# mudit1729/dinov2-od

Measured on AMD Instinct MI355X. Metric: images/sec forward, DINOv2 ViT-B/14 518x518 + 100-query head, higher is better.
Workload: dtype bf16; 1 GPU; ViT-B/14 518x518 bf16, 100 queries, batch 64 per GPU (BASELINE configs[2]'s batch of 64; it fits one GPU, so every GPU runs the whole configuration: weak scaling); global_batch=64, per_gpu_batch=64, image=518, queries=100, parallelism=dp1, hipgraph=True, n_ranks_seen=1, micro_batches=2

## Files before the change

dinov2_od_amd/csrc/dod_api.hip:

```cpp
#include "dod_internal.h"
#include "gemm_plan.h"

#include <cstdarg>
#include <cstdio>
#include <atomic>
#include <cstdlib>

using namespace dod;

static std::string g_err;

static int vfail(const dod_handle* h, int code, const char* fmt, va_list ap, int launch_rc = 0) {
  char buf[512];
  const int n = vsnprintf(buf, sizeof buf, fmt, ap);
  if (launch_rc && n >= 0 && (size_t)n < sizeof buf) snprintf(buf + n, sizeof buf - n, " rejected (rc %d)", launch_rc);
  if (h) h->err = buf; else g_err = buf;
  return code;
}
int dod::fail(const dod_handle* h, int code, const char* fmt, ...) {
  va_list ap; va_start(ap, fmt); code = vfail(h, code, fmt, ap); va_end(ap);
  return code;
}
int dod::rejected(const dod_handle* h, int r, const char* fmt, ...) {
  if (!r) return DOD_OK;
  va_list ap; va_start(ap, fmt); const int code = vfail(h, r == 3 ? DOD_ERR_HIP : DOD_ERR_INVALID, fmt, ap, r); va_end(ap);
  return code;
}

static bool check_common(dod_handle* h, int B, int H, int W, int* rc) {
  if (!h) { *rc = fail(nullptr, DOD_ERR_INVALID, "null handle"); return false; }
  if (!h->finalized) { *rc = fail(h, DOD_ERR_STATE, "dod_finalize_weights has not been called"); return false; }
  if (B <= 0) { *rc = fail(h, DOD_ERR_INVALID, "batch must be positive (got %d)", B); return false; }
  if (H < h->cfg.patch || W < h->cfg.patch) { *rc = fail(h, DOD_ERR_INVALID, "image %dx%d smaller than one %dx%d patch", H, W, h->cfg.patch, h->cfg.patch); return false; }
  return true;
}

static std::atomic<int> g_options[DOD_OPT_COUNT] = {{-1}, {-1}, {-1}, {-1}, {-1}, {-1}, {-1}, {-1}, {-1}, {-1}, {-1}};
int dod_option(int which) { return which >= 0 && which < DOD_OPT_COUNT ? g_options[which].load() : -1; }
static const char* const k_option_names[DOD_OPT_COUNT] = {"tailsplit", "dec_fused_split", "mha_chunk_images", "no_fused_patch", "ln_fold", "deterministic", "f32_ksplit",
                                                       "attn_bwd_flash", "epi_regmath", "f32x3_tile", "attn_diet"};

static std::atomic<long> g_form_launches[FORM_COUNT];
static const char* const k_form_names[FORM_COUNT] = {"bf16_128_r2", "bf16_128_r3", "bf16_m16", "k64", "ppm", "x3_16w", "x3_pp", "h2", "fp8_rows", "fp8mx_256x128",
                                                     "fp8mx2_256x128", "fp8mx2_256x256", "f32", "patch_fused"};
void gemm_form_launched(int form) { if (form >= 0 && form < FORM_COUNT) ++g_form_launches[form]; }

extern "C" {

int dod_test_set_option(const char* name, int value) {
  if (!name) return fail(nullptr, DOD_ERR_INVALID, "null option name");
  for (int i = 0; i < DOD_OPT_COUNT; ++i)
    if (!strcmp(name, k_option_names[i])) { g_options[i].store(value); return DOD_OK; }
  return fail(nullptr, DOD_ERR_INVALID, "unknown test option '%s'", name);
}
long dod_test_counter(const char* name) {
  if (name && !strcmp(name, "tail_splits")) return gemm_tail_split_count();
  if (name && !strcmp(name, "rem_cuts")) return gemm_rem_cut_count();
  if (name && !strcmp(name, "f32_ksplits")) return gemm_f32_ksplit_count();
  if (name && !strcmp(name, "epi_regmath")) return gemm_epi_regmath_count();
  if (name && !strcmp(name, "attn_diet")) return attn_half_tile_count();
  if (name && !strcmp(name, "f32x3_launches")) return gemm_f32x3_count(0);
  if (name && !strcmp(name, "f32x3_wide_launches")) return gemm_f32x3_count(1);
  if (name && !strcmp(name, "optim_launches")) return optim_launch_count();
  if (name && !strcmp(name, "optim_chunk_elems")) return optim_constant(0);
  if (name && !strcmp(name, "optim_table_tensors")) return optim_constant(1);
  if (name && !strcmp(name, "optim_norm_table_tensors")) return optim_constant(2);
  if (name && !strncmp(name, "form_", 5))
    for (int i = 0; i < FORM_COUNT; ++i)
      if (!strcmp(name + 5, k_form_names[i])) return g_form_launches[i].load();
  return -1;
}

int dod_test_gemm_plan(int family, int M, int N, int K, unsigned epi_flags, int cus, size_t scratch_bytes, dod_gemm_step* steps, int max_steps) {
  if (family < GEMM_BF16 || family > GEMM_F32 || M <= 0 || N <= 0 || K <= 0 || cus <= 0 || !steps) return -1;
  const GemmPlan pl = gemm_plan(family, M, N, K, epi_flags, gemm_policy(cus, scratch_bytes, scratch_bytes > 0));
  if (pl.n > 4 || pl.n > max_steps) return -1;
  for (int i = 0; i < pl.n; ++i) {
    const GemmStep& st = pl.step[i];
    steps[i].form = st.form; steps[i].row0 = st.row0; steps[i].rows = st.rows; steps[i].kslices = st.kslices; steps[i].regmath = st.regmath; steps[i].gm = st.gm;
  }
  return pl.n;
}

const char* dod_version(void) { return "dinodet 0.3 (gfx950)"; }
int dod_abi_version(void) { return DOD_ABI_VERSION; }

int dod_device_count(void) {
  int n = 0;
  return hipGetDeviceCount(&n) == hipSuccess ? n : -1;
}

const char* dod_last_error(const dod_handle* h) { return h ? h->err.c_str() : g_err.c_str(); }

int dod_create(const dod_config* cfg, dod_handle** out) {
  if (!cfg || !out) return fail(nullptr, DOD_ERR_INVALID, "null argument");
  const dod_config& c = *cfg;
  if (c.hidden <= 0 || c.layers <= 0 || c.heads <= 0 || c.hidden % c.heads) return fail(nullptr, DOD_ERR_INVALID, "bad backbone dims hidden=%d heads=%d layers=%d", c.hidden, c.heads, c.layers);
  if (c.hidden % 64) return fail(nullptr, DOD_ERR_INVALID, "hidden (%d) must be a multiple of 64", c.hidden);
  {
    const int fm = c.precision == DOD_PREC_FP32 ? 4 : 64;
    if (c.ffn_hidden <= 0 || c.ffn_hidden % fm) return fail(nullptr, DOD_ERR_INVALID, "ffn_hidden (%d) must be a multiple of %d in this precision", c.ffn_hidden, fm);
  }
  if (c.patch <= 0 || c.pos_grid <= 0) return fail(nullptr, DOD_ERR_INVALID, "bad patch/pos_grid");
  if (c.num_queries <= 0 || c.dec_hidden <= 0 || c.dec_heads <= 0 || c.dec_layers <= 0 || c.num_classes <= 0 || c.dim_feedforward <= 0) return fail(nullptr, DOD_ERR_INVALID, "bad decoder dims");
  if (c.dec_hidden % 64 || c.dim_feedforward % 4) return fail(nullptr, DOD_ERR_INVALID, "decoder hidden (%d) must be a multiple of 64, dim_feedforward (%d) of 4", c.dec_hidden, c.dim_feedforward);
  if (c.target_dim && c.target_dim != c.dec_hidden) return fail(nullptr, DOD_ERR_INVALID, "projection dim %d != decoder hidden %d", c.target_dim, c.dec_hidden);
  if (!c.target_dim && c.hidden != c.dec_hidden) return fail(nullptr, DOD_ERR_INVALID, "backbone width %d != decoder hidden %d and no projection", c.hidden, c.dec_hidden);
  if (c.use_deformable && (c.n_points <= 0 || c.n_points > 8)) return fail(nullptr, DOD_ERR_INVALID, "n_points must be 1..8");
  if (c.dec_layers > 64) return fail(nullptr, DOD_ERR_INVALID, "at most 64 decoder layers");
  if (c.precision != DOD_PREC_FP32 && c.precision != DOD_PREC_BF16 && c.precision != DOD_PREC_FP8 && c.precision != DOD_PREC_BF16X3 && c.precision != DOD_PREC_FP16X2) return fail(nullptr, DOD_ERR_INVALID, "unknown precision %d", c.precision);
  dod_handle* h = new (std::nothrow) dod_handle();
  if (!h) return fail(nullptr, DOD_ERR_STATE, "out of host memory");
  h->cfg = c;
  *out = h;
  return DOD_OK;
}

void dod_destroy(dod_handle* h) {
  if (!h) return;
  for (auto& r : h->prof) { (void)hipEventDestroy(r.a); (void)hipEventDestroy(r.b); }
  for (auto e : h->evpool) (void)hipEventDestroy(e);
  for (void* p : h->owned) (void)hipFree(p);
  delete h;
}

int dod_set_weight(dod_handle* h, const char* key, const void* dev_ptr, const int64_t* shape, int ndim, int dtype) {
  if (!h || !key || !dev_ptr || ndim < 0 || ndim > 8 || (ndim && !shape)) return fail(h, DOD_ERR_INVALID, "dod_set_weight: bad argument");
  if (dtype != DOD_F32 && dtype != DOD_BF16) return fail(h, DOD_ERR_INVALID, "dod_set_weight('%s'): dtype %d is neither DOD_F32 nor DOD_BF16", key, dtype);
  std::string k(key);
  if (k.rfind("module.", 0) == 0) k = k.substr(7);
  WRef r; r.raw = dev_ptr; r.dtype = dtype; r.ptr = dtype == DOD_F32 ? (const float*)dev_ptr : nullptr; r.shape.assign(shape, shape + ndim);
  h->w[k] = r;
  h->finalized = false;
  return DOD_OK;
}

int dod_reserve_gemm_scratch(size_t bytes) { return (gemm_tail_reserve(bytes) || gemm_f32_ksplit_reserve()) ? fail(nullptr, DOD_ERR_HIP, "scratch allocation of %zu bytes failed", bytes) : DOD_OK; }

int dod_finalize_weights(dod_handle* h, void* stream) {
  if (!h) return fail(nullptr, DOD_ERR_INVALID, "null handle");
  { static const size_t mb = [] { const char* v = getenv("DINODET_GEMM_SCRATCH_MB"); return v && atoi(v) > 0 ? (size_t)atoi(v) : (size_t)64; }();
    (void)gemm_tail_reserve(mb << 20);
    (void)gemm_f32_ksplit_reserve(); }
  int rc = finalize_impl(h, (hipStream_t)stream);
  if (rc || !h->has_dec) return rc;
  hipStream_t s = (hipStream_t)stream;
  const dod_config& g = h->cfg;
  const size_t Q = g.num_queries, Dd = g.dec_hidden;
  h->l0_tgt = h->l0_proj = nullptr;
  Carver sz(nullptr);
  const size_t bytes = carve_decoder(h, sz, 1, 1, nullptr, false) + 256;
  void* tmp = nullptr;
  float *t0 = nullptr, *p0 = nullptr;
  HIPCHK(h, hipMalloc(&tmp, bytes));
  if (hipMalloc((void**)&t0, Q * Dd * 4) != hipSuccess || (g.use_deformable && hipMalloc((void**)&p0, Q * (size_t)h->ncat * 4) != hipSuccess)) {
    (void)hipFree(tmp); if (t0) (void)hipFree(t0);
    return fail(h, DOD_ERR_HIP, "allocation of the decoder's layer-0 constants failed");
  }
  h->owned.push_back(t0); if (p0) h->owned.push_back(p0);
  Carver cv((void*)(((uintptr_t)tmp + 255) & ~(uintptr_t)255));
  DecWS dw;
  carve_decoder(h, cv, 1, 1, &dw, false);
  rc = decoder_impl(h, nullptr, 1, 1, dw, nullptr, s, true);
  if (!rc) {
    hipError_t e1 = hipMemcpyAsync(t0, dw.tgt, Q * Dd * 4, hipMemcpyDeviceToDevice, s);
    hipError_t e2 = p0 ? hipMemcpyAsync(p0, dw.proj, Q * (size_t)h->ncat * 4, hipMemcpyDeviceToDevice, s) : hipSuccess;
    hipError_t e3 = hipStreamSynchronize(s);
    if (e1 != hipSuccess || e2 != hipSuccess || e3 != hipSuccess) rc = fail(h, DOD_ERR_HIP, "decoder layer-0 constants: %s", hipGetErrorString(e3 != hipSuccess ? e3 : (e1 != hipSuccess ? e1 : e2)));
  } else (void)hipStreamSynchronize(s);
  (void)hipFree(tmp);
  if (rc) return rc;
  h->l0_tgt = t0; h->l0_proj = p0;
  return DOD_OK;
}

int dod_prepare(dod_handle* h, int H, int W, void* stream) {
  if (!h) return fail(nullptr, DOD_ERR_INVALID, "null handle");
  return prepare_impl(h, H, W, (hipStream_t)stream);
}

int dod_num_tokens(const dod_handle* h, int H, int W) { return h ? (H / h->cfg.patch) * (W / h->cfg.patch) + 1 : 0; }

size_t dod_workspace_bytes(const dod_handle* h, int B, int H, int W) {
  if (!h || B <= 0 || H < h->cfg.patch || W < h->cfg.patch) return 0;
  const int N = dod_num_tokens(h, H, W);
  Carver c(nullptr);
  carve_backbone(h, c, B, N, nullptr);
  carve_decoder(h, c, B, N, nullptr, false);
  return c.off + 256;
}

size_t dod_decoder_workspace_bytes(const dod_handle* h, int B, int N) {
  if (!h || B <= 0 || N <= 0) return 0;
  Carver c(nullptr);
  carve_decoder(h, c, B, N, nullptr, true);
  return c.off + 256;
}

int dod_set_tap(dod_handle* h, int stage, float* dst) {
  if (!h) return fail(nullptr, DOD_ERR_INVALID, "null handle");
  if (dst) h->taps[stage] = dst; else h->taps.erase(stage);
  return DOD_OK;
}

int dod_forward(dod_handle* h, const float* pixels, int B, int H, int W, float* det, void* workspace, size_t wsb, void* stream) {
  int rc;
  if (!check_common(h, B, H, W, &rc)) return rc;
  if (!pixels || !det || !workspace) return fail(h, DOD_ERR_INVALID, "null buffer");
  if (wsb < dod_workspace_bytes(h, B, H, W)) return fail(h, DOD_ERR_STATE, "workspace too small: %zu < %zu", wsb, dod_workspace_bytes(h, B, H, W));
  const int N = dod_num_tokens(h, H, W);
  Carver c(align_ws(workspace));
  BbWS bw; DecWS dw;
  carve_backbone(h, c, B, N, &bw);
  carve_decoder(h, c, B, N, &dw, false);
  CARVE_FITS(h, c, workspace, wsb)
  rc = backbone_impl(h, pixels, B, H, W, bw, nullptr, true, (hipStream_t)stream); if (rc) return rc;
  return decoder_impl(h, bw.mem, B, N, dw, det, (hipStream_t)stream);
}

int dod_forward_u8(dod_handle* h, const uint8_t* pixels_hwc, int B, int H, int W, float* det, void* workspace, size_t wsb, void* stream) {
  int rc;
  if (!check_common(h, B, H, W, &rc)) return rc;
  if (!pixels_hwc || !det || !workspace) return fail(h, DOD_ERR_INVALID, "null buffer");
  if (wsb < dod_workspace_bytes(h, B, H, W)) return fail(h, DOD_ERR_STATE, "workspace too small: %zu < %zu", wsb, dod_workspace_bytes(h, B, H, W));
  const int N = dod_num_tokens(h, H, W);
  Carver c(align_ws(workspace));
  BbWS bw; DecWS dw;
  carve_backbone(h, c, B, N, &bw);
  carve_decoder(h, c, B, N, &dw, false);
  CARVE_FITS(h, c, workspace, wsb)
  rc = backbone_impl(h, nullptr, B, H, W, bw, nullptr, true, (hipStream_t)stream, -1, nullptr, pixels_hwc); if (rc) return rc;
  return decoder_impl(h, bw.mem, B, N, dw, det, (hipStream_t)stream);
}

int dod_backbone_forward(dod_handle* h, const float* pixels, int B, int H, int W, float* features, void* workspace, size_t wsb, void* stream) {
  int rc;
  if (!check_common(h, B, H, W, &rc)) return rc;
  if (!pixels || !features || !workspace) return fail(h, DOD_ERR_INVALID, "null buffer");
  if (wsb < dod_workspace_bytes(h, B, H, W)) return fail(h, DOD_ERR_STATE, "workspace too small: %zu < %zu", wsb, dod_workspace_bytes(h, B, H, W));
  const int N = dod_num_tokens(h, H, W);
  Carver c(align_ws(workspace));
  BbWS bw;
  carve_backbone(h, c, B, N, &bw);
  CARVE_FITS(h, c, workspace, wsb)
  return backbone_impl(h, pixels, B, H, W, bw, features, false, (hipStream_t)stream);
}

int dod_backbone_prefix(dod_handle* h, const float* pixels, int B, int H, int W, int nblocks, float* x_out, void* workspace, size_t wsb, void* stream) {
  int rc;
  if (!check_common(h, B, H, W, &rc)) return rc;
  if (!pixels || !x_out || !workspace) return fail(h, DOD_ERR_INVALID, "null buffer");
  if (nblocks < 0 || nblocks > h->cfg.layers) return fail(h, DOD_ERR_INVALID, "nblocks %d outside 0..%d", nblocks, h->cfg.layers);
  if (wsb < dod_workspace_bytes(h, B, H, W)) return fail(h, DOD_ERR_STATE, "workspace too small: %zu < %zu", wsb, dod_workspace_bytes(h, B, H, W));
  const int N = dod_num_tokens(h, H, W);
  Carver c(align_ws(workspace));
  BbWS bw;
  carve_backbone(h, c, B, N, &bw);
  CARVE_FITS(h, c, workspace, wsb)
  return backbone_impl(h, pixels, B, H, W, bw, nullptr, false, (hipStream_t)stream, nblocks, x_out);
}

int dod_decoder_forward(dod_handle* h, const float* memory, int B, int N, float* det, void* workspace, size_t wsb, void* stream) {
  if (!h) return fail(nullptr, DOD_ERR_INVALID, "null handle");
  if (!h->finalized) return fail(h, DOD_ERR_STATE, "dod_finalize_weights has not been called");
  if (B <= 0 || N <= 0) return fail(h, DOD_ERR_INVALID, "bad B=%d N=%d", B, N);
  if (!memory || !det || !workspace) return fail(h, DOD_ERR_INVALID, "null buffer");
  if (wsb < dod_decoder_workspace_bytes(h, B, N)) return fail(h, DOD_ERR_STATE, "workspace too small");
  Carver c(align_ws(workspace));
  DecWS dw;
  carve_decoder(h, c, B, N, &dw, true);
  CARVE_FITS(h, c, workspace, wsb)
  hipStream_t s = (hipStream_t)stream;
  const void* mem_op = memory;
  if (is_bf16(h)) {
    KCHK(h, launch_cast_bf16(memory, (bf16_t*)dw.mem_op, (size_t)B * N * h->cfg.dec_hidden, s));
    mem_op = dw.mem_op;
  }
  return decoder_impl(h, mem_op, B, N, dw, det, s);
}

int dod_profile(dod_handle* h, int enable) {
  if (!h) return fail(nullptr, DOD_ERR_INVALID, "null handle");
  for (auto& r : h->prof) { h->evpool.push_back(r.a); h->evpool.push_back(r.b); }
  h->prof.clear();
  h->prof_on = enable != 0;
  return DOD_OK;
}

int dod_profile_read(dod_handle* h, int cls, double* ms, double* flops, int* launches) {
  if (!h || cls < 0 || cls >= PC_COUNT) return fail(h, DOD_ERR_INVALID, "bad profile class");
  double t = 0, f = 0; int n = 0;
  for (auto& r : h->prof) {
    if (r.cls != cls) continue;
    HIPCHK(h, hipEventSynchronize(r.b));
    float e = 0.f;
    HIPCHK(h, hipEventElapsedTime(&e, r.a, r.b));
    t += e; f += r.flops; ++n;
  }
  if (ms) *ms = t; if (flops) *flops = f; if (launches) *launches = n;
  return DOD_OK;
}

int dod_op_linear(int in_dtype, const void* A, int lda, const void* W, int ldw, int M, int N, int K, const float* bias,
                  const float* scale, const float* resid, int ldr, void* out, int out_dtype, int ldc, int act, void* stream) {
  if (!A || !W || !out) return fail(nullptr, DOD_ERR_INVALID, "null buffer");
  GemmEpi e = epi(bias, out_dtype == DOD_F32 ? (float*)out : nullptr, out_dtype == DOD_BF16 ? out : nullptr, ldc, act, scale, resid, ldr);
  if (act == DOD_ACT_SWIGLU_PAIRS) {
    if (in_dtype != DOD_BF16 || out_dtype != DOD_BF16 || scale || resid || (N & 7)) return fail(nullptr, DOD_ERR_INVALID, "DOD_ACT_SWIGLU_PAIRS: bf16 in / out, N %% 8 == 0, no scale / residual");
    e.act = ACT_NONE; e.glu = 1;
  }
  int r = in_dtype == DOD_BF16 ? launch_gemm_bf16((const bf16_t*)A, lda, (const bf16_t*)W, ldw, M, N, K, e, (hipStream_t)stream)
                               : launch_gemm_f32((const float*)A, lda, (const float*)W, ldw, M, N, K, e, (hipStream_t)stream);
  return rejected(nullptr, r, "dod_op_linear M=%d N=%d K=%d", M, N, K);
}
int dod_op_gemm_f32x(const float* A, int lda, int a_kmajor, long long a_sb, long long a_sh, const float* W, int ldw, int w_kmajor, long long w_sb,
                     long long w_sh, float* C, int ldc, long long c_sb, long long c_sh, int M, int N, int K, int batch, int hb, float alpha,
                     int accumulate, int ksplit, void* stream) {
  if (!A || !W || !C) return fail(nullptr, DOD_ERR_INVALID, "null buffer");
  GemmF32X g; memset(&g, 0, sizeof g);
  g.A = A; g.lda = lda; g.a_kmajor = a_kmajor; g.a_sb = a_sb; g.a_sh = a_sh;
  g.W = W; g.ldw = ldw; g.w_kmajor = w_kmajor; g.w_sb = w_sb; g.w_sh = w_sh;
  g.C = C; g.ldc = ldc; g.c_sb = c_sb; g.c_sh = c_sh;
  g.M = M; g.N = N; g.K = K; g.batch = batch; g.hb = hb; g.alpha = alpha; g.accumulate = accumulate; g.ksplit = ksplit;
  return rejected(nullptr, launch_gemm_f32x(g, (hipStream_t)stream), "dod_op_gemm_f32x M=%d N=%d K=%d batch=%d", M, N, K, batch);
}
int dod_op_gemm_f32x3(const float* A, int lda, int a_kmajor, long long a_sb, long long a_sh, const float* W, int ldw, int w_kmajor, long long w_sb,
                      long long w_sh, float* C, int ldc, long long c_sb, long long c_sh, int M, int N, int K, int batch, int hb, float alpha,
                      int accumulate, int ksplit, void* stream) {
  if (!A || !W || !C) return fail(nullptr, DOD_ERR_INVALID, "null buffer");
  GemmF32X g; memset(&g, 0, sizeof g);
  g.A = A; g.lda = lda; g.a_kmajor = a_kmajor; g.a_sb = a_sb; g.a_sh = a_sh;
  g.W = W; g.ldw = ldw; g.w_kmajor = w_kmajor; g.w_sb = w_sb; g.w_sh = w_sh;
  g.C = C; g.ldc = ldc; g.c_sb = c_sb; g.c_sh = c_sh;
  g.M = M; g.N = N; g.K = K; g.batch = batch; g.hb = hb; g.alpha = alpha; g.accumulate = accumulate; g.ksplit = ksplit;
  return rejected(nullptr, launch_gemm_f32x3(g, (hipStream_t)stream), "dod_op_gemm_f32x3 M=%d N=%d K=%d batch=%d", M, N, K, batch);
}
int dod_op_linear_f32x3(const float* X, int ldx, const float* W, const float* bias, const float* scale, const float* resid, int ldr, int M, int N, int K,
                        float* Y, int ldy, int act, void* stream) {
  if (!X || !W || !Y) return fail(nullptr, DOD_ERR_INVALID, "null buffer");
  if (act < DOD_ACT_NONE || act > DOD_ACT_SIGMOID) return fail(nullptr, DOD_ERR_INVALID, "dod_op_linear_f32x3: activation %d", act);
  GemmF32X g; memset(&g, 0, sizeof g);
  g.A = X; g.lda = ldx; g.W = W; g.ldw = K; g.C = Y; g.ldc = ldy; g.M = M; g.N = N; g.K = K; g.batch = 1; g.hb = 1; g.alpha = 1.0f; g.ksplit = 1;
  g.bias = bias; g.scale = scale; g.resid = resid; g.ldr = ldr; g.act = act;
  return rejected(nullptr, launch_gemm_f32x3(g, (hipStream_t)stream), "dod_op_linear_f32x3 M=%d N=%d K=%d", M, N, K);
}
int dod_op_linear_fp8(const void* A, int lda, const float* a_scale, const void* W, int ldw, const float* w_scale, int M, int N, int K,
                      const float* bias, const float* scale, const float* resid, int ldr, void* out, int out_dtype, int ldc, int act,
                      void* stream) {
  if (!A || !W || !out || !a_scale || !w_scale) return fail(nullptr, DOD_ERR_INVALID, "null buffer");
  GemmEpi e = epi(bias, out_dtype == DOD_F32 ? (float*)out : nullptr, out_dtype == DOD_BF16 ? out : nullptr, ldc, act, scale, resid, ldr);
  e.a_scale = a_scale; e.w_scale = w_scale;
  return rejected(nullptr, launch_gemm_fp8((const unsigned char*)A, lda, (const unsigned char*)W, ldw, M, N, K, e, (hipStream_t)stream), "dod_op_linear_fp8 M=%d N=%d K=%d", M, N, K);
}
int dod_op_linear_fp8_mx(const void* A, int lda, const void* a_block_scales, const void* W, int ldw, const float* w_scale, int M, int N, int K,
                         const float* bias, const float* scale, const float* resid, int ldr, void* out, int out_dtype, int ldc, int act,
                         void* stream) {
  if (!A || !W || !out || !a_block_scales || !w_scale) return fail(nullptr, DOD_ERR_INVALID, "null buffer");
  GemmEpi e = epi(bias, out_dtype == DOD_F32 ? (float*)out : nullptr, out_dtype == DOD_BF16 ? out : nullptr, ldc, act, scale, resid, ldr);
  e.a_bs = (const unsigned char*)a_block_scales; e.w_scale = w_scale;
  return rejected(nullptr, launch_gemm_fp8((const unsigned char*)A, lda, (const unsigned char*)W, ldw, M, N, K, e, (hipStream_t)stream), "dod_op_linear_fp8_mx M=%d N=%d K=%d", M, N, K);
}
int dod_op_linear_fp8_glu_mx(const void* A, int lda, const float* a_scale, const void* W, int ldw, const float* w_scale, int M, int N, int K,
                             const float* bias, void* out_q, int ldq, void* out_block_scales, void* stream) {
  if (!A || !W || !a_scale || !w_scale || !out_q || !out_block_scales) return fail(nullptr, DOD_ERR_INVALID, "null buffer");
  GemmEpi e = epi(bias, nullptr, out_q, ldq);
  e.a_scale = a_scale; e.w_scale = w_scale; e.glu = 1; e.out_bs = (unsigned char*)out_block_scales;
  return rejected(nullptr, launch_gemm_fp8((const unsigned char*)A, lda, (const unsigned char*)W, ldw, M, N, K, e, (hipStream_t)stream), "dod_op_linear_fp8_glu_mx M=%d N=%d K=%d", M, N, K);
}
int dod_op_linear_fp8_mx2(const void* A, int lda, const void* a_block_scales, const void* W, int ldw, const void* w_block_scales, int M, int N, int K,
                          const float* bias, const float* scale, const float* resid, int ldr, void* out, int out_dtype, int ldc, int act,
                          void* glu_out_block_scales, void* stream) {
  if (!A || !W || !out || !a_block_scales || !w_block_scales) return fail(nullptr, DOD_ERR_INVALID, "null buffer");
  GemmEpi e = epi(bias, out_dtype == DOD_F32 ? (float*)out : nullptr, out_dtype == DOD_BF16 ? out : nullptr, ldc, act, scale, resid, ldr);
  e.a_bs = (const unsigned char*)a_block_scales; e.w_bs = (const unsigned char*)w_block_scales;
  if (glu_out_block_scales) { e.out_f32 = nullptr; e.out_bf16 = (bf16_t*)out; e.glu = 1; e.out_bs = (unsigned char*)glu_out_block_scales; }
  return rejected(nullptr, launch_gemm_fp8((const unsigned char*)A, lda, (const unsigned char*)W, ldw, M, N, K, e, (hipStream_t)stream), "dod_op_linear_fp8_mx2 M=%d N=%d K=%d", M, N, K);
}
int dod_op_quant_mx_fp8(const void* x, int in_dtype, int ld, int rows, int cols, void* q, int ldq, void* block_scales, void* stream) {
  if (!x || !q || !block_scales) return fail(nullptr, DOD_ERR_INVALID, "null buffer");
  return rejected(nullptr, launch_quant_mx_fp8(x, in_dtype == DOD_BF16, ld, rows, cols, (unsigned char*)q, ldq, (unsigned char*)block_scales, (hipStream_t)stream), "dod_op_quant_mx_fp8 rows=%d cols=%d", rows, cols);
}
int dod_op_split_pair(const float* x, int ld, int rows, int cols, void* out, void* stream) {
  if (!x || !out) return fail(nullptr, DOD_ERR_INVALID, "null buffer");
  return launch_split2(x, ld, (bf16_t*)out, rows, cols, (hipStream_t)stream) ? fail(nullptr, DOD_ERR_HIP, "launch failed") : DOD_OK;
}
int dod_op_linear_x3(const void* A2, const void* W2, int M, int N, int K, const float* bias, const float* scale, const float* resid, int ldr,
                     void* out, int out_layout, int ldc, int act, void* stream) {
  if (!A2 || !W2 || !out) return fail(nullptr, DOD_ERR_INVALID, "null buffer");
  GemmEpi e = epi(bias, out_layout == 0 ? (float*)out : nullptr, out_layout != 0 ? out : nullptr, ldc, act, scale, resid, ldr);
  if (out_layout == 2) e.out_split = -N;
  return rejected(nullptr, launch_gemm_x3((const bf16_t*)A2, 2 * K, (const bf16_t*)W2, 2 * K, M, N, K, e, (hipStream_t)stream), "dod_op_linear_x3 M=%d N=%d K=%d", M, N, K);
}
int dod_op_split_h2(const float* x, int ld, int rows, int cols, void* out, void* wexp, void* stream) {
  if (!x || !out) return fail(nullptr, DOD_ERR_INVALID, "null buffer");
  return rejected(nullptr, launch_split_h2(x, ld, out, rows, cols, (unsigned char*)wexp, (hipStream_t)stream), "dod_op_split_h2 rows=%d cols=%d", rows, cols);
}
int dod_op_linear_h2(const void* A, const void* W, const void* wexp, int M, int N, int K, const float* bias, const float* scale, const float* resid,
                     int ldr, void* out, int out_layout, int ldc, int act, void* stream) {
  if (!A || !W || !wexp || !out) return fail(nullptr, DOD_ERR_INVALID, "null buffer");
  GemmEpi e = epi(bias, out_layout == 0 ? (float*)out : nullptr, out_layout != 0 ? out : nullptr, ldc, act, scale, resid, ldr);
  if (out_layout == 2) e.out_split = -N;
  if (out_layout == 3) e.out_h2 = 1;
  e.h2_wexp = (const unsigned char*)wexp;
  return rejected(nullptr, launch_gemm_h2(A, 4 * K, W, 3 * K, M, N, K, e, (hipStream_t)stream), "dod_op_linear_h2 M=%d N=%d K=%d", M, N, K);
}
int dod_op_linear_ln(int family, const void* A, const void* W, const void* wexp, int M, int N, int K, const float* bias, const float* scale,
                     const float* resid, int ldr, void* out, int out_layout, int ldc, int act, const dod_ln_fold* ln, void* stream) {
  if (!A || !W || !out || !ln) return fail(nullptr, DOD_ERR_INVALID, "null buffer");
  if (family != DOD_PREC_BF16 && family != DOD_PREC_BF16X3 && family != DOD_PREC_FP16X2) return fail(nullptr, DOD_ERR_INVALID, "family must be a bf16 / bf16x3 / fp16x2 precision");
  if ((ln->stats == nullptr) != (ln->csum == nullptr)) return fail(nullptr, DOD_ERR_INVALID, "stats and csum go together");
  if (ln->stats && scale) return fail(nullptr, DOD_ERR_INVALID, "the folded consumer has no LayerScale");
  if (ln->part && !(resid && out_layout == 0)) return fail(nullptr, DOD_ERR_INVALID, "the folded producer is the fp32 residual epilogue");
  GemmEpi e = epi(bias, out_layout == 0 ? (float*)out : nullptr, out_layout != 0 ? out : nullptr, ldc, act, scale, resid, ldr);
  if (out_layout == 2) e.out_split = -N;
  if (out_layout == 3) e.out_h2 = 1;
  e.ln_stats = (const float2*)ln->stats; e.ln_c = ln->csum;
  if (ln->part_in) {
    if (!ln->stats || ln->stats_out == ln->stats) return fail(nullptr, DOD_ERR_INVALID, "part_in needs stats (the shift) and a DIFFERENT stats_out buffer");
    e.ln_part_in = (const float2*)ln->part_in; e.ln_npart = (K + 127) / 128; e.ln_stats_out = (float2*)ln->stats_out; e.ln_eps = ln->eps;
  }
  if (ln->part) {
    e.ln_part = (float2*)ln->part; e.ln_npart = (N + 127) / 128; e.ln_op = ln->op_out; e.ln_shift = (const float2*)ln->shift;
    e.ln_op_kind = family == DOD_PREC_FP16X2 ? LNOP_H2 : (family == DOD_PREC_BF16X3 ? LNOP_PAIR : LNOP_BF16);
    e.ln_op_ld = family == DOD_PREC_BF16 ? N : 2 * N;
  }
  int r;
  if (family == DOD_PREC_FP16X2) {
    if (!wexp) return fail(nullptr, DOD_ERR_INVALID, "null buffer");
    e.h2_wexp = (const unsigned char*)wexp;
    r = launch_gemm_h2(A, 4 * K, W, 3 * K, M, N, K, e, (hipStream_t)stream);
  } else if (family == DOD_PREC_BF16X3) r = launch_gemm_x3((const bf16_t*)A, 2 * K, (const bf16_t*)W, 2 * K, M, N, K, e, (hipStream_t)stream);
  else r = launch_gemm_bf16((const bf16_t*)A, K, (const bf16_t*)W, K, M, N, K, e, (hipStream_t)stream);
  return rejected(nullptr, r, "dod_op_linear_ln M=%d N=%d K=%d", M, N, K);
}
int dod_op_rowstats(const float* x, int rows, int D, float eps, void* op_out, int family, void* stats, void* stream) {
  if (!x || !op_out || !stats) return fail(nullptr, DOD_ERR_INVALID, "null buffer");
  const int kind = family == DOD_PREC_FP16X2 ? LNOP_H2 : (family == DOD_PREC_BF16X3 ? LNOP_PAIR : (family == DOD_PREC_BF16 ? LNOP_BF16 : 0));
  return rejected(nullptr, launch_rowstats(x, rows, D, eps, op_out, kind, (float2*)stats, (hipStream_t)stream), "dod_op_rowstats rows=%d D=%d", rows, D);
}
int dod_op_ln_finalize(const void* part, int rows, int D, float eps, void* stats, void* stream) {
  if (!part || !stats) return fail(nullptr, DOD_ERR_INVALID, "null buffer");
  return rejected(nullptr, launch_ln_finalize((const float2*)part, (D + 127) / 128, rows, D, eps, (float2*)stats, (hipStream_t)stream), "dod_op_ln_finalize rows=%d D=%d", rows, D);
}
int dod_op_attention_x3(const void* qkv2, void* ctx2, int B, int N, int heads, float scale, void* stream) {
  if (!qkv2 || !ctx2) return fail(nullptr, DOD_ERR_INVALID, "null buffer");
  return rejected(nullptr, launch_attn_x3((const bf16_t*)qkv2, (bf16_t*)ctx2, B, N, heads, scale, (hipStream_t)stream), "dod_op_attention_x3");
}
static bool attn_grid_fits(int B, int N, int heads) {
  return (((long long)B * heads + 7) / 8 * 8) * (((long long)N + 127) / 128 + 1) <= 0x7fffffffLL;
}
int dod_op_attention_x3_h2(const void* qkv2, void* ctx_h2, int B, int N, int heads, float scale, void* stream) {
  if (!qkv2 || !ctx_h2) return fail(nullptr, DOD_ERR_INVALID, "null buffer");
  if (B <= 0 || N <= 0 || heads <= 0) return fail(nullptr, DOD_ERR_INVALID, "dod_op_attention_x3_h2: B=%d N=%d heads=%d must be positive", B, N, heads);
  if (!attn_grid_fits(B, N, heads)) return fail(nullptr, DOD_ERR_INVALID, "dod_op_attention_x3_h2: B=%d N=%d heads=%d is more workgroups than one launch holds", B, N, heads);
  return rejected(nullptr, launch_attn_x3((const bf16_t*)qkv2, (bf16_t*)ctx_h2, B, N, heads, scale, (hipStream_t)stream, 1), "dod_op_attention_x3_h2");
}
int dod_op_quant_rows_fp8(const void* x, int in_dtype, int ld, int rows, int cols, void* q, int ldq, float* scale, void* stream) {
  if (!x || !q || !scale) return fail(nullptr, DOD_ERR_INVALID, "null buffer");
  return rejected(nullptr, launch_quant_rows_fp8(x, in_dtype == DOD_BF16, ld, rows, cols, (unsigned char*)q, ldq, scale, (hipStream_t)stream), "dod_op_quant_rows_fp8 rows=%d cols=%d", rows, cols);
}
int dod_op_layernorm(const float* x, const float* add, const float* gamma, const float* beta, float eps, int rows, int D, void* out, int out_dtype, void* stream) {
  if (!x || !gamma || !beta || !out) return fail(nullptr, DOD_ERR_INVALID, "null buffer");
  return rejected(nullptr, launch_layernorm(x, add, gamma, beta, eps, rows, D, ln_out(out_dtype == DOD_F32 ? (float*)out : nullptr, out_dtype == DOD_BF16 ? (bf16_t*)out : nullptr), (hipStream_t)stream), "dod_op_layernorm rows=%d D=%d", rows, D);
}
int dod_op_attention_bf16(const void* qkv, void* ctx, int B, int N, int heads, float scale, void* stream) {
  if (!qkv || !ctx) return fail(nullptr, DOD_ERR_INVALID, "null buffer");
  return rejected(nullptr, launch_attn_bf16((const bf16_t*)qkv, (bf16_t*)ctx, B, N, heads, scale, (hipStream_t)stream), "dod_op_attention_bf16");
}
int dod_op_attention_bf16_mx(const void* qkv, void* ctx_q8, void* ctx_bs, int B, int N, int heads, float scale, void* stream) {
  if (!qkv || !ctx_q8 || !ctx_bs) return fail(nullptr, DOD_ERR_INVALID, "null buffer");
  if (B <= 0 || N <= 0 || heads <= 0) return fail(nullptr, DOD_ERR_INVALID, "dod_op_attention_bf16_mx: B=%d N=%d heads=%d must be positive", B, N, heads);
  if (!attn_grid_fits(B, N, heads)) return fail(nullptr, DOD_ERR_INVALID, "dod_op_attention_bf16_mx: B=%d N=%d heads=%d is more workgroups than one launch holds", B, N, heads);
  return rejected(nullptr, launch_attn_bf16((const bf16_t*)qkv, (bf16_t*)ctx_q8, B, N, heads, scale, (hipStream_t)stream, (unsigned char*)ctx_bs), "dod_op_attention_bf16_mx");
}
int dod_op_attention_f32(const float* q, const float* k, const float* v, float* o, int ldq, int ldk, int ldv, int ldo, int Lq, int Lk,
                         int B, int heads, int dh, float scale, void* stream) {
  if (!q || !k || !v || !o) return fail(nullptr, DOD_ERR_INVALID, "null buffer");
  AttnF32 a; a.q = q; a.k = k; a.v = v; a.o = o; a.ldq = ldq; a.ldk = ldk; a.ldv = ldv; a.ldo = ldo; a.Lq = Lq; a.Lk = Lk; a.B = B; a.heads = heads; a.dh = dh; a.scale = scale;
  return rejected(nullptr, launch_attn_f32(a, (hipStream_t)stream), "dod_op_attention_f32 (dh=%d)", dh);
}
int dod_op_deform_sample(const float* proj, int ldp, const float* values, int B, int Q, int N, int Hd, int P, int dh, int hh, int ww, float* out, void* stream) {
  if (!proj || !values || !out) return fail(nullptr, DOD_ERR_INVALID, "null buffer");
  if (hh * ww != N) return fail(nullptr, DOD_ERR_INVALID, "Cannot reshape input of size %d into a %dx%d feature map", N, hh, ww);
  return rejected(nullptr, launch_deform_sample(proj, ldp, values, B, Q, N, Hd, P, dh, hh, ww, out, (hipStream_t)stream), "dod_op_deform_sample");
}
int dod_op_pos_resize(const float* pos_in, int G, int gh, int gw, int D, float* pos_out, void* stream) {
  if (!pos_in || !pos_out) return fail(nullptr, DOD_ERR_INVALID, "null buffer");
  return launch_pos_resize(pos_in, G, gh, gw, D, pos_out, (hipStream_t)stream) ? fail(nullptr, DOD_ERR_HIP, "launch failed") : DOD_OK;
}
int dod_op_im2col(const float* img, int B, int H, int W, int patch, int Kp, void* out, int out_dtype, void* stream) {
  if (!img || !out) return fail(nullptr, DOD_ERR_INVALID, "null buffer");
  int r = launch_im2col(img, B, H, W, patch, Kp, out_dtype == DOD_F32 ? (float*)out : nullptr, out_dtype == DOD_BF16 ? (bf16_t*)out : nullptr, (hipStream_t)stream);
  return r ? fail(nullptr, DOD_ERR_INVALID, "dod_op_im2col rejected") : DOD_OK;
}

}
```

dinov2_od_amd/csrc/dod_common.h:

```cpp
#pragma once
#include <hip/hip_runtime.h>
#include <stdint.h>
#include <stdlib.h>

typedef __attribute__((ext_vector_type(8))) __bf16 bf16x8;
typedef __attribute__((ext_vector_type(4))) __bf16 bf16x4;
typedef __attribute__((ext_vector_type(2))) __bf16 bf16x2;
typedef __attribute__((ext_vector_type(16))) float f32x16;
typedef __attribute__((ext_vector_type(4))) float f32x4;
typedef __attribute__((ext_vector_type(2))) float f32x2;
typedef unsigned short bf16_t;

#define DOD_WAVE 64

enum { DOD_OPT_TAILSPLIT = 0,
       DOD_OPT_DEC_FUSED_SPLIT,
       DOD_OPT_MHA_CHUNK_IMAGES,
       DOD_OPT_NO_FUSED_PATCH,
       DOD_OPT_LN_FOLD,
       DOD_OPT_DETERMINISTIC,
       DOD_OPT_F32_KSPLIT,
       DOD_OPT_ATTN_BWD_FLASH,
       DOD_OPT_EPI_REGMATH,
       DOD_OPT_F32X3_TILE,
       DOD_OPT_ATTN_DIET,
       DOD_OPT_COUNT };
int dod_option(int which);
long gemm_tail_split_count();
long optim_launch_count();
long optim_constant(int which);
long gemm_rem_cut_count();
long attn_half_tile_count();
long gemm_epi_regmath_count();
enum { FORM_BF16_128_R2 = 0, FORM_BF16_128_R3, FORM_BF16_M16, FORM_K64, FORM_PPM, FORM_X3_16W, FORM_X3_PP, FORM_H2, FORM_FP8_ROWS, FORM_FP8MX_256X128,
       FORM_FP8MX2_256X128, FORM_FP8MX2_256X256, FORM_F32, FORM_PATCH_FUSED, FORM_COUNT };
void gemm_form_launched(int form);
enum { GEMM_BF16 = 0, GEMM_X3, GEMM_H2, GEMM_FP8, GEMM_F32 };

#ifdef DINODET_TUNING
#define DOD_TUNE_ENV(name) getenv(name)
#else
#define DOD_TUNE_ENV(name) (static_cast<const char*>(nullptr))
#endif

__device__ __forceinline__ bf16_t f2bf(float f) {
  __bf16 b = (__bf16)f;
  return __builtin_bit_cast(bf16_t, b);
}
__device__ __forceinline__ float bf2f(bf16_t h) {
  return __builtin_bit_cast(float, ((uint32_t)h) << 16);
}
__device__ __forceinline__ uint32_t pack2bf(float lo, float hi) {
  f32x2 v = {lo, hi};
  bf16x2 h = __builtin_convertvector(v, bf16x2);
  return __builtin_bit_cast(uint32_t, h);
}
__device__ __forceinline__ float wave_sum(float v) {
#pragma unroll
  for (int o = 32; o > 0; o >>= 1) v += __shfl_xor(v, o, 64);
  return v;
}
__device__ __forceinline__ float wave_max(float v) {
#pragma unroll
  for (int o = 32; o > 0; o >>= 1) v = fmaxf(v, __shfl_xor(v, o, 64));
  return v;
}
__device__ __forceinline__ unsigned pack4_fp8(float a, float b, float c, float d) {
  int w = __builtin_amdgcn_cvt_pk_fp8_f32(a, b, 0, false);
  w = __builtin_amdgcn_cvt_pk_fp8_f32(c, d, w, true);
  return (unsigned)w;
}
__device__ __forceinline__ unsigned mx_ebyte(float amax) {
  const unsigned b = __float_as_uint(amax * (1.0f / 448.0f));
  unsigned eb = ((b >> 23) & 0xffu) + ((b & 0x7fffffu) ? 1u : 0u);
  eb = eb < 1u ? 1u : (eb > 253u ? 253u : eb);
  return eb;
}
__device__ __forceinline__ float mx_inv_scale(unsigned eb) { return __uint_as_float((254u - eb) << 23); }
__device__ __forceinline__ size_t mx_scale_off(int K, int bi) { return (size_t)(bi & 1) * (K >> 6) + (bi >> 1); }
typedef __attribute__((ext_vector_type(2))) _Float16 f16x2;
typedef __attribute__((ext_vector_type(8))) _Float16 f16x8;
__device__ __forceinline__ float clampf_(float v, float lim) { return __builtin_fminf(__builtin_fmaxf(v, -lim), lim); }
__device__ __forceinline__ void h2_quad(float4 v, float shi, uint2& f16, unsigned& hi8, unsigned& lo8) {
  v.x = clampf_(v.x, 65504.f); v.y = clampf_(v.y, 65504.f); v.z = clampf_(v.z, 65504.f); v.w = clampf_(v.w, 65504.f);
  const f16x2 p0 = {(_Float16)v.x, (_Float16)v.y}, p1 = {(_Float16)v.z, (_Float16)v.w};
  f16.x = __builtin_bit_cast(unsigned, p0); f16.y = __builtin_bit_cast(unsigned, p1);
  const float hx = (float)p0.x, hy = (float)p0.y, hz = (float)p1.x, hw = (float)p1.y;
  const float slo = shi * 2048.0f;
  hi8 = pack4_fp8(clampf_(hx * shi, 448.f), clampf_(hy * shi, 448.f), clampf_(hz * shi, 448.f), clampf_(hw * shi, 448.f));
  lo8 = pack4_fp8(clampf_((v.x - hx) * slo, 448.f), clampf_((v.y - hy) * slo, 448.f), clampf_((v.z - hz) * slo, 448.f), clampf_((v.w - hw) * slo, 448.f));
}
__device__ __forceinline__ size_t h2_off8(int K, int c) { return (size_t)2 * K + (size_t)(c >> 4) * 32 + (c & 15); }

__device__ __forceinline__ float gelu_erf(float x) { return 0.5f * x * (1.0f + erff(x * 0.70710678118654752440f)); }
typedef float f32x2_t __attribute__((ext_vector_type(2)));
__device__ __forceinline__ f32x2_t gelu_fast2(f32x2_t x) {
  f32x2_t ax; ax.x = __builtin_fabsf(x.x); ax.y = __builtin_fabsf(x.y);
  const f32x2_t z = ax * 0.8493218002880191f;
  const f32x2_t d = __builtin_elementwise_fma(z, (f32x2_t)(0.2727374808792225f), (f32x2_t)(1.0f));
  f32x2_t t; t.x = __builtin_amdgcn_rcpf(d.x); t.y = __builtin_amdgcn_rcpf(d.y);
  f32x2_t p = __builtin_elementwise_fma(t, (f32x2_t)(0.5f * 1.061405429f), (f32x2_t)(0.5f * -1.453152027f));
  p = __builtin_elementwise_fma(p, t, (f32x2_t)(0.5f * 1.421413741f));
  p = __builtin_elementwise_fma(p, t, (f32x2_t)(0.5f * -0.284496736f));
  p = __builtin_elementwise_fma(p, t, (f32x2_t)(0.5f * 0.254829592f));
  const f32x2_t nz2 = -z * z;
  f32x2_t e; e.x = __builtin_amdgcn_exp2f(nz2.x); e.y = __builtin_amdgcn_exp2f(nz2.y);
  const f32x2_t q = ax * (t * p);
  const f32x2_t r = __builtin_elementwise_fma(ax, (f32x2_t)(0.5f), x * 0.5f);
  return __builtin_elementwise_fma(-q, e, r);
}
__device__ __forceinline__ void gelu_fast4(float4& v) {
  f32x2_t a = {v.x, v.y}, b = {v.z, v.w};
  a = gelu_fast2(a); b = gelu_fast2(b);
  v.x = a.x; v.y = a.y; v.z = b.x; v.w = b.y;
}
__device__ __forceinline__ float sigmoidf_(float x) { return 1.0f / (1.0f + expf(-x)); }

enum { ACT_NONE = 0, ACT_RELU = 1, ACT_GELU = 2, ACT_SIGMOID = 3 };

struct GemmEpi {
  const float* bias;
  const float* scale;
  const float* resid;
  int ldr;
  float* out_f32;
  bf16_t* out_bf16;
  int ldc;
  int act;
  const float* pos;
  int rows_per_img;
  int out_rows_per_img;
  int out_split;
  const float* a_scale;
  const float* w_scale;
  unsigned char* out_bs;
  const unsigned char* a_bs;
  const unsigned char* w_bs;
  int out_h2;
  const unsigned char* h2_wexp;
  int ksplit;
  int kslice_len;
  long long kslice_stride;
  int glu;
  void* ln_op;
  int ln_op_kind;
  int ln_op_ld;
  float2* ln_part;
  int ln_npart;
  const float2* ln_shift;
  const float2* ln_stats;
  const float* ln_c;
  const float2* ln_part_in;
  float2* ln_stats_out;
  float ln_eps;
};
enum { LNOP_BF16 = 1, LNOP_PAIR = 2, LNOP_H2 = 3 };
inline bool gemm_epi_rows_ok(const GemmEpi& e) {
  return e.rows_per_img == 0 && !e.pos && e.ksplit <= 1 && !e.a_scale && !e.a_bs && !e.out_bs;
}
inline GemmEpi gemm_epi_rows(const GemmEpi& e, int m0) {
  GemmEpi r = e;
  const size_t m = (size_t)m0;
  if (r.resid) r.resid += m * r.ldr;
  if (r.out_f32) r.out_f32 += m * r.ldc;
  if (r.out_bf16) r.out_bf16 += m * r.ldc;
  if (r.ln_op) r.ln_op = reinterpret_cast<char*>(r.ln_op) + m * (size_t)r.ln_op_ld * 2;
  if (r.ln_part) r.ln_part += m * r.ln_npart;
  if (r.ln_shift) r.ln_shift += m;
  if (r.ln_stats) r.ln_stats += m;
  if (r.ln_part_in) r.ln_part_in += m * r.ln_npart;
  if (r.ln_stats_out) r.ln_stats_out += m;
  return r;
}

int launch_gemm_bf16(const bf16_t* A, int lda, const bf16_t* W, int ldw, int M, int N, int K,
                     const GemmEpi& e, hipStream_t s);
int launch_gemm_f32(const float* A, int lda, const float* W, int ldw, int M, int N, int K,
                    const GemmEpi& e, hipStream_t s, bool allow_ksplit = false);
int gemm_f32_ksplit_reserve();
long gemm_f32_ksplit_count();
struct GemmF32X {
  const float* A; const float* W; float* C; const float* bias;
  const float* scale;
  const float* resid;
  int ldr;
  int lda, ldw, ldc, M, N, K;
  long long a_sb, a_sh, w_sb, w_sh, c_sb, c_sh;
  int batch, hb;
  int a_kmajor, w_kmajor;
  float alpha;
  int accumulate;
  int act;
  int ksplit;
};
int launch_gemm_f32x(const GemmF32X& g, hipStream_t s);
int launch_gemm_f32x3(const GemmF32X& g, hipStream_t s);
long gemm_f32x3_count(int wide);
int launch_quant_mx_fp8(const void* x, int in_bf16, int ld, int rows, int cols, unsigned char* q, int ldq, unsigned char* bs, hipStream_t s);
int launch_gemm_fp8(const unsigned char* A, int lda, const unsigned char* W, int ldw, int M, int N, int K,
                    const GemmEpi& e, hipStream_t s);
int launch_attn_x3(const bf16_t* qkv2, bf16_t* ctx3, int B, int N, int heads, float scale, hipStream_t s, int ctx_h2 = 0);
int launch_swiglu_fp8(const bf16_t* in, int rows, int Fh, unsigned char* q, float* scale, hipStream_t s);
int launch_quant_rows_fp8(const void* x, int in_bf16, int ld, int rows, int cols, unsigned char* q, int ldq, float* scale,
                          hipStream_t s);

struct LnOut {
  float* f32 = nullptr;
  bf16_t* bf16 = nullptr;
  unsigned char* fp8 = nullptr;
  float* scale = nullptr;
  bf16_t* split = nullptr;
  bf16_t* a3 = nullptr;
  unsigned char* bs = nullptr;
};
inline LnOut ln_out(float* f32, bf16_t* bf16 = nullptr, bf16_t* a3 = nullptr) { LnOut o; o.f32 = f32; o.bf16 = bf16; o.a3 = a3; return o; }
int launch_layernorm(const float* x, const float* add, const float* gamma, const float* beta, float eps, int rows, int D, const LnOut& out,
                     hipStream_t s, int split_h2 = 0);
int launch_rowstats(const float* x, int rows, int D, float eps, void* op, int op_kind, float2* stats, hipStream_t s);
int launch_ln_finalize(const float2* part, int npart, int rows, int D, float eps, float2* stats, hipStream_t s);
int launch_ln_fold(const float* W, int rows, int cols, const float* gamma, const float* beta, const float* bias_in, float* Wout, float* bias_out, hipStream_t s);
int launch_rowsum(const float* W, int rows, int cols, int round_bf16, float* c, hipStream_t s);

int launch_attn_bf16(const bf16_t* qkv, bf16_t* ctx, int B, int N, int heads, float scale, hipStream_t s, unsigned char* ctx_bs = nullptr);

struct AttnF32 {
  const float *q, *k, *v; float* o;
  int ldq, ldk, ldv, ldo;
  int Lq, Lk;
  int B, heads, dh;
  float scale;
  bf16_t* o3 = nullptr;
  float* lse = nullptr;
};
int launch_attn_f32(const AttnF32& a, hipStream_t s);
struct AttnF32Bwd {
  const float *q, *k, *v, *o, *d_o, *lse;
  float *dq, *dk, *dv, *delta;
  int ldq, ldk, ldv, ldo, lddq, lddk, lddv;
  int Lq, Lk, B, heads, dh;
  float scale;
};
int launch_attn_f32_bwd(const AttnF32Bwd& a, hipStream_t s);

int launch_im2col(const float* img, int B, int H, int W, int patch, int Kp, float* out_f32, bf16_t* out_bf16, hipStream_t s);
int launch_patch_pack(const float* W, int D, int p, bf16_t* out, int x3, hipStream_t s);
int launch_patch_embed(const void* img, int u8, int B, int H, int W, int p, const bf16_t* Wp, int x3, const float* bias, const float* pos,
                       float* out, int D, hipStream_t s);
int launch_cls_row(const float* cls, const float* pos, float* x, int B, int N, int D, hipStream_t s);
int launch_pos_resize(const float* pos_in, int G, int gh, int gw, int D, float* pos_out, hipStream_t s);
int launch_interleave_halves(const float* src, float* dst, int F, int cols, hipStream_t s);
int launch_swiglu(const float* in_f32, const bf16_t* in_bf16, int rows, int Fh, float* out_f32, bf16_t* out_bf16, hipStream_t s);
int launch_cast_bf16(const float* in, bf16_t* out, size_t n, hipStream_t s);
int launch_copy2d(const float* src, int ld_src, float* dst, int ld_dst, int rows, int cols, int cols_pad, hipStream_t s);
int launch_lora_merge(const float* W, const float* A, const float* Bm, float alpha, int out_f, int in_f, int r, float* dst, hipStream_t s);
int launch_split3(const float* in, int ld_in, bf16_t* out, int rows, int K, int mode, hipStream_t s);
int launch_split2(const float* in, int ld_in, bf16_t* out, int rows, int K, hipStream_t s);
int launch_split_h2(const float* in, int ld_in, void* out, int rows, int K, unsigned char* wexp, hipStream_t s);
int launch_gemm_h2(const void* A, int lda, const void* W, int ldw, int M, int N, int K, const GemmEpi& e, hipStream_t s);
int launch_gemm_x3(const bf16_t* A2, int lda, const bf16_t* W2, int ldw, int M, int N, int K, const GemmEpi& e, hipStream_t s);
int gemm_dispatch(int family, const void* A, int lda, const void* W, int ldw, int M, int N, int K, const GemmEpi& e, hipStream_t s, bool allow_ksplit = false);
int device_cus();
struct KernelLds { const void* fn; int bytes; };
void gemm_lds_attr_once(bool* done, const KernelLds* k, int n);
int gemm_tile_mode();
int run_gemm_bf16_128(const bf16_t* A, int lda, const bf16_t* W, int ldw, int M, int N, int K, const GemmEpi& e, int slots, hipStream_t s);
int run_gemm_bf16_m16(const bf16_t* A, int lda, const bf16_t* W, int ldw, int M, int N, int K, const GemmEpi& e, int gm, hipStream_t s);
int run_gemm_x3_16w(const bf16_t* A2, int lda, const bf16_t* W2, int ldw, int M, int N, int K, const GemmEpi& e, hipStream_t s);
int run_gemm_k64(const bf16_t* A, int lda, const bf16_t* W, int ldw, int M, int N, int K, const GemmEpi& e, bool regmath, hipStream_t s);
int run_gemm_pp(bool x3, const bf16_t* A, int lda, const bf16_t* W, int ldw, int M, int N, int K, const GemmEpi& e, hipStream_t s);
int run_gemm_h2(const void* A, int lda, const void* W, int ldw, int M, int N, int K, const GemmEpi& e, hipStream_t s);
int run_gemm_ksplit_reduce(const float* part, int S, int R, int N, const GemmEpi& e, int m_base, int M, int K, hipStream_t s);
int run_gemm_fp8(int form, const unsigned char* A, int lda, const unsigned char* W, int ldw, int M, int N, int K, const GemmEpi& e, int gm, hipStream_t s);
int run_gemm_f32(const float* A, int lda, const float* W, int ldw, int M, int N, int K, const GemmEpi& e, int S, hipStream_t s);
int gemm_tail_reserve(size_t bytes);
size_t gemm_tail_reserved();
float* gemm_tail_slab(hipStream_t s);
bool gemm_f32_ksplit_reserved();
int launch_bcast_rows(const float* src, float* dst, int B, int rows, int D, hipStream_t s);

int launch_deform_sample(const float* proj, int ldp, const float* values, int B, int Q, int N, int Hd, int P, int dh,
                         int h, int w, float* out, hipStream_t s, int proj_shared = 0, bf16_t* out3 = nullptr);
```

dinov2_od_amd/csrc/dod_forward.hip:

```cpp
#include "dod_internal.h"

#include <cmath>
#include <cstdlib>

using namespace dod;

size_t dod::carve_decoder(const dod_handle* h, Carver& c, int B, int N, DecWS* w, bool need_mem_op) {
  const dod_config& g = h->cfg;
  const size_t BQ = (size_t)B * g.num_queries, Dd = g.dec_hidden, M = (size_t)B * N;
  DecWS t;
  t.tgt = (float*)c.take(BQ * Dd * 4); t.t2 = (float*)c.take(BQ * Dd * 4); t.att = (float*)c.take(BQ * Dd * 4);
  t.samp = (float*)c.take(BQ * Dd * 4); t.qkv = (float*)c.take(BQ * 3 * Dd * 4);
  t.proj = (float*)c.take(BQ * (size_t)(h->ncat > 0 ? h->ncat : 4) * 4);
  t.ffn = (float*)c.take(BQ * (size_t)g.dim_feedforward * 4); t.hb = (float*)c.take(BQ * (Dd / 2) * 4);
  t.qd = (float*)c.take(BQ * Dd * 4);
  { const size_t kmax = Dd > (size_t)g.dim_feedforward ? Dd : (size_t)g.dim_feedforward;
    const bool want3 = is_bf16(h) || is_x3(h);
    t.a3 = want3 ? (bf16_t*)c.take(BQ * 3 * kmax * 2) : nullptr;
    t.a3b = want3 ? (bf16_t*)c.take(BQ * 3 * kmax * 2) : nullptr; }
  t.mem2 = is_x3(h) ? (bf16_t*)c.take(M * 2 * Dd * 2) : nullptr;
  t.mem_op = need_mem_op ? c.take(M * Dd * esz(h)) : nullptr;
  if (g.use_deformable) {
    int uniq = 0; for (auto& L : h->DL) if (L.vp_alias < 0) ++uniq;
    if (!h->finalized) uniq = g.dec_layers;
    t.values = (float*)c.take(M * Dd * 4 * (size_t)(uniq > 0 ? uniq : 1)); t.kv = nullptr;
  } else {
    t.values = nullptr; t.kv = (float*)c.take(M * 2 * Dd * 4);
  }
  if (w) *w = t;
  return c.off;
}

size_t dod::carve_backbone(const dod_handle* h, Carver& c, int B, int N, BbWS* w) {
  const dod_config& g = h->cfg;
  const size_t M = (size_t)B * N, D = g.hidden, es = esz(h), Np = N - 1;
  const size_t F1 = g.swiglu ? 2 * (size_t)g.ffn_hidden : (size_t)g.ffn_hidden;
  size_t hb = M * F1; const size_t col = (size_t)B * Np * (size_t)(h->Kp ? h->Kp : (3 * g.patch * g.patch + 63) / 64 * 64);
  if (col > hb) hb = col;
  BbWS t;
  t.x = (float*)c.take(M * D * 4); t.y = c.take(M * D * es); t.qkv = c.take(M * 3 * D * es); t.ctx = c.take(M * D * es);
  t.hbuf = c.take(hb * es); t.gated = g.swiglu ? c.take(M * (size_t)g.ffn_hidden * es) : nullptr;
  t.mem = c.take(M * (size_t)(g.target_dim ? g.target_dim : g.hidden) * es);
  t.rs = is_fp8(h) ? (float*)c.take(M * 4) : nullptr;
  t.bs = (is_fp8(h) && g.swiglu && g.ffn_hidden % 256 == 0) ? (unsigned char*)c.take(M * (size_t)(g.ffn_hidden / 32)) : nullptr;
  t.bsx = (is_fp8(h) && D % 256 == 0) ? (unsigned char*)c.take(M * (D / 32)) : nullptr;
  const bool foldable = ln_foldable(h);
  t.lnp = foldable ? (float2*)c.take(M * ((D + 127) / 128) * 8) : nullptr;
  t.lns = foldable ? (float2*)c.take(M * 8) : nullptr;
  t.lns2 = foldable ? (float2*)c.take(M * 8) : nullptr;
  if (w) *w = t;
  return c.off;
}

int dod::prepare_impl(dod_handle* h, int H, int W, hipStream_t s) {
  const dod_config& g = h->cfg;
  if (!h->finalized || !h->has_bb) return fail(h, DOD_ERR_STATE, "backbone weights not finalized");
  if (H < g.patch || W < g.patch) return fail(h, DOD_ERR_INVALID, "image %dx%d smaller than one patch", H, W);
  if (h->pos_H == H && h->pos_W == W) return DOD_OK;
  const int gh = H / g.patch, gw = W / g.patch;
  if (gh * gw == g.pos_grid * g.pos_grid && H == W) { h->pos_hw = h->pos; h->pos_H = H; h->pos_W = W; return DOD_OK; }
  const std::pair<int, int> key(gh, gw);
  auto it = h->pos_cache.find(key);
  if (it == h->pos_cache.end()) {
    hipStreamCaptureStatus cs = hipStreamCaptureStatusNone;
    if (s && hipStreamIsCapturing(s, &cs) == hipSuccess && cs != hipStreamCaptureStatusNone)
      return fail(h, DOD_ERR_STATE, "first forward at %dx%d inside a stream capture: call dod_prepare(h, %d, %d) before capturing", H, W, H, W);
    const size_t need = (size_t)(gh * gw + 1) * g.hidden;
    float* buf = nullptr;
    HIPCHK(h, hipMalloc((void**)&buf, need * 4));
    h->owned.push_back(buf);
    KCHK(h, launch_pos_resize(h->pos, g.pos_grid, gh, gw, g.hidden, buf, s));
    it = h->pos_cache.emplace(key, buf).first;
  }
  h->pos_hw = it->second; h->pos_H = H; h->pos_W = W;
  return DOD_OK;
}

namespace {

void spatial_factor(int hw, int* h, int* w) {
  int s = (int)std::sqrt((double)hw);
  while ((s + 1) * (s + 1) <= hw) ++s;
  while (s * s > hw) --s;
  if (s * s != hw) {
    for (int i = s; i > 0; --i) if (hw % i == 0) { *h = i; *w = hw / i; return; }
  }
  *h = s; *w = s;
}

int tap(dod_handle* h, int stage, const void* src, bool src_bf16, size_t n, hipStream_t s) {
  auto it = h->taps.find(stage);
  if (it == h->taps.end() || !it->second) return 0;
  if (!src_bf16) { (void)hipMemcpyAsync(it->second, src, n * 4, hipMemcpyDeviceToDevice, s); return 0; }
  return launch_widen_bf16((const bf16_t*)src, it->second, n, s);
}

int linear(dod_handle* h, bool bf, const void* A, int lda, const void* W, int ldw, int M, int N, int K, const GemmEpi& e, hipStream_t s, int flops_K = 0) {
  ProfScope ps(h, s, bf ? PC_GEMM_BF16 : PC_GEMM_F32, 2.0 * M * N * (e.rows_per_img > 0 ? 3.0 * h->cfg.patch * h->cfg.patch : (double)(flops_K ? flops_K : K)));
  int r = bf ? launch_gemm_bf16((const bf16_t*)A, lda, (const bf16_t*)W, ldw, M, N, K, e, s)
             : launch_gemm_f32((const float*)A, lda, (const float*)W, ldw, M, N, K, e, s, h->cfg.precision != DOD_PREC_FP32);
  return rejected(h, r, "linear launch (M=%d N=%d K=%d bf16=%d)", M, N, K, (int)bf);
}
int linear3(dod_handle* h, const void* A3, const void* W3, int M, int N, int K, const GemmEpi& e, hipStream_t s) {
  ProfScope ps(h, s, PC_GEMM_BF16, 2.0 * M * N * (double)K);
  int r = launch_gemm_x3((const bf16_t*)A3, 2 * K, (const bf16_t*)W3, 2 * K, M, N, K, e, s);
  return rejected(h, r, "bf16x3 linear launch (M=%d N=%d K=%d)", M, N, K);
}

struct Operand {
  const void* rows;
  const float* row_scale = nullptr;
  const unsigned char* bs = nullptr;
};

int block_linear(dod_handle* h, const Operand& a, const PackedLinear& W, int M, int N, int K, GemmEpi e, hipStream_t s) {
  if (is_h2(h)) {
    ProfScope ps(h, s, PC_GEMM_BF16, 2.0 * M * N * (double)K);
    e.h2_wexp = W.wexp;
    return rejected(h, launch_gemm_h2(a.rows, 4 * K, W.W, 3 * K, M, N, K, e, s), "fp16x2 linear launch (M=%d N=%d K=%d)", M, N, K);
  }
  if (is_x3(h)) return linear3(h, a.rows, W.W, M, N, K, e, s);
  if (W.wscale || W.wbs) {
    ProfScope ps(h, s, PC_GEMM_FP8, 2.0 * M * N * (double)K);
    e.a_scale = a.row_scale; e.w_scale = W.wscale; e.a_bs = a.bs; e.w_bs = W.wbs;
    return rejected(h, launch_gemm_fp8((const unsigned char*)a.rows, K, (const unsigned char*)W.W, K, M, N, K, e, s), "fp8 linear launch (M=%d N=%d K=%d)", M, N, K);
  }
  return linear(h, is_bf16(h), a.rows, K, W.W, K, M, N, K, e, s);
}

struct BlockRun {
  dod_handle* h; const BbWS& ws; hipStream_t s;
  int B, N, M, D, F;
  bool bf, f8, x3, h2, fold;
  float scale;
  float2* stat[2];
  int cur = 0;
  bool fresh = false;
  int op_kind, npart;

  BlockRun(dod_handle* h_, const BbWS& ws_, hipStream_t s_, int B_, int N_, bool fold_)
      : h(h_), ws(ws_), s(s_), B(B_), N(N_), M(B_ * N_), D(h_->cfg.hidden), F(h_->cfg.ffn_hidden), bf(is_bf16(h_)), f8(is_fp8(h_)), x3(is_x3(h_)),
        h2(is_h2(h_)), fold(fold_), scale(1.0f / std::sqrt((float)(h_->cfg.hidden / h_->cfg.heads))), stat{ws_.lns, ws_.lns2},
        op_kind(is_h2(h_) ? LNOP_H2 : (is_x3(h_) ? LNOP_PAIR : LNOP_BF16)), npart((h_->cfg.hidden + 127) / 128) {}

  bool mx(const BLayer& L) const { return f8 && L.qkv.wbs && ws.bsx; }

  GemmEpi residual_epi(const PackedLinear& W, const float* layer_scale, bool next_norm_reads) {
    GemmEpi e = epi(W.bias, ws.x, nullptr, D, ACT_NONE, layer_scale, ws.x, D);
    if (fold && next_norm_reads) {
      e.ln_op = ws.y; e.ln_op_kind = op_kind; e.ln_op_ld = (op_kind == LNOP_BF16 ? D : 2 * D); e.ln_part = ws.lnp; e.ln_npart = npart; e.ln_shift = stat[cur];
      fresh = true;
    }
    return e;
  }
  GemmEpi normed_epi(GemmEpi e, const PackedLinear& W) {
    if (fold) {
      e.ln_stats = stat[cur]; e.ln_c = W.csum;
      if (fresh) { e.ln_part_in = ws.lnp; e.ln_npart = npart; e.ln_stats_out = stat[cur ^ 1]; e.ln_eps = h->cfg.ln_eps; cur ^= 1; fresh = false; }
    }
    return e;
  }
  int norm(const BLayer& L, const float* gamma, const float* beta, Operand* y) {
    *y = Operand{ws.y, f8 && !mx(L) ? ws.rs : nullptr, mx(L) ? ws.bsx : nullptr};
    if (fold) return 0;
    LnOut o;
    if (x3) o.split = (bf16_t*)ws.y;
    else if (f8) { o.fp8 = (unsigned char*)ws.y; o.scale = (float*)y->row_scale; o.bs = (unsigned char*)y->bs; }
    else if (bf) o.bf16 = (bf16_t*)ws.y;
    else o.f32 = (float*)ws.y;
    ProfScope ps(h, s, PC_LAYERNORM, 0);
    KCHK(h, launch_layernorm(ws.x, nullptr, gamma, beta, h->cfg.ln_eps, M, D, o, s, h2 ? 1 : 0));
    return 0;
  }
  int attention(const BLayer& L, const Operand& y, Operand* ctx) {
    const int heads = h->cfg.heads;
    const bool flash = D / heads == 64;
    GemmEpi eq = epi(L.qkv.bias, bf ? nullptr : (float*)ws.qkv, bf ? ws.qkv : nullptr, 3 * D);
    if (x3 && flash) { eq = epi(L.qkv.bias, nullptr, ws.qkv, 6 * D); eq.out_split = -3 * D; }
    int rc = block_linear(h, y, L.qkv, M, 3 * D, D, normed_epi(eq, L.qkv), s); if (rc) return rc;
    const double flops = 4.0 * B * (double)N * N * D;
    *ctx = Operand{ws.ctx};
    if (x3 && flash) {
      ProfScope ps(h, s, PC_ATTN_BF16, flops);
      KCHK(h, launch_attn_x3((const bf16_t*)ws.qkv, (bf16_t*)ws.ctx, B, N, heads, scale, s, h2 ? 1 : 0));
    } else if (bf && mx(L)) {
      ProfScope ps(h, s, PC_ATTN_BF16, flops);
      KCHK(h, launch_attn_bf16((const bf16_t*)ws.qkv, (bf16_t*)ws.y, B, N, heads, scale, s, ws.bsx));
      *ctx = Operand{ws.y, nullptr, ws.bsx};
    } else if (bf) {
      { ProfScope ps(h, s, PC_ATTN_BF16, flops); KCHK(h, launch_attn_bf16((const bf16_t*)ws.qkv, (bf16_t*)ws.ctx, B, N, heads, scale, s)); }
      if (f8) {
        KCHK(h, launch_quant_rows_fp8(ws.ctx, 1, D, M, D, (unsigned char*)ws.y, D, ws.rs, s));
        *ctx = Operand{ws.y, ws.rs};
      }
    } else {
      float* o = x3 ? (float*)ws.hbuf : (float*)ws.ctx;
      {
        ProfScope ps(h, s, PC_ATTN_F32, flops);
        AttnF32 a; const float* q = (const float*)ws.qkv;
        a.q = q; a.k = q + D; a.v = q + 2 * D; a.o = o; a.ldq = a.ldk = a.ldv = 3 * D; a.ldo = D;
        a.Lq = a.Lk = N; a.B = B; a.heads = heads; a.dh = D / heads; a.scale = scale;
        KCHK(h, launch_attn_f32(a, s));
      }
      if (x3) KCHK(h, split(o, D, ws.ctx));
    }
    return 0;
  }
  int split(const float* src, int cols, void* dst) {
    return h2 ? launch_split_h2(src, cols, dst, M, cols, nullptr, s) : launch_split2(src, cols, (bf16_t*)dst, M, cols, s);
  }
  int mlp_in(const BLayer& L, const Operand& y, Operand* hidden) {
    const dod_config& g = h->cfg;
    static const bool mx_gate_env = [] { const char* v = DOD_TUNE_ENV("DINODET_FP8_MX_GATE"); return !(v && v[0] == '0'); }();
    const PackedLinear& W = L.fc1;
    int rc;
    if (!g.swiglu) {
      GemmEpi e1 = epi(W.bias, bf ? nullptr : (float*)ws.hbuf, bf ? ws.hbuf : nullptr, F, ACT_GELU);
      if (x3) { e1 = epi(W.bias, nullptr, ws.hbuf, 2 * F, ACT_GELU); if (h2) e1.out_h2 = 1; else e1.out_split = -F; }
      *hidden = Operand{ws.hbuf};
      return block_linear(h, y, W, M, F, D, normed_epi(e1, W), s);
    }
    if (L.glu) {
      GemmEpi eg = epi(W.bias, nullptr, ws.gated, F);
      *hidden = Operand{ws.gated};
      const bool gate_mx = f8 && ws.bs && (mx(L) || (mx_gate_env && F % 256 == 0));
      if (x3) { eg = epi(W.bias, nullptr, ws.hbuf, 2 * F); if (h2) eg.out_h2 = 1; else eg.out_split = -F; *hidden = Operand{ws.hbuf}; }
      else if (gate_mx) { eg.out_bs = ws.bs; *hidden = Operand{ws.gated, nullptr, ws.bs}; }
      else if (f8) eg = epi(W.bias, nullptr, ws.hbuf, F);
      eg.glu = 1;
      rc = block_linear(h, y, W, M, 2 * F, D, normed_epi(eg, W), s); if (rc) return rc;
      if (f8 && !gate_mx) {
        KCHK(h, launch_quant_rows_fp8(ws.hbuf, 1, F, M, F, (unsigned char*)ws.gated, F, ws.rs, s));
        *hidden = Operand{ws.gated, ws.rs};
      }
      return 0;
    }
    rc = block_linear(h, y, W, M, 2 * F, D, normed_epi(epi(W.bias, bf ? nullptr : (float*)ws.hbuf, bf ? ws.hbuf : nullptr, 2 * F), W), s); if (rc) return rc;
    *hidden = Operand{ws.gated};
    if (f8) { KCHK(h, launch_swiglu_fp8((const bf16_t*)ws.hbuf, M, F, (unsigned char*)ws.gated, ws.rs, s)); *hidden = Operand{ws.gated, ws.rs}; }
    else KCHK(h, launch_swiglu(bf ? nullptr : (const float*)ws.hbuf, bf ? (const bf16_t*)ws.hbuf : nullptr, M, F, bf ? nullptr : (float*)ws.gated, bf ? (bf16_t*)ws.gated : nullptr, s));
    if (x3) { KCHK(h, split((const float*)ws.gated, F, ws.hbuf)); *hidden = Operand{ws.hbuf}; }
    return 0;
  }
  int block(const BLayer& L, bool more) {
    if (mx(L) && h->cfg.swiglu && !(L.glu && ws.bs)) return fail(h, DOD_ERR_STATE, "fp8 SwiGLU MLP needs the fused gate (block-scaled rows)");
    Operand y, ctx, hidden;
    int rc = norm(L, L.ln1w, L.ln1b, &y); if (rc) return rc;
    rc = attention(L, y, &ctx); if (rc) return rc;
    rc = block_linear(h, ctx, L.o, M, D, D, residual_epi(L.o, L.ls1, true), s); if (rc) return rc;
    rc = norm(L, L.ln2w, L.ln2b, &y); if (rc) return rc;
    rc = mlp_in(L, y, &hidden); if (rc) return rc;
    return block_linear(h, hidden, L.fc2, M, D, F, residual_epi(L.fc2, L.ls2, more), s);
  }
};

}

int dod::backbone_impl(dod_handle* h, const float* pixels, int B, int H, int W, const BbWS& ws, float* feat_f32, bool want_mem, hipStream_t s,
                       int stop_blocks, float* x_out, const unsigned char* pixels_u8) {
  const dod_config& g = h->cfg;
  const bool bf = is_bf16(h);
  const int D = g.hidden, p = g.patch;
  const int gh = H / p, gw = W / p, Np = gh * gw, N = Np + 1, M = B * N;
  if (!h->has_bb) return fail(h, DOD_ERR_STATE, "no backbone weights were registered");
  if (bf && D / g.heads != 64) return fail(h, DOD_ERR_INVALID, "bf16 attention kernel needs head_dim 64 (got %d)", D / g.heads);
  int rc = prepare_impl(h, H, W, s); if (rc) return rc;
  if (pixels_u8 && !h->Wpe) return fail(h, DOD_ERR_INVALID, "uint8 input needs the fused patch embed (bf16 / bf16x3 / fp8 precision, patch size 14 or 16)");
  if (h->Wpe && (pixels_u8 || W % 2 == 0)) {
    ProfScope ps(h, s, PC_GEMM_BF16, 2.0 * B * Np * (double)D * 3.0 * p * p);
    KCHK(h, launch_patch_embed(pixels_u8 ? (const void*)pixels_u8 : (const void*)pixels, pixels_u8 ? 1 : 0, B, H, W, p, h->Wpe, is_x3(h) ? 1 : 0,
                               h->bpatch, h->pos_hw, ws.x, D, s));
  } else if (is_x3(h) && h->Wpatch2 && (size_t)3 * D * 6 >= (size_t)h->Kp2 * 4) {
    const int K2 = h->Kp2;
    KCHK(h, launch_im2col(pixels, B, H, W, p, K2, (float*)ws.hbuf, nullptr, s));
    KCHK(h, launch_split2((const float*)ws.hbuf, K2, (bf16_t*)ws.qkv, B * Np, K2, s));
    GemmEpi e = epi(h->bpatch, ws.x, nullptr, D);
    e.pos = h->pos_hw; e.rows_per_img = Np; e.out_rows_per_img = N;
    ProfScope ps(h, s, PC_GEMM_BF16, 2.0 * B * Np * (double)D * 3.0 * p * p);
    KCHK(h, launch_gemm_x3((const bf16_t*)ws.qkv, 2 * K2, h->Wpatch2, 2 * K2, B * Np, D, K2, e, s));
  } else {
    KCHK(h, launch_im2col(pixels, B, H, W, p, h->Kp, bf ? nullptr : (float*)ws.hbuf, bf ? (bf16_t*)ws.hbuf : nullptr, s));
    GemmEpi e = epi(h->bpatch, ws.x, nullptr, D);
    e.pos = h->pos_hw; e.rows_per_img = Np; e.out_rows_per_img = N;
    rc = linear(h, bf, ws.hbuf, h->Kp, h->Wpatch, h->Kp, B * Np, D, h->Kp, e, s); if (rc) return rc;
  }
  KCHK(h, launch_cls_row(h->cls, h->pos_hw, ws.x, B, N, D, s));
  tap(h, 0, ws.x, false, (size_t)M * D, s);
  float* yf = bf ? nullptr : (float*)ws.y; bf16_t* yb = bf ? (bf16_t*)ws.y : nullptr;
  const bool x3 = is_x3(h);
  const int nblocks = stop_blocks >= 0 ? (stop_blocks < g.layers ? stop_blocks : g.layers) : g.layers;
  const bool fold = ln_foldable(h) && !h->L.empty() && h->L[0].fold;
  if (fold && !(ws.lnp && ws.lns && ws.lns2)) return fail(h, DOD_ERR_STATE, "internal: the weights were packed with the LayerNorm folded but the workspace has no statistics buffers");
  BlockRun run(h, ws, s, B, N, fold);
  if (fold && nblocks > 0) { ProfScope ps(h, s, PC_LAYERNORM, 0); KCHK(h, launch_rowstats(ws.x, M, D, g.ln_eps, ws.y, run.op_kind, run.stat[0], s)); }
  for (int i = 0; i < nblocks; ++i) {
    rc = run.block(h->L[i], i + 1 < g.layers); if (rc) return rc;
    tap(h, 1 + i, ws.x, false, (size_t)M * D, s);
  }
  if (stop_blocks >= 0) {
    HIPCHK(h, hipMemcpyAsync(x_out, ws.x, (size_t)M * D * 4, hipMemcpyDeviceToDevice, s));
    return DOD_OK;
  }
  if (!g.target_dim) {
    float* of = feat_f32 ? feat_f32 : (bf ? nullptr : (want_mem ? (float*)ws.mem : nullptr));
    bf16_t* ob = (bf && want_mem) ? (bf16_t*)ws.mem : nullptr;
    KCHK(h, launch_layernorm(ws.x, nullptr, h->lnfw, h->lnfb, g.ln_eps, M, D, ln_out(of, ob), s));
    if (!bf && want_mem && feat_f32) HIPCHK(h, hipMemcpyAsync(ws.mem, feat_f32, (size_t)M * D * 4, hipMemcpyDeviceToDevice, s));
  } else {
    const int Dd = g.target_dim;
    if (x3) {
      { LnOut o; o.split = (bf16_t*)ws.y; KCHK(h, launch_layernorm(ws.x, nullptr, h->lnfw, h->lnfb, g.ln_eps, M, D, o, s)); }
      float* dst = feat_f32 ? feat_f32 : (float*)ws.mem;
      rc = linear3(h, ws.y, h->Wproj, M, Dd, D, epi(h->bproj, dst, nullptr, Dd), s); if (rc) return rc;
      if (feat_f32 && want_mem) HIPCHK(h, hipMemcpyAsync(ws.mem, feat_f32, (size_t)M * Dd * 4, hipMemcpyDeviceToDevice, s));
      return DOD_OK;
    }
    KCHK(h, launch_layernorm(ws.x, nullptr, h->lnfw, h->lnfb, g.ln_eps, M, D, ln_out(yf, yb), s));
    if (feat_f32) { rc = linear(h, bf, ws.y, D, h->Wproj, D, M, Dd, D, epi(h->bproj, feat_f32, nullptr, Dd), s); if (rc) return rc; }
    if (want_mem) { rc = linear(h, bf, ws.y, D, h->Wproj, D, M, Dd, D, epi(h->bproj, bf ? nullptr : (float*)ws.mem, bf ? ws.mem : nullptr, Dd), s); if (rc) return rc; }
  }
  return DOD_OK;
}

int dod::decoder_impl(dod_handle* h, const void* mem_op, int B, int N, const DecWS& ws, float* det, hipStream_t s, bool l0_only) {
  const dod_config& g = h->cfg;
  const bool bf = is_bf16(h);
  const int Dd = g.dec_hidden, Q = g.num_queries, Hd = g.dec_heads, Pn = g.n_points, Fd = g.dim_feedforward, C = g.num_classes;
  const int BQ = B * Q, M = B * N, dh = Dd / Hd;
  if (!h->has_dec) return fail(h, DOD_ERR_STATE, "no decoder weights were registered");
  if (Dd % Hd) return fail(h, DOD_ERR_INVALID, "decoder hidden %d not divisible by heads %d", Dd, Hd);
  if (dh > 128 || dh % 4) return fail(h, DOD_ERR_INVALID, "decoder head_dim %d unsupported (<=128, multiple of 4)", dh);
  int rc;
  if (!l0_only) tap(h, 1000, mem_op, bf, (size_t)M * Dd, s);
  const bool x3 = is_x3(h) && ws.mem2;
  if (x3 && !l0_only) KCHK(h, launch_split2((const float*)mem_op, Dd, ws.mem2, M, Dd, s));
  const bool l0_const = !l0_only && h->l0_tgt && (!g.use_deformable || h->l0_proj);
  if (!l0_const) KCHK(h, launch_bcast_rows(h->query, ws.tgt, 1, Q, Dd, s));
  int fh = 0, fw = 0;
  if (g.use_deformable && !l0_only) {
    spatial_factor(N, &fh, &fw);
    int u = 0;
    for (int j = 0; j < g.dec_layers; ++j) {
      DLayer& L = h->DL[j];
      if (L.vp_alias >= 0) continue;
      float* dst = ws.values + (size_t)u * M * Dd; ++u;
      if (x3 && L.vp_w2) rc = linear3(h, ws.mem2, L.vp_w2, M, Dd, Dd, epi(L.vp_b, dst, nullptr, Dd), s);
      else rc = linear(h, bf, mem_op, Dd, L.vp_w, Dd, M, Dd, Dd, epi(L.vp_b, dst, nullptr, Dd), s);
      if (rc) return rc;
    }
    tap(h, 2000, ws.values, false, (size_t)M * Dd, s);
  }
  const float sscale = 1.0f / std::sqrt((float)dh);
  static const int qrows = DOD_TUNE_ENV("DINODET_QSPLIT_ROWS") ? atoi(DOD_TUNE_ENV("DINODET_QSPLIT_ROWS")) : 1024;
  const bool fuse3 = dod_option(DOD_OPT_DEC_FUSED_SPLIT) != 0;
  auto splits = [&](const bf16_t* W3, int rows, int Nout, int ldc, int act) {
    return (bf || x3) && W3 && ws.a3 && rows >= qrows && Nout >= 128 && Nout % 4 == 0 && ldc % 4 == 0 && act != ACT_SIGMOID;
  };
  auto qlinear = [&](const float* A, int K, const float* Wf, const bf16_t* W3, int rows, int Nout, const GemmEpi& e, const bf16_t* A3 = nullptr) -> int {
    if (splits(W3, rows, Nout, e.ldc, e.act)) {
      if (!A3) { KCHK(h, launch_split3(A, K, ws.a3, rows, K, 0, s)); A3 = ws.a3; }
      return linear(h, true, A3, 3 * K, W3, 3 * K, rows, Nout, 3 * K, e, s, K);
    }
    return linear(h, false, A, K, Wf, K, rows, Nout, K, e, s);
  };
  const bf16_t* tgt3 = nullptr;
  auto post_norm = [&](const float* gamma, const float* beta, int rows, bool next_splits) -> int {
    KCHK(h, launch_layernorm(ws.t2, nullptr, gamma, beta, g.dec_ln_eps, rows, Dd, ln_out(ws.tgt, nullptr, next_splits ? ws.a3 : nullptr), s));
    tgt3 = next_splits ? ws.a3 : nullptr;
    return 0;
  };
  auto self_attn = [&](const DLayer& L, int nb) -> int {
    const int rows = nb * Q;
    int r = qlinear(ws.tgt, Dd, L.in_w, L.in_w3, rows, 3 * Dd, epi(L.in_b, ws.qkv, nullptr, 3 * Dd), tgt3); if (r) return r;
    tgt3 = nullptr;
    AttnF32 a; a.q = ws.qkv; a.k = ws.qkv + Dd; a.v = ws.qkv + 2 * Dd; a.o = ws.att; a.ldq = a.ldk = a.ldv = 3 * Dd; a.ldo = Dd;
    a.Lq = a.Lk = Q; a.B = nb; a.heads = Hd; a.dh = dh; a.scale = sscale;
    const bool o3 = fuse3 && splits(L.out_w3, rows, Dd, Dd, ACT_NONE);
    if (o3) a.o3 = ws.a3;
    KCHK(h, launch_attn_f32(a, s));
    r = qlinear(ws.att, Dd, L.out_w, L.out_w3, rows, Dd, epi(L.out_b, ws.t2, nullptr, Dd, ACT_NONE, nullptr, ws.tgt, Dd), o3 ? ws.a3 : nullptr); if (r) return r;
    const bool n3 = fuse3 && !g.use_deformable && nb == B && splits(L.ca_q_w3, rows, Dd, Dd, ACT_NONE);
    return post_norm(L.n1w, L.n1b, rows, n3);
  };
  auto ffn = [&](const DLayer& L, bool last_layer, const bf16_t* L_next_in_w3) -> int {
    const bool f3 = fuse3 && splits(L.l1w3, BQ, Fd, Fd, ACT_RELU) && splits(L.l2w3, BQ, Dd, Dd, ACT_NONE) && Fd % 4 == 0;
    int r;
    if (f3) {
      GemmEpi e1 = epi(L.l1b, nullptr, nullptr, 3 * Fd, ACT_RELU);
      e1.out_bf16 = ws.a3b; e1.out_split = Fd;
      r = qlinear(ws.tgt, Dd, L.l1w, L.l1w3, BQ, Fd, e1, tgt3);
    } else r = qlinear(ws.tgt, Dd, L.l1w, L.l1w3, BQ, Fd, epi(L.l1b, ws.ffn, nullptr, Fd, ACT_RELU), tgt3);
    if (r) return r;
    tgt3 = nullptr;
    r = qlinear(ws.ffn, Fd, L.l2w, L.l2w3, BQ, Dd, epi(L.l2b, ws.t2, nullptr, Dd, ACT_NONE, nullptr, ws.tgt, Dd), f3 ? ws.a3b : nullptr); if (r) return r;
    const bool n3 = fuse3 && (last_layer ? splits(h->bb0_w3, BQ, Dd / 2, Dd / 2, ACT_RELU) : splits(L_next_in_w3, BQ, 3 * Dd, 3 * Dd, ACT_NONE));
    return post_norm(L.n3w, L.n3b, BQ, n3);
  };
  int uniq_idx[64]; { int u = 0; for (int j = 0; j < g.dec_layers && j < 64; ++j) uniq_idx[j] = h->DL[j].vp_alias < 0 ? u++ : -1; }
  for (int j = 0; j < g.dec_layers; ++j) {
    const DLayer& L = h->DL[j];
    const bool const0 = j == 0 && l0_const;
    const bool shared0 = (j == 0 && (B > 1 || const0));
    if (const0) { KCHK(h, launch_bcast_rows(h->l0_tgt, ws.tgt, B, Q, Dd, s)); tgt3 = nullptr; }
    else { rc = self_attn(L, shared0 ? 1 : B); if (rc) return rc; }
    if (g.use_deformable) {
      if (!const0) { rc = linear(h, false, ws.tgt, Dd, L.cat_w, Dd, shared0 ? Q : BQ, h->ncat, Dd, epi(L.cat_b, ws.proj, nullptr, h->ncat), s); if (rc) return rc; }
      if (l0_only) return DOD_OK;
      if (shared0 && !const0) KCHK(h, launch_bcast_rows(ws.tgt, ws.tgt + (size_t)Q * Dd, B - 1, Q, Dd, s));
      const int src = L.vp_alias >= 0 ? L.vp_alias : j;
      const float* vals = ws.values + (size_t)uniq_idx[src] * M * Dd;
      const bool s3 = fuse3 && splits(L.op_w3, BQ, Dd, Dd, ACT_NONE);
      KCHK(h, launch_deform_sample(const0 ? h->l0_proj : ws.proj, h->ncat, vals, B, Q, N, Hd, Pn, dh, fh, fw, ws.samp, s, shared0 ? 1 : 0, s3 ? ws.a3 : nullptr));
      rc = qlinear(ws.samp, Dd, L.op_w, L.op_w3, BQ, Dd, epi(L.op_b, ws.t2, nullptr, Dd, ACT_NONE, nullptr, ws.tgt, Dd), s3 ? ws.a3 : nullptr); if (rc) return rc;
      const bool n3 = fuse3 && splits(L.l1w3, BQ, Fd, Fd, ACT_RELU);
      rc = post_norm(L.n2w, L.n2b, BQ, n3); if (rc) return rc;
    } else {
      if (l0_only) return DOD_OK;
      if (shared0 && !const0) KCHK(h, launch_bcast_rows(ws.tgt, ws.tgt + (size_t)Q * Dd, B - 1, Q, Dd, s));
      rc = qlinear(ws.tgt, Dd, L.ca_q_w, L.ca_q_w3, BQ, Dd, epi(L.ca_q_b, ws.qd, nullptr, Dd), tgt3); if (rc) return rc;
      tgt3 = nullptr;
      if (x3 && L.ca_kv_w2) rc = linear3(h, ws.mem2, L.ca_kv_w2, M, 2 * Dd, Dd, epi(L.ca_kv_b, ws.kv, nullptr, 2 * Dd), s);
      else rc = linear(h, bf, mem_op, Dd, L.ca_kv_w, Dd, M, 2 * Dd, Dd, epi(L.ca_kv_b, ws.kv, nullptr, 2 * Dd), s);
      if (rc) return rc;
      AttnF32 a; a.q = ws.qd; a.k = ws.kv; a.v = ws.kv + Dd; a.o = ws.att; a.ldq = Dd; a.ldk = a.ldv = 2 * Dd; a.ldo = Dd;
      a.Lq = Q; a.Lk = N; a.B = B; a.heads = Hd; a.dh = dh; a.scale = sscale;
      const bool o3 = fuse3 && splits(L.ca_out_w3, BQ, Dd, Dd, ACT_NONE);
      if (o3) a.o3 = ws.a3;
      KCHK(h, launch_attn_f32(a, s));
      rc = qlinear(ws.att, Dd, L.ca_out_w, L.ca_out_w3, BQ, Dd, epi(L.ca_out_b, ws.t2, nullptr, Dd, ACT_NONE, nullptr, ws.tgt, Dd), o3 ? ws.a3 : nullptr); if (rc) return rc;
      const bool n3 = fuse3 && splits(L.l1w3, BQ, Fd, Fd, ACT_RELU);
      rc = post_norm(L.n2w, L.n2b, BQ, n3); if (rc) return rc;
    }
    rc = ffn(L, j + 1 == g.dec_layers, j + 1 < g.dec_layers ? h->DL[j + 1].in_w3 : nullptr); if (rc) return rc;
    tap(h, 3000 + j, ws.tgt, false, (size_t)BQ * Dd, s);
  }
  rc = linear(h, false, ws.tgt, Dd, h->cls_w, Dd, BQ, C, Dd, epi(h->cls_b, det, nullptr, C + 4), s); if (rc) return rc;
  rc = qlinear(ws.tgt, Dd, h->bb0_w, h->bb0_w3, BQ, Dd / 2, epi(h->bb0_b, ws.hb, nullptr, Dd / 2, ACT_RELU), tgt3); if (rc) return rc;
  rc = linear(h, false, ws.hb, Dd / 2, h->bb2_w, Dd / 2, BQ, 4, Dd / 2, epi(h->bb2_b, det + C, nullptr, C + 4, ACT_SIGMOID), s); if (rc) return rc;
  return DOD_OK;
}
```

dinov2_od_amd/csrc/dod_internal.h:

```cpp
#pragma once
#include "dod_common.h"
#include "../../include/dinodet.h"

#include <cstring>
#include <map>
#include <string>
#include <vector>

struct WRef { const float* ptr; std::vector<int64_t> shape; const void* raw = nullptr; int dtype = DOD_F32; size_t numel() const { size_t n = 1; for (auto s : shape) n *= (size_t)s; return n; } };

struct PackedLinear {
  void* W = nullptr;
  float* bias = nullptr;
  const unsigned char* wexp = nullptr;
  const float* wscale = nullptr;
  const unsigned char* wbs = nullptr;
  const float* csum = nullptr;
};
struct BLayer {
  PackedLinear qkv, o, fc1, fc2;
  float *ln1w = nullptr, *ln1b = nullptr, *ln2w = nullptr, *ln2b = nullptr, *ls1 = nullptr, *ls2 = nullptr;
  bool glu = false;
  bool fold = false;
};
struct DLayer {
  float *in_w = nullptr, *in_b = nullptr, *out_w = nullptr, *out_b = nullptr;
  float *n1w = nullptr, *n1b = nullptr, *n2w = nullptr, *n2b = nullptr, *n3w = nullptr, *n3b = nullptr;
  float *l1w = nullptr, *l1b = nullptr, *l2w = nullptr, *l2b = nullptr;
  bf16_t *in_w3 = nullptr, *out_w3 = nullptr, *l1w3 = nullptr, *l2w3 = nullptr, *op_w3 = nullptr, *ca_q_w3 = nullptr, *ca_out_w3 = nullptr;
  float *cat_w = nullptr, *cat_b = nullptr, *op_w = nullptr, *op_b = nullptr, *vp_b = nullptr;
  void* vp_w = nullptr;
  bf16_t* vp_w2 = nullptr;
  bf16_t* ca_kv_w2 = nullptr;
  int vp_alias = -1;
  float *ca_q_w = nullptr, *ca_q_b = nullptr, *ca_kv_b = nullptr, *ca_out_w = nullptr, *ca_out_b = nullptr;
  void* ca_kv_w = nullptr;
};

struct dod_handle {
  dod_config cfg;
  std::map<std::string, WRef> w;
  mutable std::string err;
  bool finalized = false;
  bool has_bb = false, has_dec = false;
  std::vector<void*> owned;
  std::vector<BLayer> L;
  void* Wpatch = nullptr; int Kp = 0;
  bf16_t* Wpatch2 = nullptr; int Kp2 = 0;
  bf16_t* Wpe = nullptr;
  float *bpatch = nullptr, *cls = nullptr, *pos = nullptr, *lnfw = nullptr, *lnfb = nullptr, *bproj = nullptr;
  void* Wproj = nullptr;
  std::vector<DLayer> DL;
  bf16_t* bb0_w3 = nullptr;
  float *query = nullptr, *cls_w = nullptr, *cls_b = nullptr, *bb0_w = nullptr, *bb0_b = nullptr, *bb2_w = nullptr, *bb2_b = nullptr;
  int ncat = 0;
  float *l0_tgt = nullptr, *l0_proj = nullptr;
  std::map<std::pair<int, int>, float*> pos_cache;
  int pos_H = -1, pos_W = -1; float* pos_hw = nullptr;
  std::map<int, float*> taps;
  bool prof_on = false;
  struct ProfRec { hipEvent_t a, b; int cls; double flops; };
  std::vector<ProfRec> prof;
  std::vector<hipEvent_t> evpool;
};

namespace dod {

int fail(const dod_handle* h, int code, const char* fmt, ...) __attribute__((format(printf, 3, 4)));
int rejected(const dod_handle* h, int r, const char* fmt, ...) __attribute__((format(printf, 3, 4)));
#define HIPCHK(h, x) do { hipError_t e_ = (x); if (e_ != hipSuccess) return dod::fail(h, DOD_ERR_HIP, "%s: %s", #x, hipGetErrorString(e_)); } while (0)
#define KCHK(h, x) do { int r_ = (x); if (r_) return dod::rejected(h, r_, "%s", #x); } while (0)

enum { PC_GEMM_BF16 = 0, PC_ATTN_BF16 = 1, PC_GEMM_F32 = 2, PC_ATTN_F32 = 3, PC_LAYERNORM = 4, PC_OTHER = 5, PC_GEMM_FP8 = 6, PC_COUNT = 7 };
struct ProfScope {
  dod_handle* h; hipStream_t s; int cls; double flops; hipEvent_t a = nullptr;
  ProfScope(dod_handle* h_, hipStream_t s_, int cls_, double flops_) : h(h_), s(s_), cls(cls_), flops(flops_) {
    if (!h->prof_on) return;
    a = take();
    if (a) (void)hipEventRecord(a, s);
  }
  hipEvent_t take() {
    hipEvent_t e = nullptr;
    if (!h->evpool.empty()) { e = h->evpool.back(); h->evpool.pop_back(); return e; }
    if (hipEventCreate(&e) != hipSuccess) return nullptr;
    return e;
  }
  ~ProfScope() {
    if (!h->prof_on || !a) return;
    hipEvent_t b = take();
    if (!b) { h->evpool.push_back(a); return; }
    (void)hipEventRecord(b, s);
    h->prof.push_back({a, b, cls, flops});
  }
};

inline bool is_fp8(const dod_handle* h) { return h->cfg.precision == DOD_PREC_FP8; }
inline bool is_x3(const dod_handle* h) { return h->cfg.precision == DOD_PREC_BF16X3 || h->cfg.precision == DOD_PREC_FP16X2; }
inline bool is_h2(const dod_handle* h) { return h->cfg.precision == DOD_PREC_FP16X2; }
inline bool is_bf16(const dod_handle* h) { return h->cfg.precision == DOD_PREC_BF16 || is_fp8(h); }
inline size_t esz(const dod_handle* h) { return is_x3(h) ? 6 : (is_bf16(h) ? 2 : 4); }
inline size_t align_up(size_t x, size_t a = 256) { return (x + a - 1) / a * a; }
inline bool ln_foldable(const dod_handle* h) { return !is_fp8(h) && (is_bf16(h) || is_x3(h)) && h->cfg.hidden % 32 == 0; }

inline GemmEpi epi(const float* bias, float* of32, void* obf, int ldc, int act = ACT_NONE, const float* scale = nullptr, const float* resid = nullptr, int ldr = 0) {
  GemmEpi e; memset(&e, 0, sizeof e);
  e.bias = bias; e.out_f32 = of32; e.out_bf16 = (bf16_t*)obf; e.ldc = ldc; e.act = act; e.scale = scale; e.resid = resid; e.ldr = ldr;
  return e;
}

struct Carver {
  char* base; size_t off = 0;
  explicit Carver(void* b) : base((char*)b) {}
  void* take(size_t bytes) { void* p = base ? base + off : nullptr; off += align_up(bytes); return p; }
};
inline void* align_ws(void* p) { return (void*)(((uintptr_t)p + 255) & ~(uintptr_t)255); }
#define CARVE_FITS(h, c, workspace, wsb)                                                                                      \
  if ((size_t)((c).base - (char*)(workspace)) + (c).off > (wsb))                                                              \
    return dod::fail(h, DOD_ERR_STATE, "internal: workspace carve %zu exceeds the %zu bytes provided", (size_t)((c).base - (char*)(workspace)) + (c).off, (size_t)(wsb));
struct DecWS { float *tgt, *t2, *att, *samp, *qkv, *proj, *ffn, *hb, *qd; void* mem_op; float* values; float* kv; bf16_t* a3; bf16_t* a3b; bf16_t* mem2; };
struct BbWS { float* x; void *y, *qkv, *ctx, *hbuf, *gated, *mem; float* rs; unsigned char* bs; unsigned char* bsx; float2 *lnp, *lns, *lns2; };
size_t carve_decoder(const dod_handle* h, Carver& c, int B, int N, DecWS* w, bool need_mem_op);
size_t carve_backbone(const dod_handle* h, Carver& c, int B, int N, BbWS* w);

int finalize_impl(dod_handle* h, hipStream_t s);
int launch_widen_bf16(const bf16_t* in, float* out, size_t n, hipStream_t s);
int prepare_impl(dod_handle* h, int H, int W, hipStream_t s);
int backbone_impl(dod_handle* h, const float* pixels, int B, int H, int W, const BbWS& ws, float* feat_f32, bool want_mem, hipStream_t s,
                  int stop_blocks = -1, float* x_out = nullptr, const unsigned char* pixels_u8 = nullptr);
int decoder_impl(dod_handle* h, const void* mem_op, int B, int N, const DecWS& ws, float* det, hipStream_t s, bool l0_only = false);

}
```

dinov2_od_amd/csrc/dod_pack.hip:

```cpp
#include "dod_internal.h"

#include <cstdlib>

using namespace dod;

namespace {

struct Packer {
  dod_handle* h; hipStream_t s; std::vector<void*> tmp; int rc = 0;
  Packer(dod_handle* h_, hipStream_t s_) : h(h_), s(s_) {}
  Packer(const Packer&) = delete;
  ~Packer() {
    if (tmp.empty()) return;
    (void)hipStreamSynchronize(s);
    for (void* t : tmp) (void)hipFree(t);
  }
  template <typename T> T* alloc(size_t n, bool temp = false) {
    void* p = nullptr;
    if (rc) return nullptr;
    hipError_t me = hipMalloc(&p, n * sizeof(T) ? n * sizeof(T) : 4);
    if (me != hipSuccess) { rc = fail(h, DOD_ERR_HIP, "hipMalloc of %zu bytes failed: %s", n * sizeof(T), hipGetErrorString(me)); return nullptr; }
    (temp ? tmp : h->owned).push_back(p);
    return (T*)p;
  }
  const WRef* find(const std::string& k) { auto it = h->w.find(k); return it == h->w.end() ? nullptr : &it->second; }
  const WRef* need(const std::string& k, std::initializer_list<int64_t> shape) {
    const WRef* r = find(k);
    if (!r) { if (!rc) rc = fail(h, DOD_ERR_MISSING, "missing weight '%s'", k.c_str()); return nullptr; }
    if (r->shape != std::vector<int64_t>(shape)) {
      if (!rc) { std::string got; for (auto d : r->shape) got += std::to_string(d) + ","; rc = fail(h, DOD_ERR_INVALID, "weight '%s' has shape [%s] (unexpected)", k.c_str(), got.c_str()); }
      return nullptr;
    }
    return r;
  }
  float* copy(const std::string& k, std::initializer_list<int64_t> shape) {
    const WRef* r = need(k, shape); if (!r) return nullptr;
    float* d = alloc<float>(r->numel()); if (!d) return nullptr;
    hipError_t ce = hipMemcpyAsync(d, r->ptr, r->numel() * 4, hipMemcpyDeviceToDevice, s);
    if (ce != hipSuccess && !rc) rc = fail(h, DOD_ERR_HIP, "copy of '%s' failed: %s", k.c_str(), hipGetErrorString(ce));
    return d;
  }
  const float* eff_weight(const std::string& prefix, int out_f, int in_f) {
    if (find(prefix + ".linear.weight")) {
      const WRef* W = need(prefix + ".linear.weight", {out_f, in_f});
      const WRef* A = find(prefix + ".lora_A.weight");
      const WRef* Bm = find(prefix + ".lora_B.weight");
      if (!W) return nullptr;
      if (!A || !Bm) { rc = fail(h, DOD_ERR_MISSING, "missing lora_A/lora_B for '%s'", prefix.c_str()); return nullptr; }
      const int r = (int)A->shape[0];
      if (A->shape != std::vector<int64_t>{r, in_f} || Bm->shape != std::vector<int64_t>{out_f, r}) { rc = fail(h, DOD_ERR_INVALID, "bad LoRA shapes for '%s'", prefix.c_str()); return nullptr; }
      float* m = alloc<float>((size_t)out_f * in_f, true); if (!m) return nullptr;
      if (launch_lora_merge(W->ptr, A->ptr, Bm->ptr, h->cfg.lora_alpha, out_f, in_f, r, m, s) && !rc) rc = fail(h, DOD_ERR_HIP, "lora merge launch failed: %s", hipGetErrorString(hipGetLastError()));
      return m;
    }
    const WRef* W = need(prefix + ".weight", {out_f, in_f});
    return W ? W->ptr : nullptr;
  }
  float* eff_bias(const std::string& prefix, int out_f) {
    if (find(prefix + ".linear.bias")) return copy(prefix + ".linear.bias", {out_f});
    return copy(prefix + ".bias", {out_f});
  }
  bf16_t* split_w(const float* src, int rows, int cols) {
    if (!src || !(is_bf16(h) || is_x3(h)) || cols % 64) return nullptr;
    bf16_t* b = alloc<bf16_t>((size_t)rows * 3 * cols); if (!b) return nullptr;
    if (launch_split3(src, cols, b, rows, cols, 1, s)) { if (!rc) rc = fail(h, DOD_ERR_HIP, "split3 launch failed"); return nullptr; }
    return b;
  }
  bf16_t* pair_w(const float* src, int rows, int cols) {
    if (!src || cols % 32) return nullptr;
    bf16_t* b = alloc<bf16_t>((size_t)rows * 2 * cols); if (!b) return nullptr;
    if (launch_split2(src, cols, b, rows, cols, s)) { if (!rc) rc = fail(h, DOD_ERR_HIP, "split2 launch failed"); return nullptr; }
    return b;
  }
  void* pack_operand(const float* src, int rows, int cols, int cols_pad, bool force_f32 = false) {
    if (!src) return nullptr;
    const bool bf = is_bf16(h) && !force_f32;
    float* f = alloc<float>((size_t)rows * cols_pad, bf); if (!f) return nullptr;
    if (launch_copy2d(src, cols, f, cols_pad, rows, cols, cols_pad, s)) { if (!rc) rc = fail(h, DOD_ERR_HIP, "copy2d launch failed"); return nullptr; }
    if (!bf) return f;
    bf16_t* b = alloc<bf16_t>((size_t)rows * cols_pad); if (!b) return nullptr;
    if (launch_cast_bf16(f, b, (size_t)rows * cols_pad, s)) { if (!rc) rc = fail(h, DOD_ERR_HIP, "cast launch failed"); return nullptr; }
    return b;
  }
  PackedLinear pack_linear(const float* src, int rows, int cols, float* bias, const float* csum = nullptr, bool fp8_ok = true) {
    const dod_config& c = h->cfg;
    PackedLinear p; p.bias = bias; p.csum = csum;
    if (is_h2(h)) {
      if (!src || cols % 32) return p;
      unsigned char* b = alloc<unsigned char>((size_t)rows * 3 * cols); unsigned char* ex = alloc<unsigned char>((size_t)rows);
      if (!b || !ex) return p;
      if (launch_split_h2(src, cols, b, rows, cols, ex, s)) { if (!rc) rc = fail(h, DOD_ERR_HIP, "split_h2 launch failed"); return p; }
      p.W = b; p.wexp = ex;
    } else if (is_x3(h)) p.W = pair_w(src, rows, cols);
    else if (is_fp8(h) && fp8_ok) {
      if (!src) return p;
      unsigned char* q = alloc<unsigned char>((size_t)rows * cols);
      if (c.hidden % 256 == 0 && (!c.swiglu || c.ffn_hidden % 256 == 0)) {
        unsigned char* bs = alloc<unsigned char>((size_t)rows * (cols >> 5));
        if (!q || !bs) return p;
        if (launch_quant_mx_fp8(src, 0, cols, rows, cols, q, cols, bs, s)) { if (!rc) rc = fail(h, DOD_ERR_HIP, "fp8 block-scaled weight quantisation launch failed"); return p; }
        p.W = q; p.wbs = bs;
      } else {
        float* sc = alloc<float>(rows);
        if (!q || !sc) return p;
        if (launch_quant_rows_fp8(src, 0, cols, rows, cols, q, cols, sc, s)) { if (!rc) rc = fail(h, DOD_ERR_HIP, "fp8 weight quantisation launch failed"); return p; }
        p.W = q; p.wscale = sc;
      }
    } else p.W = pack_operand(src, rows, cols, cols);
    return p;
  }
  float* fold_ln(const float* w, int rows, const float* gamma, const float* beta, float* bias) {
    const int D = h->cfg.hidden;
    float* wf = alloc<float>((size_t)rows * D, true);
    if (!w || !wf || !gamma || !beta || !bias) return nullptr;
    if (launch_ln_fold(w, rows, D, gamma, beta, bias, wf, bias, s)) { if (!rc) rc = fail(h, DOD_ERR_HIP, "LayerNorm fold launch failed"); return nullptr; }
    return wf;
  }
  float* col_sums(const float* wf, int rows) {
    float* cs = alloc<float>((size_t)rows);
    if (!wf || !cs) return nullptr;
    if (launch_rowsum(wf, rows, h->cfg.hidden, (is_bf16(h) && !is_x3(h)) ? 1 : 0, cs, s)) { if (!rc) rc = fail(h, DOD_ERR_HIP, "row sum launch failed"); return nullptr; }
    return cs;
  }
};

int widen_bf16_weights(Packer& P) {
  dod_handle* h = P.h;
  std::map<const void*, float*> widened;
  for (auto& kv : h->w) {
    WRef& r = kv.second;
    if (r.dtype == DOD_F32) { r.ptr = (const float*)r.raw; continue; }
    auto it = widened.find(r.raw);
    if (it == widened.end()) {
      float* f = P.alloc<float>(r.numel(), true);
      if (!f || launch_widen_bf16((const bf16_t*)r.raw, f, r.numel(), P.s)) return P.rc ? P.rc : fail(h, DOD_ERR_HIP, "widening of a bf16 weight failed");
      it = widened.emplace(r.raw, f).first;
    }
    r.ptr = it->second;
  }
  return DOD_OK;
}

int pack_backbone(Packer& P) {
  dod_handle* h = P.h; hipStream_t s = P.s;
  const dod_config& c = h->cfg;
  const int D = c.hidden, F = c.ffn_hidden, G = c.pos_grid, p = c.patch;
  const std::string bb = "backbone.dino.", e = bb + "embeddings.";
  h->cls = P.copy(e + "cls_token", {1, 1, D});
  h->pos = P.copy(e + "position_embeddings", {1, (int64_t)G * G + 1, D});
  h->bpatch = P.copy(e + "patch_embeddings.projection.bias", {D});
  {
    const WRef* W = P.need(e + "patch_embeddings.projection.weight", {D, 3, p, p});
    const int K = 3 * p * p;
    h->Kp = is_bf16(h) ? (K + 63) / 64 * 64 : K;
    if (W) h->Wpatch = P.pack_operand(W->ptr, D, K, h->Kp);
    h->Wpe = nullptr;
    if (W && (is_bf16(h) || is_x3(h)) && (p == 14 || p == 16) && D % 4 == 0 && dod_option(DOD_OPT_NO_FUSED_PATCH) <= 0) {
      bf16_t* wp = P.alloc<bf16_t>((size_t)D * 3 * (p / 2) * 32 * (is_x3(h) ? 2 : 1));
      if (wp && !launch_patch_pack(W->ptr, D, p, wp, is_x3(h) ? 1 : 0, s)) h->Wpe = wp;
    }
    if (W && is_x3(h)) {
      h->Kp2 = (K + 31) / 32 * 32;
      float* padded = P.alloc<float>((size_t)D * h->Kp2, true);
      if (padded && !launch_copy2d(W->ptr, K, padded, h->Kp2, D, K, h->Kp2, s)) h->Wpatch2 = P.pair_w(padded, D, h->Kp2);
    }
  }
  static const bool fold_env = [] { const char* v = getenv("DINODET_LN_FOLD"); return !(v && v[0] == '0'); }();
  const int fold_opt = dod_option(DOD_OPT_LN_FOLD);
  const bool fold = (fold_opt >= 0 ? fold_opt != 0 : fold_env) && ln_foldable(h);
  h->L.resize(c.layers);
  for (int i = 0; i < c.layers && !P.rc; ++i) {
    BLayer& L = h->L[i];
    const std::string lp = bb + "encoder.layer." + std::to_string(i) + ".";
    L.ln1w = P.copy(lp + "norm1.weight", {D}); L.ln1b = P.copy(lp + "norm1.bias", {D});
    L.ln2w = P.copy(lp + "norm2.weight", {D}); L.ln2b = P.copy(lp + "norm2.bias", {D});
    L.ls1 = P.copy(lp + "layer_scale1.lambda1", {D}); L.ls2 = P.copy(lp + "layer_scale2.lambda1", {D});
    L.fold = fold;
    float* cat = P.alloc<float>((size_t)3 * D * D, true);
    float* bqkv = P.alloc<float>((size_t)3 * D);
    const char* names[3] = {"query", "key", "value"};
    for (int t = 0; t < 3 && !P.rc; ++t) {
      const std::string q = lp + "attention.attention." + names[t];
      const float* w = P.eff_weight(q, D, D);
      float* b = P.eff_bias(q, D);
      if (!w || !b || !cat || !bqkv) break;
      HIPCHK(h, hipMemcpyAsync(cat + (size_t)t * D * D, w, (size_t)D * D * 4, hipMemcpyDeviceToDevice, s));
      HIPCHK(h, hipMemcpyAsync(bqkv + (size_t)t * D, b, (size_t)D * 4, hipMemcpyDeviceToDevice, s));
    }
    if (P.rc) break;
    float* cqkv = nullptr;
    if (fold) {
      float* cf = P.fold_ln(cat, 3 * D, L.ln1w, L.ln1b, bqkv);
      if (cf) { cat = cf; cqkv = P.col_sums(cat, 3 * D); }
      if (!cf || !cqkv) { if (!P.rc) P.rc = fail(h, DOD_ERR_HIP, "LayerNorm fold failed"); break; }
    }
    L.qkv = P.pack_linear(cat, 3 * D, D, bqkv, cqkv);
    const float* wo = P.eff_weight(lp + "attention.output.dense", D, D);
    L.o = P.pack_linear(wo, D, D, nullptr);
    L.o.bias = P.eff_bias(lp + "attention.output.dense", D);
    float* c1 = nullptr;
    if (c.swiglu) {
      const float* w_in = P.eff_weight(lp + "mlp.weights_in", 2 * F, D);
      float* b1 = P.eff_bias(lp + "mlp.weights_in", 2 * F);
      static const bool glu_off = DOD_TUNE_ENV("DINODET_NO_FUSED_GLU") != nullptr;
      const bool glu_ok = is_x3(h) ? (F % 32 == 0) : is_bf16(h);
      if (fold) w_in = P.fold_ln(w_in, 2 * F, L.ln2w, L.ln2b, b1);
      if (w_in && b1 && glu_ok && !glu_off) {
        float* wi = P.alloc<float>((size_t)2 * F * D, true);
        float* bi = P.alloc<float>((size_t)2 * F);
        if (wi && bi && !launch_interleave_halves(w_in, wi, F, D, s) && !launch_interleave_halves(b1, bi, F, 1, s)) { w_in = wi; b1 = bi; L.glu = true; }
      }
      if (fold) c1 = P.col_sums(w_in, 2 * F);
      L.fc1 = P.pack_linear(w_in, 2 * F, D, b1, c1);
      L.fc2 = P.pack_linear(P.eff_weight(lp + "mlp.weights_out", D, F), D, F, nullptr);
      L.fc2.bias = P.eff_bias(lp + "mlp.weights_out", D);
    } else {
      const float* w1 = P.eff_weight(lp + "mlp.fc1", F, D);
      float* b1 = P.eff_bias(lp + "mlp.fc1", F);
      if (fold) { w1 = P.fold_ln(w1, F, L.ln2w, L.ln2b, b1); c1 = P.col_sums(w1, F); }
      L.fc1 = P.pack_linear(w1, F, D, b1, c1);
      L.fc2 = P.pack_linear(P.eff_weight(lp + "mlp.fc2", D, F), D, F, nullptr, nullptr, false);
      L.fc2.bias = P.eff_bias(lp + "mlp.fc2", D);
    }
  }
  if (!P.rc) for (auto& L : h->L) if (L.fold && (!L.qkv.csum || !L.fc1.csum || !L.fc1.W)) { P.rc = fail(h, DOD_ERR_HIP, "LayerNorm fold failed"); break; }
  if (P.rc) return P.rc;
  h->lnfw = P.copy(bb + "layernorm.weight", {D}); h->lnfb = P.copy(bb + "layernorm.bias", {D});
  if (c.target_dim) {
    const WRef* W = P.need("backbone.projection.weight", {c.target_dim, D});
    if (W) h->Wproj = is_x3(h) ? (void*)P.pair_w(W->ptr, c.target_dim, D) : P.pack_operand(W->ptr, c.target_dim, D, D);
    h->bproj = P.copy("backbone.projection.bias", {c.target_dim});
  }
  return DOD_OK;
}

int pack_decoder(Packer& P) {
  dod_handle* h = P.h; hipStream_t s = P.s;
  const dod_config& c = h->cfg;
  const int Dd = c.dec_hidden, Q = c.num_queries, Hd = c.dec_heads, Pn = c.n_points, Fd = c.dim_feedforward, C = c.num_classes;
  const std::string dp = "decoder.";
  h->query = P.copy(dp + "query_embed.weight", {Q, Dd});
  h->cls_w = P.copy(dp + "class_embed.weight", {C, Dd}); h->cls_b = P.copy(dp + "class_embed.bias", {C});
  h->bb0_w = P.copy(dp + "bbox_embed.mlp.0.weight", {Dd / 2, Dd}); h->bb0_b = P.copy(dp + "bbox_embed.mlp.0.bias", {Dd / 2});
  h->bb0_w3 = P.split_w(h->bb0_w, Dd / 2, Dd);
  h->bb2_w = P.copy(dp + "bbox_embed.mlp.2.weight", {4, Dd / 2}); h->bb2_b = P.copy(dp + "bbox_embed.mlp.2.bias", {4});
  h->ncat = 2 + 3 * Hd * Pn;
  h->DL.resize(c.dec_layers);
  for (int j = 0; j < c.dec_layers && !P.rc; ++j) {
    DLayer& L = h->DL[j];
    const std::string lp = dp + "decoder.layers." + std::to_string(j) + ".";
    L.in_w = P.copy(lp + "self_attn.in_proj_weight", {3 * Dd, Dd}); L.in_b = P.copy(lp + "self_attn.in_proj_bias", {3 * Dd});
    L.out_w = P.copy(lp + "self_attn.out_proj.weight", {Dd, Dd}); L.out_b = P.copy(lp + "self_attn.out_proj.bias", {Dd});
    L.n1w = P.copy(lp + "norm1.weight", {Dd}); L.n1b = P.copy(lp + "norm1.bias", {Dd});
    L.n2w = P.copy(lp + "norm2.weight", {Dd}); L.n2b = P.copy(lp + "norm2.bias", {Dd});
    L.n3w = P.copy(lp + "norm3.weight", {Dd}); L.n3b = P.copy(lp + "norm3.bias", {Dd});
    L.l1w = P.copy(lp + "linear1.weight", {Fd, Dd}); L.l1b = P.copy(lp + "linear1.bias", {Fd});
    L.l2w = P.copy(lp + "linear2.weight", {Dd, Fd}); L.l2b = P.copy(lp + "linear2.bias", {Dd});
    L.in_w3 = P.split_w(L.in_w, 3 * Dd, Dd); L.out_w3 = P.split_w(L.out_w, Dd, Dd);
    L.l1w3 = P.split_w(L.l1w, Fd, Dd); L.l2w3 = P.split_w(L.l2w, Dd, Fd);
    if (c.use_deformable) {
      const WRef* rw = P.need(lp + "reference_points_proj.weight", {2, Dd});
      const WRef* rb = P.need(lp + "reference_points_proj.bias", {2});
      const WRef* ow = P.need(lp + "cross_attn.sampling_offsets.weight", {(int64_t)Hd * Pn * 2, Dd});
      const WRef* ob = P.need(lp + "cross_attn.sampling_offsets.bias", {(int64_t)Hd * Pn * 2});
      const WRef* aw = P.need(lp + "cross_attn.attention_weights.weight", {(int64_t)Hd * Pn, Dd});
      const WRef* ab = P.need(lp + "cross_attn.attention_weights.bias", {(int64_t)Hd * Pn});
      L.cat_w = P.alloc<float>((size_t)h->ncat * Dd); L.cat_b = P.alloc<float>(h->ncat);
      if (P.rc || !rw || !rb || !ow || !ob || !aw || !ab || !L.cat_w || !L.cat_b) break;
      HIPCHK(h, hipMemcpyAsync(L.cat_w, rw->ptr, (size_t)2 * Dd * 4, hipMemcpyDeviceToDevice, s));
      HIPCHK(h, hipMemcpyAsync(L.cat_w + (size_t)2 * Dd, ow->ptr, (size_t)Hd * Pn * 2 * Dd * 4, hipMemcpyDeviceToDevice, s));
      HIPCHK(h, hipMemcpyAsync(L.cat_w + (size_t)(2 + Hd * Pn * 2) * Dd, aw->ptr, (size_t)Hd * Pn * Dd * 4, hipMemcpyDeviceToDevice, s));
      HIPCHK(h, hipMemcpyAsync(L.cat_b, rb->ptr, 2 * 4, hipMemcpyDeviceToDevice, s));
      HIPCHK(h, hipMemcpyAsync(L.cat_b + 2, ob->ptr, (size_t)Hd * Pn * 2 * 4, hipMemcpyDeviceToDevice, s));
      HIPCHK(h, hipMemcpyAsync(L.cat_b + 2 + Hd * Pn * 2, ab->ptr, (size_t)Hd * Pn * 4, hipMemcpyDeviceToDevice, s));
      L.op_w = P.copy(lp + "cross_attn.output_proj.weight", {Dd, Dd}); L.op_b = P.copy(lp + "cross_attn.output_proj.bias", {Dd});
      L.op_w3 = P.split_w(L.op_w, Dd, Dd);
      const WRef* vw = P.need(lp + "cross_attn.value_proj.weight", {Dd, Dd});
      const WRef* vb = P.need(lp + "cross_attn.value_proj.bias", {Dd});
      if (!vw || !vb) break;
      for (int k = 0; k < j; ++k) {
        const std::string kp = dp + "decoder.layers." + std::to_string(k) + ".";
        if (h->w[kp + "cross_attn.value_proj.weight"].ptr == vw->ptr && h->w[kp + "cross_attn.value_proj.bias"].ptr == vb->ptr) { L.vp_alias = h->DL[k].vp_alias >= 0 ? h->DL[k].vp_alias : k; break; }
      }
      if (L.vp_alias < 0) {
        L.vp_w = P.pack_operand(vw->ptr, Dd, Dd, Dd); L.vp_b = P.copy(lp + "cross_attn.value_proj.bias", {Dd});
        if (is_x3(h)) L.vp_w2 = P.pair_w(vw->ptr, Dd, Dd);
      }
    } else {
      const WRef* iw = P.need(lp + "multihead_attn.in_proj_weight", {3 * Dd, Dd});
      const WRef* ib = P.need(lp + "multihead_attn.in_proj_bias", {3 * Dd});
      if (!iw || !ib) break;
      L.ca_q_w = (float*)P.pack_operand(iw->ptr, Dd, Dd, Dd, true);
      L.ca_kv_w = P.pack_operand(iw->ptr + (size_t)Dd * Dd, 2 * Dd, Dd, Dd);
      if (is_x3(h)) L.ca_kv_w2 = P.pair_w(iw->ptr + (size_t)Dd * Dd, 2 * Dd, Dd);
      L.ca_q_b = P.alloc<float>(Dd); L.ca_kv_b = P.alloc<float>(2 * Dd);
      if (P.rc) break;
      HIPCHK(h, hipMemcpyAsync(L.ca_q_b, ib->ptr, (size_t)Dd * 4, hipMemcpyDeviceToDevice, s));
      HIPCHK(h, hipMemcpyAsync(L.ca_kv_b, ib->ptr + Dd, (size_t)2 * Dd * 4, hipMemcpyDeviceToDevice, s));
      L.ca_out_w = P.copy(lp + "multihead_attn.out_proj.weight", {Dd, Dd}); L.ca_out_b = P.copy(lp + "multihead_attn.out_proj.bias", {Dd});
      L.ca_q_w3 = P.split_w(L.ca_q_w, Dd, Dd); L.ca_out_w3 = P.split_w(L.ca_out_w, Dd, Dd);
    }
  }
  return DOD_OK;
}

}

__global__ void widen_bf16_kernel(const bf16_t* __restrict__ in, float* __restrict__ out, size_t n) {
  for (size_t i = (size_t)blockIdx.x * blockDim.x + threadIdx.x; i < n; i += (size_t)gridDim.x * blockDim.x) out[i] = bf2f(in[i]);
}
int dod::launch_widen_bf16(const bf16_t* in, float* out, size_t n, hipStream_t s) {
  const int blocks = (int)((n + 255) / 256 < 4096 ? (n + 255) / 256 : 4096);
  hipLaunchKernelGGL(widen_bf16_kernel, dim3(blocks), dim3(256), 0, s, in, out, n);
  return hipGetLastError() == hipSuccess ? 0 : 3;
}

int dod::finalize_impl(dod_handle* h, hipStream_t s) {
  for (void* p : h->owned) (void)hipFree(p);
  h->owned.clear(); h->L.clear(); h->DL.clear(); h->finalized = false;
  h->pos_H = h->pos_W = -1; h->pos_hw = nullptr; h->pos_cache.clear();
  Packer P(h, s);
  int rc = widen_bf16_weights(P); if (rc) return rc;
  h->has_bb = h->has_dec = false;
  for (auto& kv : h->w) {
    if (kv.first.rfind("backbone.", 0) == 0) h->has_bb = true;
    if (kv.first.rfind("decoder.", 0) == 0) h->has_dec = true;
  }
  if (!h->has_bb && !h->has_dec) return fail(h, DOD_ERR_MISSING, "no 'backbone.*' or 'decoder.*' weights were registered");
  if (h->has_bb) { rc = pack_backbone(P); if (rc) return rc; }
  if (h->has_dec) { rc = pack_decoder(P); if (rc) return rc; }
  hipError_t se = hipStreamSynchronize(s);
  if (P.rc) return P.rc;
  if (se != hipSuccess) return fail(h, DOD_ERR_HIP, "finalize: %s", hipGetErrorString(se));
  h->finalized = true;
  return DOD_OK;
}
```

dinov2_od_amd/csrc/patch_embed.hip:

```cpp
#include "dod_common.h"

#define PE_M 128
#define PE_N 128
#define PE_PLANE (128 * 64)

__device__ __forceinline__ int pe_swz(int row, int chunk) { return chunk ^ (((row >> 3) & 1) << 1); }

template <bool X3, bool U8, int P>
__global__ __launch_bounds__(256) void patch_embed_kernel(const void* __restrict__ img_, const bf16_t* __restrict__ Wp, int ldw,
                                                          const float* __restrict__ bias, const float* __restrict__ pos,
                                                          float* __restrict__ out, int B, int H, int W, int gh, int gw, int D) {
  constexpr int p = P;
  extern __shared__ __attribute__((aligned(16))) char smem[];
  constexpr int NPL = X3 ? 4 : 2;
  constexpr int STAGE = NPL * PE_PLANE;
  const int tid = threadIdx.x, lane = tid & 63, wid = tid >> 6;
  const int wu = __builtin_amdgcn_readfirstlane(wid);
  const int wm = wu >> 1, wn = wu & 1;
  const int Np = gh * gw, Mtot = B * Np;
  const int tiles_m = (Mtot + PE_M - 1) / PE_M;
  const int tiles_n = (D + PE_N - 1) / PE_N;
  const int xcd = blockIdx.x & 7, idx = blockIdx.x >> 3;
  const int tn = idx % tiles_n, tm = (idx / tiles_n) * 8 + xcd;
  if (tm >= tiles_m) return;
  const int m0 = tm * PE_M, n0 = tn * PE_N;
  const int nsteps = 3 * (p / 2), kp = nsteps * 32;

  constexpr int NP2 = P / 2;
  unsigned goff[NP2];
  int lofs[NP2];
  size_t cstride, rstride;
  if (U8) { cstride = 1; rstride = (size_t)W * 3; } else { cstride = (size_t)H * W; rstride = (size_t)W; }
#pragma unroll
  for (int i = 0; i < NP2; ++i) {
    const int e = tid + 256 * i;
    const int rr = e / (PE_M * NP2), rem_e = e - rr * (PE_M * NP2), pl = rem_e / NP2, j = 2 * (rem_e - pl * NP2);
    int m = m0 + pl; m = m < Mtot ? m : Mtot - 1;
    const int b = m / Np, rem = m - b * Np, py = rem / gw, px = rem - py * gw;
    if (U8) goff[i] = (unsigned)((((size_t)b * H + (size_t)py * p + rr) * W + (size_t)px * p + j) * 3);
    else goff[i] = (unsigned)((((size_t)b * 3) * H + (size_t)py * p + rr) * W + (size_t)px * p + j);
    const int kq = rr * 16 + j;
    lofs[i] = pl * 64 + pe_swz(pl, kq >> 3) * 16 + (kq & 7) * 2;
  }
  float pv0[P], pv1[P], pv2[P];
  uint4 wA0, wB0, wC0, wD0, wA1, wB1, wC1, wD1, wA2, wB2, wC2, wD2;
  const bf16_t* gWr;
  int wofs0, wofs1;
  {
    const int rl = tid >> 1, hf = tid & 1;
    int rr = n0 + rl; rr = rr < D ? rr : D - 1;
    gWr = Wp + (size_t)rr * ldw + hf * 16;
    wofs0 = rl * 64 + pe_swz(rl, 2 * hf) * 16;
    wofs1 = rl * 64 + pe_swz(rl, 2 * hf + 1) * 16;
  }
#define PE_GLOAD(PV, WA, WB, WC, WD, s_)                                                                    \
  {                                                                                                         \
    const int c_ = (s_) / (p / 2), si_ = (s_) - c_ * (p / 2);                                               \
    const size_t o_ = c_ * cstride + (size_t)(2 * si_) * rstride;                                           \
    _Pragma("unroll") for (int i = 0; i < NP2; ++i) {                                                       \
      if (U8) {                                                                                             \
        const unsigned char* q_ = (const unsigned char*)img_ + goff[i] + o_;                                \
        PV[2 * i] = (float)q_[0] / 255.0f; PV[2 * i + 1] = (float)q_[3] / 255.0f;              \
      } else {                                                                                              \
        const float2 v_ = *reinterpret_cast<const float2*>((const float*)img_ + goff[i] + o_);              \
        PV[2 * i] = v_.x; PV[2 * i + 1] = v_.y;                                                             \
      }                                                                                                     \
    }                                                                                                       \
    const uint4* wp_ = reinterpret_cast<const uint4*>(gWr + (s_) * 32);                                     \
    WA = wp_[0]; WB = wp_[1];                                                                               \
    if (X3) { const uint4* wq_ = reinterpret_cast<const uint4*>(gWr + kp + (s_) * 32); WC = wq_[0]; WD = wq_[1]; } \
  }
#define PE_SWRITE(PV, WA, WB, WC, WD, stage_)                                                               \
  {                                                                                                         \
    char* sa_ = smem + (stage_) * STAGE;                                                                    \
    _Pragma("unroll") for (int i = 0; i < NP2; ++i) {                                                       \
      const unsigned hi_ = pack2bf(PV[2 * i], PV[2 * i + 1]);                                               \
      *reinterpret_cast<unsigned*>(sa_ + lofs[i]) = hi_;                                                    \
      if (X3) *reinterpret_cast<unsigned*>(sa_ + PE_PLANE + lofs[i]) =                                      \
          pack2bf(PV[2 * i] - __uint_as_float(hi_ << 16), PV[2 * i + 1] - __uint_as_float(hi_ & 0xffff0000u)); \
    }                                                                                                       \
    char* sw_ = sa_ + (X3 ? 2 : 1) * PE_PLANE;                                                              \
    *reinterpret_cast<uint4*>(sw_ + wofs0) = WA;                                                            \
    *reinterpret_cast<uint4*>(sw_ + wofs1) = WB;                                                            \
    if (X3) { *reinterpret_cast<uint4*>(sw_ + PE_PLANE + wofs0) = WC; *reinterpret_cast<uint4*>(sw_ + PE_PLANE + wofs1) = WD; } \
  }

  f32x4 acc[4][4];
#pragma unroll
  for (int i = 0; i < 4; ++i)
#pragma unroll
    for (int j = 0; j < 4; ++j) acc[i][j] = f32x4{0.f, 0.f, 0.f, 0.f};
  const int l15 = lane & 15, l4 = lane >> 4;
  int offA[4], offW[4];
#pragma unroll
  for (int i = 0; i < 4; ++i) { const int row = wm * 64 + i * 16 + l15; offA[i] = row * 64 + pe_swz(row, l4) * 16; }
#pragma unroll
  for (int j = 0; j < 4; ++j) { const int row = wn * 64 + j * 16 + l15; offW[j] = (X3 ? 2 : 1) * PE_PLANE + row * 64 + pe_swz(row, l4) * 16; }

  for (int i = tid; i < 2 * STAGE / 16; i += 256) {
    const int st_ = i / (STAGE / 16), o_ = (i - st_ * (STAGE / 16)) * 16;
    if (o_ < (X3 ? 2 : 1) * PE_PLANE) *reinterpret_cast<uint4*>(smem + st_ * STAGE + o_) = make_uint4(0u, 0u, 0u, 0u);
  }
  __syncthreads();
  auto compute = [&](int stage) {
    const char* st = smem + stage * STAGE;
    bf16x8 wh[4], wl[4];
#pragma unroll
    for (int j = 0; j < 4; ++j) {
      wh[j] = *reinterpret_cast<const bf16x8*>(st + offW[j]);
      if (X3) wl[j] = *reinterpret_cast<const bf16x8*>(st + offW[j] + PE_PLANE);
    }
#pragma unroll
    for (int i = 0; i < 4; ++i) {
      const bf16x8 ah = *reinterpret_cast<const bf16x8*>(st + offA[i]);
      bf16x8 al;
      if (X3) al = *reinterpret_cast<const bf16x8*>(st + offA[i] + PE_PLANE);
#pragma unroll
      for (int j = 0; j < 4; ++j) {
        if (X3) {
          acc[i][j] = __builtin_amdgcn_mfma_f32_16x16x32_bf16(wl[j], ah, acc[i][j], 0, 0, 0);
          acc[i][j] = __builtin_amdgcn_mfma_f32_16x16x32_bf16(wh[j], al, acc[i][j], 0, 0, 0);
        }
        acc[i][j] = __builtin_amdgcn_mfma_f32_16x16x32_bf16(wh[j], ah, acc[i][j], 0, 0, 0);
      }
    }
  };
  PE_GLOAD(pv0, wA0, wB0, wC0, wD0, 0)
  PE_GLOAD(pv1, wA1, wB1, wC1, wD1, 1)
  PE_GLOAD(pv2, wA2, wB2, wC2, wD2, 2)
  PE_SWRITE(pv0, wA0, wB0, wC0, wD0, 0)
  __syncthreads();
  for (int s = 0; s < nsteps; s += 3) {
    if (s + 3 < nsteps) PE_GLOAD(pv0, wA0, wB0, wC0, wD0, s + 3)
    compute(s & 1);
    PE_SWRITE(pv1, wA1, wB1, wC1, wD1, (s + 1) & 1)
    __syncthreads();
    if (s + 4 < nsteps) PE_GLOAD(pv1, wA1, wB1, wC1, wD1, s + 4)
    compute((s + 1) & 1);
    PE_SWRITE(pv2, wA2, wB2, wC2, wD2, (s + 2) & 1)
    __syncthreads();
    if (s + 5 < nsteps) PE_GLOAD(pv2, wA2, wB2, wC2, wD2, s + 5)
    compute((s + 2) & 1);
    if (s + 3 < nsteps) PE_SWRITE(pv0, wA0, wB0, wC0, wD0, (s + 3) & 1)
    __syncthreads();
  }
  const int N = Np + 1;
#pragma unroll
  for (int i = 0; i < 4; ++i) {
    const int m = m0 + wm * 64 + i * 16 + l15;
    if (m >= Mtot) continue;
    const int b = m / Np, rem = m - b * Np;
    float* orow = out + ((size_t)b * N + 1 + rem) * D;
    const float* prow = pos + (size_t)(1 + rem) * D;
#pragma unroll
    for (int j = 0; j < 4; ++j) {
      const int n = n0 + wn * 64 + j * 16 + 4 * l4;
      if (n >= D) continue;
      const float4 bv = *reinterpret_cast<const float4*>(bias + n), pp = *reinterpret_cast<const float4*>(prow + n);
      const f32x4 a = acc[i][j];
      *reinterpret_cast<float4*>(orow + n) = make_float4(a[0] + bv.x + pp.x, a[1] + bv.y + pp.y, a[2] + bv.z + pp.z, a[3] + bv.w + pp.w);
    }
  }
}

__global__ void patch_pack_kernel(const float* __restrict__ W, int D, int p, bf16_t* __restrict__ out, int x3) {
  const int kp = 3 * (p / 2) * 32;
  const size_t total = (size_t)D * kp;
  for (size_t idx = (size_t)blockIdx.x * blockDim.x + threadIdx.x; idx < total; idx += (size_t)gridDim.x * blockDim.x) {
    const int n = (int)(idx / kp), k = (int)(idx - (size_t)n * kp);
    const int s = k >> 5, kk = k & 31, r = kk >> 4, j = kk & 15;
    const int c = s / (p / 2), si = s - c * (p / 2);
    const float v = j < p ? W[(((size_t)n * 3 + c) * p + (2 * si + r)) * p + j] : 0.f;
    const bf16_t hi = f2bf(v);
    if (x3) {
      out[(size_t)n * 2 * kp + k] = hi;
      out[(size_t)n * 2 * kp + kp + k] = f2bf(v - bf2f(hi));
    } else {
      out[idx] = hi;
    }
  }
}

int launch_patch_pack(const float* W, int D, int p, bf16_t* out, int x3, hipStream_t s) {
  if (p < 2 || p > 16 || (p & 1)) return 2;
  const size_t total = (size_t)D * 3 * (p / 2) * 32;
  hipLaunchKernelGGL(patch_pack_kernel, dim3((unsigned)((total + 255) / 256 < 4096 ? (total + 255) / 256 : 4096)), dim3(256), 0, s, W, D, p, out, x3);
  return hipGetLastError() == hipSuccess ? 0 : 3;
}

int launch_patch_embed(const void* img, int u8, int B, int H, int W, int p, const bf16_t* Wp, int x3, const float* bias, const float* pos,
                       float* out, int D, hipStream_t s) {
  if ((p != 14 && p != 16) || D % 4 != 0 || B <= 0 || (!u8 && (W & 1))) return 2;
  const int gh = H / p, gw = W / p;
  if (gh <= 0 || gw <= 0) return 2;
  if ((size_t)B * 3 * H * W >= 0xffffffffull) return 2;
  const int kp = 3 * (p / 2) * 32, ldw = x3 ? 2 * kp : kp;
  const int tiles = ((((B * gh * gw) + PE_M - 1) / PE_M + 7) / 8 * 8) * ((D + PE_N - 1) / PE_N);
  const int lds = 2 * (x3 ? 4 : 2) * PE_PLANE;
#define PE_LAUNCH(X3_, U8_, P_) hipLaunchKernelGGL((patch_embed_kernel<X3_, U8_, P_>), dim3(tiles), dim3(256), lds, s, img, Wp, ldw, bias, pos, out, B, H, W, gh, gw, D)
  if (p == 14) {
    if (x3) { if (u8) PE_LAUNCH(true, true, 14); else PE_LAUNCH(true, false, 14); }
    else { if (u8) PE_LAUNCH(false, true, 14); else PE_LAUNCH(false, false, 14); }
  } else {
    if (x3) { if (u8) PE_LAUNCH(true, true, 16); else PE_LAUNCH(true, false, 16); }
    else { if (u8) PE_LAUNCH(false, true, 16); else PE_LAUNCH(false, false, 16); }
  }
#undef PE_LAUNCH
  gemm_form_launched(FORM_PATCH_FUSED);
  return hipGetLastError() == hipSuccess ? 0 : 3;
}
```

dinov2_od_amd/csrc/rowops.hip:

```cpp
#include "dod_common.h"

#define LN_MAXC 8
enum { LN_F32 = 1, LN_BF16 = 2, LN_PAIR = 4, LN_H2 = 8, LN_FP8 = 16, LN_S3 = 32, LN_FP8MX = 64 };
template <int NCH, bool EXACT, int OUT>
__global__ __launch_bounds__(256) void layernorm_kernel(const float* __restrict__ x, const float* __restrict__ add,
                                                        const float* __restrict__ gamma, const float* __restrict__ beta,
                                                        float eps, int rows, int D, LnOut o) {
  const int lane = threadIdx.x & 63;
  const int row = blockIdx.x * 4 + (threadIdx.x >> 6);
  if (row >= rows) return;
  const int nc = D >> 2;
  const float4* xr = reinterpret_cast<const float4*>(x + (size_t)row * D);
  const float4* ar = add ? reinterpret_cast<const float4*>(add + (size_t)row * D) : nullptr;
  float4 v[NCH];
  float s = 0.f;
#pragma unroll
  for (int i = 0; i < NCH; ++i) {
    const int c = lane + 64 * i;
    if (EXACT || c < nc) v[i] = xr[c];
  }
  if (ar) {
#pragma unroll
    for (int i = 0; i < NCH; ++i) {
      const int c = lane + 64 * i;
      if (EXACT || c < nc) { const float4 a = ar[c]; v[i].x += a.x; v[i].y += a.y; v[i].z += a.z; v[i].w += a.w; }
    }
  }
#pragma unroll
  for (int i = 0; i < NCH; ++i) {
    const int c = lane + 64 * i;
    if (EXACT || c < nc) s += (v[i].x + v[i].y) + (v[i].z + v[i].w);
  }
  const float mean = wave_sum(s) / (float)D;
  float q = 0.f;
#pragma unroll
  for (int i = 0; i < NCH; ++i) {
    const int c = lane + 64 * i;
    if (EXACT || c < nc) {
      const float a = v[i].x - mean, b = v[i].y - mean, cc = v[i].z - mean, d = v[i].w - mean;
      q += (a * a + b * b) + (cc * cc + d * d);
    }
  }
  const float rstd = 1.0f / sqrtf(wave_sum(q) / (float)D + eps);
#pragma unroll
  for (int i = 0; i < NCH; ++i) {
    const int c = lane + 64 * i;
    if (EXACT || c < nc) {
      const float4 g = reinterpret_cast<const float4*>(gamma)[c];
      const float4 b = reinterpret_cast<const float4*>(beta)[c];
      v[i].x = (v[i].x - mean) * rstd * g.x + b.x;
      v[i].y = (v[i].y - mean) * rstd * g.y + b.y;
      v[i].z = (v[i].z - mean) * rstd * g.z + b.z;
      v[i].w = (v[i].w - mean) * rstd * g.w + b.w;
    }
  }
  if (OUT & LN_FP8MX) {
#pragma unroll
    for (int i = 0; i < NCH; ++i) {
      const int c = lane + 64 * i;
      const bool ok = EXACT || c < nc;
      float amax = ok ? fmaxf(fmaxf(fabsf(v[i].x), fabsf(v[i].y)), fmaxf(fabsf(v[i].z), fabsf(v[i].w))) : 0.f;
      amax = fmaxf(amax, __shfl_xor(amax, 1, 64));
      amax = fmaxf(amax, __shfl_xor(amax, 2, 64));
      amax = fmaxf(amax, __shfl_xor(amax, 4, 64));
      const unsigned eb = mx_ebyte(amax);
      const float inv = mx_inv_scale(eb);
      if (ok) {
        reinterpret_cast<unsigned*>(o.fp8 + (size_t)row * D)[c] = pack4_fp8(v[i].x * inv, v[i].y * inv, v[i].z * inv, v[i].w * inv);
        if ((lane & 7) == 0) o.bs[(size_t)row * (D >> 5) + mx_scale_off(D, c >> 3)] = (unsigned char)eb;
      }
    }
    return;
  }
  if (OUT & LN_FP8) {
    float amax = 0.f;
#pragma unroll
    for (int i = 0; i < NCH; ++i) {
      const int c = lane + 64 * i;
      if (EXACT || c < nc) amax = fmaxf(amax, fmaxf(fmaxf(fabsf(v[i].x), fabsf(v[i].y)), fmaxf(fabsf(v[i].z), fabsf(v[i].w))));
    }
    amax = wave_max(amax);
    const float sc = amax > 0.f ? amax / 448.0f : 1.0f;
    const float inv = 1.0f / sc;
    if (lane == 0) o.scale[row] = sc;
#pragma unroll
    for (int i = 0; i < NCH; ++i) {
      const int c = lane + 64 * i;
      if (EXACT || c < nc) reinterpret_cast<unsigned*>(o.fp8 + (size_t)row * D)[c] = pack4_fp8(v[i].x * inv, v[i].y * inv, v[i].z * inv, v[i].w * inv);
    }
    return;
  }
#pragma unroll
  for (int i = 0; i < NCH; ++i) {
    const int c = lane + 64 * i;
    if (EXACT || c < nc) {
      const float4 w = v[i];
      if (OUT & LN_F32) reinterpret_cast<float4*>(o.f32 + (size_t)row * D)[c] = w;
      if (OUT & LN_H2) {
        uint2 f16; unsigned hi8, lo8;
        h2_quad(w, 1.0f, f16, hi8, lo8);
        char* ob = reinterpret_cast<char*>(o.split) + (size_t)row * 4 * D;
        reinterpret_cast<uint2*>(ob)[c] = f16;
        char* p8 = ob + h2_off8(D, 4 * c);
        *reinterpret_cast<unsigned*>(p8) = hi8;
        *reinterpret_cast<unsigned*>(p8 + 16) = lo8;
      }
      if (OUT & LN_PAIR) {
        uint2 hi, lo;
        hi.x = pack2bf(w.x, w.y);
        hi.y = pack2bf(w.z, w.w);
        lo.x = pack2bf(w.x - __uint_as_float(hi.x << 16), w.y - __uint_as_float(hi.x & 0xffff0000u));
        lo.y = pack2bf(w.z - __uint_as_float(hi.y << 16), w.w - __uint_as_float(hi.y & 0xffff0000u));
        bf16_t* ob = o.split + (size_t)row * 2 * D;
        reinterpret_cast<uint2*>(ob)[c] = hi;
        reinterpret_cast<uint2*>(ob + D)[c] = lo;
      }
      if (OUT & LN_S3) {
        uint2 hi, lo;
        hi.x = pack2bf(w.x, w.y);
        hi.y = pack2bf(w.z, w.w);
        lo.x = pack2bf(w.x - __uint_as_float(hi.x << 16), w.y - __uint_as_float(hi.x & 0xffff0000u));
        lo.y = pack2bf(w.z - __uint_as_float(hi.y << 16), w.w - __uint_as_float(hi.y & 0xffff0000u));
        bf16_t* ob = o.a3 + (size_t)row * 3 * D;
        reinterpret_cast<uint2*>(ob)[c] = hi;
        reinterpret_cast<uint2*>(ob + D)[c] = hi;
        reinterpret_cast<uint2*>(ob + 2 * D)[c] = lo;
      }
      if (OUT & LN_BF16) {
        uint2 p;
        p.x = pack2bf(w.x, w.y);
        p.y = pack2bf(w.z, w.w);
        reinterpret_cast<uint2*>(o.bf16 + (size_t)row * D)[c] = p;
      }
    }
  }
}

template <int OUT>
static void ln_dispatch(const float* x, const float* add, const float* gamma, const float* beta, float eps, int rows, int D,
                        const LnOut& o, hipStream_t s) {
  const dim3 grid((rows + 3) / 4), block(256);
  const int nc = D >> 2, nch = (nc + 63) / 64;
  const bool exact = nc == 64 * nch;
#define LN_GO(N, E) hipLaunchKernelGGL((layernorm_kernel<N, E, OUT>), grid, block, 0, s, x, add, gamma, beta, eps, rows, D, o)
  if (exact) {
    switch (nch) {
      case 1: LN_GO(1, true); return;
      case 2: LN_GO(2, true); return;
      case 3: LN_GO(3, true); return;
      case 4: LN_GO(4, true); return;
      case 6: LN_GO(6, true); return;
      default: break;
    }
  }
  if (nch <= 1) LN_GO(1, false);
  else if (nch <= 2) LN_GO(2, false);
  else if (nch <= 4) LN_GO(4, false);
  else LN_GO(LN_MAXC, false);
#undef LN_GO
}

int launch_layernorm(const float* x, const float* add, const float* gamma, const float* beta, float eps, int rows, int D, const LnOut& o,
                     hipStream_t s, int split_h2) {
  if (rows <= 0) return 1;
  if (D % 4 != 0 || D > 256 * LN_MAXC) return 2;
  if (split_h2 && (!o.split || D % 32 != 0)) return 2;
  if (o.bs) {
    if (!o.fp8 || o.scale || o.f32 || o.bf16 || o.split || o.a3 || D % 64 != 0) return 2;
    ln_dispatch<LN_FP8MX>(x, add, gamma, beta, eps, rows, D, o, s);
    return hipGetLastError() == hipSuccess ? 0 : 3;
  }
  if ((o.fp8 == nullptr) != (o.scale == nullptr)) return 2;
  if (o.a3) {
    if (!o.f32 || o.bf16 || o.fp8 || o.split) return 2;
    ln_dispatch<LN_F32 | LN_S3>(x, add, gamma, beta, eps, rows, D, o, s);
  } else if (o.fp8) ln_dispatch<LN_FP8>(x, add, gamma, beta, eps, rows, D, o, s);
  else if (o.split && (o.f32 || o.bf16)) return 2;
  else if (o.split) { if (split_h2) ln_dispatch<LN_H2>(x, add, gamma, beta, eps, rows, D, o, s); else ln_dispatch<LN_PAIR>(x, add, gamma, beta, eps, rows, D, o, s); }
  else if (o.f32 && o.bf16) ln_dispatch<LN_F32 | LN_BF16>(x, add, gamma, beta, eps, rows, D, o, s);
  else if (o.bf16) ln_dispatch<LN_BF16>(x, add, gamma, beta, eps, rows, D, o, s);
  else if (o.f32) ln_dispatch<LN_F32>(x, add, gamma, beta, eps, rows, D, o, s);
  else return 2;
  return hipGetLastError() == hipSuccess ? 0 : 3;
}

template <int NCH, bool EXACT, int KIND>
__global__ __launch_bounds__(256) void rowstats_kernel(const float* __restrict__ x, int rows, int D, float eps, void* __restrict__ op, float2* __restrict__ stats) {
  const int lane = threadIdx.x & 63;
  const int row = blockIdx.x * 4 + (threadIdx.x >> 6);
  if (row >= rows) return;
  const int nc = D >> 2;
  const float4* xr = reinterpret_cast<const float4*>(x + (size_t)row * D);
  float4 v[NCH];
  float s = 0.f;
#pragma unroll
  for (int i = 0; i < NCH; ++i) {
    const int c = lane + 64 * i;
    if (EXACT || c < nc) { v[i] = xr[c]; s += (v[i].x + v[i].y) + (v[i].z + v[i].w); }
  }
  const float mean = wave_sum(s) / (float)D;
  float q = 0.f;
#pragma unroll
  for (int i = 0; i < NCH; ++i) {
    const int c = lane + 64 * i;
    if (EXACT || c < nc) {
      const float a = v[i].x - mean, b = v[i].y - mean, cc = v[i].z - mean, d = v[i].w - mean;
      q += (a * a + b * b) + (cc * cc + d * d);
    }
  }
  const float rstd = 1.0f / sqrtf(wave_sum(q) / (float)D + eps);
  if (lane == 0) stats[row] = make_float2(mean, rstd);
#pragma unroll
  for (int i = 0; i < NCH; ++i) {
    const int c = lane + 64 * i;
    if (!(EXACT || c < nc)) continue;
    const float4 w = v[i];
    if (KIND == LNOP_H2) {
      uint2 f16; unsigned hi8, lo8;
      h2_quad(w, 1.0f, f16, hi8, lo8);
      char* ob = reinterpret_cast<char*>(op) + (size_t)row * 4 * D;
      reinterpret_cast<uint2*>(ob)[c] = f16;
      char* p8 = ob + h2_off8(D, 4 * c);
      *reinterpret_cast<unsigned*>(p8) = hi8;
      *reinterpret_cast<unsigned*>(p8 + 16) = lo8;
    } else {
      uint2 hi;
      hi.x = pack2bf(w.x, w.y);
      hi.y = pack2bf(w.z, w.w);
      bf16_t* ob = reinterpret_cast<bf16_t*>(op) + (size_t)row * (KIND == LNOP_PAIR ? 2 : 1) * D;
      reinterpret_cast<uint2*>(ob)[c] = hi;
      if (KIND == LNOP_PAIR) {
        uint2 lo;
        lo.x = pack2bf(w.x - __uint_as_float(hi.x << 16), w.y - __uint_as_float(hi.x & 0xffff0000u));
        lo.y = pack2bf(w.z - __uint_as_float(hi.y << 16), w.w - __uint_as_float(hi.y & 0xffff0000u));
        reinterpret_cast<uint2*>(ob + D)[c] = lo;
      }
    }
  }
}

template <int KIND>
static void rowstats_dispatch(const float* x, int rows, int D, float eps, void* op, float2* stats, hipStream_t s) {
  const dim3 grid((rows + 3) / 4), block(256);
  const int nc = D >> 2, nch = (nc + 63) / 64;
  const bool exact = nc == 64 * nch;
#define RS_GO(N, E) hipLaunchKernelGGL((rowstats_kernel<N, E, KIND>), grid, block, 0, s, x, rows, D, eps, op, stats)
  if (exact && nch == 3) RS_GO(3, true);
  else if (exact && nch == 4) RS_GO(4, true);
  else if (exact && nch == 6) RS_GO(6, true);
  else if (nch <= 2) RS_GO(2, false);
  else if (nch <= 4) RS_GO(4, false);
  else RS_GO(LN_MAXC, false);
#undef RS_GO
}

int launch_rowstats(const float* x, int rows, int D, float eps, void* op, int op_kind, float2* stats, hipStream_t s) {
  if (rows <= 0) return 1;
  if (D % 4 != 0 || D > 256 * LN_MAXC || !op || !stats) return 2;
  if (op_kind == LNOP_H2) { if (D % 32) return 2; rowstats_dispatch<LNOP_H2>(x, rows, D, eps, op, stats, s); }
  else if (op_kind == LNOP_PAIR) rowstats_dispatch<LNOP_PAIR>(x, rows, D, eps, op, stats, s);
  else if (op_kind == LNOP_BF16) rowstats_dispatch<LNOP_BF16>(x, rows, D, eps, op, stats, s);
  else return 2;
  return hipGetLastError() == hipSuccess ? 0 : 3;
}

__global__ __launch_bounds__(256) void ln_finalize_kernel(const float2* __restrict__ part, int npart, int rows, int D, float eps, float2* __restrict__ stats) {
  const int row = blockIdx.x * 256 + threadIdx.x;
  if (row >= rows) return;
  const float2* p = part + (size_t)row * npart;
  float S = 0.f, Q = 0.f;
  for (int g = 0; g < npart; ++g) { S += p[g].x; Q += p[g].y; }
  const float k = stats[row].x, dm = S / (float)D;
  const float var = fmaxf(Q / (float)D - dm * dm, 0.f);
  stats[row] = make_float2(k + dm, 1.0f / sqrtf(var + eps));
}

int launch_ln_finalize(const float2* part, int npart, int rows, int D, float eps, float2* stats, hipStream_t s) {
  if (rows <= 0) return 1;
  if (npart != (D + 127) / 128 || !part || !stats) return 2;
  hipLaunchKernelGGL(ln_finalize_kernel, dim3((rows + 255) / 256), dim3(256), 0, s, part, npart, rows, D, eps, stats);
  return hipGetLastError() == hipSuccess ? 0 : 3;
}

__global__ __launch_bounds__(256) void ln_fold_kernel(const float* __restrict__ W, int rows, int cols, const float* __restrict__ gamma, const float* __restrict__ beta,
                                                      const float* __restrict__ bias_in, float* __restrict__ Wout, float* __restrict__ bias_out) {
  const int lane = threadIdx.x & 63;
  const int n = blockIdx.x * 4 + (threadIdx.x >> 6);
  if (n >= rows) return;
  float acc = 0.f;
  for (int k = lane; k < cols; k += 64) {
    const float w = W[(size_t)n * cols + k];
    acc = fmaf(w, beta[k], acc);
    Wout[(size_t)n * cols + k] = w * gamma[k];
  }
  acc = wave_sum(acc);
  if (lane == 0) bias_out[n] = bias_in[n] + acc;
}

int launch_ln_fold(const float* W, int rows, int cols, const float* gamma, const float* beta, const float* bias_in, float* Wout, float* bias_out, hipStream_t s) {
  if (rows <= 0 || cols <= 0) return 1;
  hipLaunchKernelGGL(ln_fold_kernel, dim3((rows + 3) / 4), dim3(256), 0, s, W, rows, cols, gamma, beta, bias_in, Wout, bias_out);
  return hipGetLastError() == hipSuccess ? 0 : 3;
}

__global__ __launch_bounds__(256) void rowsum_kernel(const float* __restrict__ W, int rows, int cols, int round_bf16, float* __restrict__ c) {
  const int lane = threadIdx.x & 63;
  const int n = blockIdx.x * 4 + (threadIdx.x >> 6);
  if (n >= rows) return;
  float acc = 0.f;
  for (int k = lane; k < cols; k += 64) {
    const float w = W[(size_t)n * cols + k];
    acc += round_bf16 ? bf2f(f2bf(w)) : w;
  }
  acc = wave_sum(acc);
  if (lane == 0) c[n] = acc;
}

int launch_rowsum(const float* W, int rows, int cols, int round_bf16, float* c, hipStream_t s) {
  if (rows <= 0 || cols <= 0) return 1;
  hipLaunchKernelGGL(rowsum_kernel, dim3((rows + 3) / 4), dim3(256), 0, s, W, rows, cols, round_bf16, c);
  return hipGetLastError() == hipSuccess ? 0 : 3;
}

__global__ void im2col_kernel(const float* __restrict__ img, int B, int H, int W, int p, int gh, int gw, int Kp,
                              float* __restrict__ out_f32, bf16_t* __restrict__ out_bf16) {
  const size_t total = (size_t)B * gh * gw * Kp;
  const int K = 3 * p * p;
  for (size_t idx = (size_t)blockIdx.x * blockDim.x + threadIdx.x; idx < total; idx += (size_t)gridDim.x * blockDim.x) {
    const int k = (int)(idx % Kp);
    const size_t m = idx / Kp;
    float v = 0.f;
    if (k < K) {
      const int c = k / (p * p), r = k - c * p * p, i = r / p, j = r - i * p;
      const int px = (int)(m % gw);
      const size_t t = m / gw;
      const int py = (int)(t % gh);
      const int b = (int)(t / gh);
      v = img[(((size_t)b * 3 + c) * H + (py * p + i)) * W + (px * p + j)];
    }
    if (out_f32) out_f32[idx] = v; else out_bf16[idx] = f2bf(v);
  }
}

int launch_im2col(const float* img, int B, int H, int W, int patch, int Kp, float* out_f32, bf16_t* out_bf16, hipStream_t s) {
  const int gh = H / patch, gw = W / patch;
  if (B <= 0 || gh <= 0 || gw <= 0 || Kp < 3 * patch * patch) return 2;
  const size_t total = (size_t)B * gh * gw * Kp;
  const int blocks = (int)((total + 255) / 256 < 8192 ? (total + 255) / 256 : 8192);
  hipLaunchKernelGGL(im2col_kernel, dim3(blocks), dim3(256), 0, s, img, B, H, W, patch, gh, gw, Kp, out_f32, out_bf16);
  return hipGetLastError() == hipSuccess ? 0 : 3;
}

__global__ void cls_row_kernel(const float* __restrict__ cls, const float* __restrict__ pos, float* __restrict__ x,
                               int B, int N, int D) {
  const int i = blockIdx.x * blockDim.x + threadIdx.x;
  if (i >= B * D) return;
  const int b = i / D, d = i - b * D;
  x[(size_t)b * N * D + d] = cls[d] + pos[d];
}
int launch_cls_row(const float* cls, const float* pos, float* x, int B, int N, int D, hipStream_t s) {
  hipLaunchKernelGGL(cls_row_kernel, dim3((B * D + 255) / 256), dim3(256), 0, s, cls, pos, x, B, N, D);
  return hipGetLastError() == hipSuccess ? 0 : 3;
}

__device__ __forceinline__ float cubic1(float x, float A) { return ((A + 2.f) * x - (A + 3.f)) * x * x + 1.f; }
__device__ __forceinline__ float cubic2(float x, float A) { return ((A * x - 5.f * A) * x + 8.f * A) * x - 4.f * A; }
__global__ void pos_resize_kernel(const float* __restrict__ pin, int G, int gh, int gw, int D, float* __restrict__ pout) {
  const size_t total = (size_t)(gh * gw + 1) * D;
  const size_t idx = (size_t)blockIdx.x * blockDim.x + threadIdx.x;
  if (idx >= total) return;
  const int d = (int)(idx % D);
  const int tok = (int)(idx / D);
  if (tok == 0) { pout[idx] = pin[d]; return; }
  const int oy = (tok - 1) / gw, ox = (tok - 1) - oy * gw;
  const float A = -0.75f;
  const float sy = (float)G / (float)gh, sx = (float)G / (float)gw;
  const float ry = sy * ((float)oy + 0.5f) - 0.5f, rx = sx * ((float)ox + 0.5f) - 0.5f;
  const float fy = floorf(ry), fx = floorf(rx);
  const int iy = (int)fy, ix = (int)fx;
  const float ty = ry - fy, tx = rx - fx;
  const float cy[4] = {cubic2(ty + 1.f, A), cubic1(ty, A), cubic1(1.f - ty, A), cubic2(2.f - ty, A)};
  const float cx[4] = {cubic2(tx + 1.f, A), cubic1(tx, A), cubic1(1.f - tx, A), cubic2(2.f - tx, A)};
  float acc = 0.f;
#pragma unroll
  for (int a = 0; a < 4; ++a) {
    int yy = iy - 1 + a; yy = yy < 0 ? 0 : (yy > G - 1 ? G - 1 : yy);
    float rowv = 0.f;
#pragma unroll
    for (int b = 0; b < 4; ++b) {
      int xx = ix - 1 + b; xx = xx < 0 ? 0 : (xx > G - 1 ? G - 1 : xx);
      rowv += pin[(size_t)(1 + yy * G + xx) * D + d] * cx[b];
    }
    acc += rowv * cy[a];
  }
  pout[idx] = acc;
}
int launch_pos_resize(const float* pos_in, int G, int gh, int gw, int D, float* pos_out, hipStream_t s) {
  const size_t total = (size_t)(gh * gw + 1) * D;
  hipLaunchKernelGGL(pos_resize_kernel, dim3((unsigned)((total + 255) / 256)), dim3(256), 0, s, pos_in, G, gh, gw, D, pos_out);
  return hipGetLastError() == hipSuccess ? 0 : 3;
}

__global__ void swiglu_kernel(const float* __restrict__ in_f32, const bf16_t* __restrict__ in_bf16, int rows, int Fh,
                              float* __restrict__ out_f32, bf16_t* __restrict__ out_bf16) {
  const size_t total = (size_t)rows * Fh;
  for (size_t idx = (size_t)blockIdx.x * blockDim.x + threadIdx.x; idx < total; idx += (size_t)gridDim.x * blockDim.x) {
    const size_t r = idx / Fh;
    const int c = (int)(idx - r * Fh);
    float a, b;
    if (in_f32) { a = in_f32[r * 2 * Fh + c]; b = in_f32[r * 2 * Fh + Fh + c]; }
    else { a = bf2f(in_bf16[r * 2 * Fh + c]); b = bf2f(in_bf16[r * 2 * Fh + Fh + c]); }
    const float v = a / (1.0f + expf(-a)) * b;
    if (out_f32) out_f32[idx] = v; else out_bf16[idx] = f2bf(v);
  }
}
int launch_swiglu(const float* in_f32, const bf16_t* in_bf16, int rows, int Fh, float* out_f32, bf16_t* out_bf16, hipStream_t s) {
  const size_t total = (size_t)rows * Fh;
  const int blocks = (int)((total + 255) / 256 < 8192 ? (total + 255) / 256 : 8192);
  hipLaunchKernelGGL(swiglu_kernel, dim3(blocks), dim3(256), 0, s, in_f32, in_bf16, rows, Fh, out_f32, out_bf16);
  return hipGetLastError() == hipSuccess ? 0 : 3;
}

__global__ void cast_bf16_kernel(const float* __restrict__ in, bf16_t* __restrict__ out, size_t n) {
  for (size_t i = (size_t)blockIdx.x * blockDim.x + threadIdx.x; i < n; i += (size_t)gridDim.x * blockDim.x) out[i] = f2bf(in[i]);
}
int launch_cast_bf16(const float* in, bf16_t* out, size_t n, hipStream_t s) {
  const int blocks = (int)((n + 255) / 256 < 4096 ? (n + 255) / 256 : 4096);
  hipLaunchKernelGGL(cast_bf16_kernel, dim3(blocks), dim3(256), 0, s, in, out, n);
  return hipGetLastError() == hipSuccess ? 0 : 3;
}

__global__ void copy2d_kernel(const float* __restrict__ src, int ld_src, float* __restrict__ dst, int ld_dst, int rows,
                              int cols, int cols_pad) {
  const size_t total = (size_t)rows * cols_pad;
  for (size_t i = (size_t)blockIdx.x * blockDim.x + threadIdx.x; i < total; i += (size_t)gridDim.x * blockDim.x) {
    const size_t r = i / cols_pad;
    const int c = (int)(i - r * cols_pad);
    dst[r * ld_dst + c] = c < cols ? src[r * ld_src + c] : 0.f;
  }
}
int launch_copy2d(const float* src, int ld_src, float* dst, int ld_dst, int rows, int cols, int cols_pad, hipStream_t s) {
  const size_t total = (size_t)rows * cols_pad;
  if (total == 0) return 0;
  const int blocks = (int)((total + 255) / 256 < 4096 ? (total + 255) / 256 : 4096);
  hipLaunchKernelGGL(copy2d_kernel, dim3(blocks), dim3(256), 0, s, src, ld_src, dst, ld_dst, rows, cols, cols_pad);
  return hipGetLastError() == hipSuccess ? 0 : 3;
}

__global__ void lora_merge_kernel(const float* __restrict__ W, const float* __restrict__ A, const float* __restrict__ Bm,
                                  float alpha, int out_f, int in_f, int r, float* __restrict__ dst) {
  const size_t total = (size_t)out_f * in_f;
  for (size_t i = (size_t)blockIdx.x * blockDim.x + threadIdx.x; i < total; i += (size_t)gridDim.x * blockDim.x) {
    const size_t o = i / in_f;
    const int c = (int)(i - o * in_f);
    float acc = 0.f;
    for (int t = 0; t < r; ++t) acc += Bm[o * r + t] * A[(size_t)t * in_f + c];
    dst[i] = W[i] + alpha * acc;
  }
}
int launch_lora_merge(const float* W, const float* A, const float* Bm, float alpha, int out_f, int in_f, int r, float* dst, hipStream_t s) {
  const size_t total = (size_t)out_f * in_f;
  const int blocks = (int)((total + 255) / 256 < 4096 ? (total + 255) / 256 : 4096);
  hipLaunchKernelGGL(lora_merge_kernel, dim3(blocks), dim3(256), 0, s, W, A, Bm, alpha, out_f, in_f, r, dst);
  return hipGetLastError() == hipSuccess ? 0 : 3;
}

__global__ void bcast_rows_kernel(const float* __restrict__ src, float* __restrict__ dst, int B, size_t n) {
  const size_t total = (size_t)B * n;
  for (size_t i = (size_t)blockIdx.x * blockDim.x + threadIdx.x; i < total; i += (size_t)gridDim.x * blockDim.x) dst[i] = src[i % n];
}
int launch_bcast_rows(const float* src, float* dst, int B, int rows, int D, hipStream_t s) {
  const size_t n = (size_t)rows * D, total = n * B;
  const int blocks = (int)((total + 255) / 256 < 4096 ? (total + 255) / 256 : 4096);
  hipLaunchKernelGGL(bcast_rows_kernel, dim3(blocks), dim3(256), 0, s, src, dst, B, n);
  return hipGetLastError() == hipSuccess ? 0 : 3;
}

__global__ void split3_kernel(const float* __restrict__ in, int ld_in, bf16_t* __restrict__ out, int rows, int K, int mode) {
  const size_t total = (size_t)rows * K;
  for (size_t i = (size_t)blockIdx.x * blockDim.x + threadIdx.x; i < total; i += (size_t)gridDim.x * blockDim.x) {
    const size_t r = i / K;
    const int c = (int)(i - r * K);
    const float x = in[r * ld_in + c];
    const bf16_t hi = f2bf(x);
    const bf16_t lo = f2bf(x - bf2f(hi));
    bf16_t* o = out + r * 3 * (size_t)K + c;
    o[0] = hi;
    o[K] = mode ? lo : hi;
    o[2 * (size_t)K] = mode ? hi : lo;
  }
}
__global__ void split2_kernel(const float* __restrict__ in, int ld_in, bf16_t* __restrict__ out, int rows, int K) {
  const size_t total = (size_t)rows * K;
  for (size_t i = (size_t)blockIdx.x * blockDim.x + threadIdx.x; i < total; i += (size_t)gridDim.x * blockDim.x) {
    const size_t r = i / K;
    const int c = (int)(i - r * K);
    const float x = in[r * ld_in + c];
    const bf16_t hi = f2bf(x);
    bf16_t* o = out + r * 2 * (size_t)K + c;
    o[0] = hi;
    o[K] = f2bf(x - bf2f(hi));
  }
}
int launch_split2(const float* in, int ld_in, bf16_t* out, int rows, int K, hipStream_t s) {
  const size_t total = (size_t)rows * K;
  if (total == 0) return 0;
  const int blocks = (int)((total + 255) / 256 < 4096 ? (total + 255) / 256 : 4096);
  hipLaunchKernelGGL(split2_kernel, dim3(blocks), dim3(256), 0, s, in, ld_in, out, rows, K);
  return hipGetLastError() == hipSuccess ? 0 : 3;
}
__global__ __launch_bounds__(256) void split_h2_kernel(const float* __restrict__ in, int ld_in, char* __restrict__ out, int rows, int K,
                                                       unsigned char* __restrict__ wexp) {
  const int lane = threadIdx.x & 63;
  const int row = blockIdx.x * 4 + (threadIdx.x >> 6);
  if (row >= rows) return;
  const float* xr = in + (size_t)row * ld_in;
  float shi = 1.0f;
  if (wexp) {
    float amax = 0.f;
    for (int c = lane; c < K; c += 64) amax = fmaxf(amax, fabsf((float)(_Float16)clampf_(xr[c], 65504.f)));
    amax = wave_max(amax);
    int e = 0;
    if (amax > 0.f) {
      int ex; const float m = frexpf(amax, &ex);
      e = (m <= 0.875f ? 9 : 8) - ex;
      e = e < -100 ? -100 : (e > 100 ? 100 : e);
    }
    shi = ldexpf(1.0f, e);
    if (lane == 0) wexp[row] = (unsigned char)(127 - e);
  }
  char* ob = out + (size_t)row * (wexp ? 3 : 4) * K;
  for (int c = lane * 4; c < K; c += 256) {
    const float4 v = make_float4(xr[c], xr[c + 1], xr[c + 2], xr[c + 3]);
    uint2 f16; unsigned hi8, lo8;
    h2_quad(v, shi, f16, hi8, lo8);
    *reinterpret_cast<uint2*>(ob + 2 * c) = f16;
    if (wexp) *reinterpret_cast<unsigned*>(ob + 2 * K + c) = lo8;
    else {
      char* p8 = ob + h2_off8(K, c);
      *reinterpret_cast<unsigned*>(p8) = hi8;
      *reinterpret_cast<unsigned*>(p8 + 16) = lo8;
    }
  }
}
int launch_split_h2(const float* in, int ld_in, void* out, int rows, int K, unsigned char* wexp, hipStream_t s) {
  if (rows <= 0) return 1;
  if (K % 32 != 0) return 2;
  hipLaunchKernelGGL(split_h2_kernel, dim3((rows + 3) / 4), dim3(256), 0, s, in, ld_in, (char*)out, rows, K, wexp);
  return hipGetLastError() == hipSuccess ? 0 : 3;
}

int launch_split3(const float* in, int ld_in, bf16_t* out, int rows, int K, int mode, hipStream_t s) {
  const size_t total = (size_t)rows * K;
  if (total == 0) return 0;
  const int blocks = (int)((total + 255) / 256 < 4096 ? (total + 255) / 256 : 4096);
  hipLaunchKernelGGL(split3_kernel, dim3(blocks), dim3(256), 0, s, in, ld_in, out, rows, K, mode);
  return hipGetLastError() == hipSuccess ? 0 : 3;
}

__global__ void interleave_halves_kernel(const float* __restrict__ src, float* __restrict__ dst, int F, int cols) {
  const size_t total = (size_t)2 * F * cols;
  for (size_t idx = (size_t)blockIdx.x * blockDim.x + threadIdx.x; idx < total; idx += (size_t)gridDim.x * blockDim.x) {
    const size_t r = idx / cols; const int c = (int)(idx - r * cols);
    const size_t sr = (r & 1) ? (size_t)F + (r >> 1) : (r >> 1);
    dst[idx] = src[sr * cols + c];
  }
}
int launch_interleave_halves(const float* src, float* dst, int F, int cols, hipStream_t s) {
  if (F <= 0 || cols <= 0) return 1;
  const size_t total = (size_t)2 * F * cols;
  hipLaunchKernelGGL(interleave_halves_kernel, dim3((unsigned)((total + 255) / 256 < 4096 ? (total + 255) / 256 : 4096)), dim3(256), 0, s, src, dst, F, cols);
  return hipGetLastError() == hipSuccess ? 0 : 3;
}
```

Before: 2575 images/s.

## Fuse first-block LayerNorm statistics and bf16 operand production into patch-embed epilogue

The patch-embed GEMM epilogue now also writes the bf16 LayerNorm operand and per-128-column partial sums and sums of squares, shifted by a precomputed per-token mean estimate. This removes the separate rowstats pass over the embedded activations before block 0. The CLS row gets a matching producer kernel. It also adds an optional 256-wide N tile with 512 threads, chosen by grid-size heuristics. The cost is a heavier epilogue, extra LDS reduction and a new cached shift table per position grid.

```diff
diff --git a/dinov2_od_amd/csrc/dod_api.hip b/dinov2_od_amd/csrc/dod_api.hip
--- a/dinov2_od_amd/csrc/dod_api.hip
+++ b/dinov2_od_amd/csrc/dod_api.hip
@@ -35,10 +35,10 @@
   return true;
 }
 
-static std::atomic<int> g_options[DOD_OPT_COUNT] = {{-1}, {-1}, {-1}, {-1}, {-1}, {-1}, {-1}, {-1}, {-1}, {-1}, {-1}};
+static std::atomic<int> g_options[DOD_OPT_COUNT] = {{-1}, {-1}, {-1}, {-1}, {-1}, {-1}, {-1}, {-1}, {-1}, {-1}, {-1}, {-1}};
 int dod_option(int which) { return which >= 0 && which < DOD_OPT_COUNT ? g_options[which].load() : -1; }
 static const char* const k_option_names[DOD_OPT_COUNT] = {"tailsplit", "dec_fused_split", "mha_chunk_images", "no_fused_patch", "ln_fold", "deterministic", "f32_ksplit",
-                                                       "attn_bwd_flash", "epi_regmath", "f32x3_tile", "attn_diet"};
+                                                       "attn_bwd_flash", "epi_regmath", "f32x3_tile", "attn_diet", "pe_producer"};
 
 static std::atomic<long> g_form_launches[FORM_COUNT];
 static const char* const k_form_names[FORM_COUNT] = {"bf16_128_r2", "bf16_128_r3", "bf16_m16", "k64", "ppm", "x3_16w", "x3_pp", "h2", "fp8_rows", "fp8mx_256x128",
@@ -59,6 +59,8 @@
   if (name && !strcmp(name, "f32_ksplits")) return gemm_f32_ksplit_count();
   if (name && !strcmp(name, "epi_regmath")) return gemm_epi_regmath_count();
   if (name && !strcmp(name, "attn_diet")) return attn_half_tile_count();
+  if (name && !strcmp(name, "rowstats_launches")) return rowstats_launch_count();
+  if (name && !strcmp(name, "pe_wide_launches")) return pe_wide_launch_count();
   if (name && !strcmp(name, "f32x3_launches")) return gemm_f32x3_count(0);
   if (name && !strcmp(name, "f32x3_wide_launches")) return gemm_f32x3_count(1);
   if (name && !strcmp(name, "optim_launches")) return optim_launch_count();
diff --git a/dinov2_od_amd/csrc/dod_common.h b/dinov2_od_amd/csrc/dod_common.h
--- a/dinov2_od_amd/csrc/dod_common.h
+++ b/dinov2_od_amd/csrc/dod_common.h
@@ -24,6 +24,7 @@
        DOD_OPT_EPI_REGMATH,
        DOD_OPT_F32X3_TILE,
        DOD_OPT_ATTN_DIET,
+       DOD_OPT_PE_PRODUCER,
        DOD_OPT_COUNT };
 int dod_option(int which);
 long gemm_tail_split_count();
@@ -32,6 +33,7 @@
 long gemm_rem_cut_count();
 long attn_half_tile_count();
 long gemm_epi_regmath_count();
+long rowstats_launch_count();
 enum { FORM_BF16_128_R2 = 0, FORM_BF16_128_R3, FORM_BF16_M16, FORM_K64, FORM_PPM, FORM_X3_16W, FORM_X3_PP, FORM_H2, FORM_FP8_ROWS, FORM_FP8MX_256X128,
        FORM_FP8MX2_256X128, FORM_FP8MX2_256X256, FORM_F32, FORM_PATCH_FUSED, FORM_COUNT };
 void gemm_form_launched(int form);
@@ -244,9 +246,19 @@
 
 int launch_im2col(const float* img, int B, int H, int W, int patch, int Kp, float* out_f32, bf16_t* out_bf16, hipStream_t s);
 int launch_patch_pack(const float* W, int D, int p, bf16_t* out, int x3, hipStream_t s);
+struct PeProd {
+  bf16_t* op;
+  float2* part;
+  float2* shift_out;
+  const float* kshift;
+  int tile;
+};
+long pe_wide_launch_count();
+bool pe_producer_pays(int B, int gh, int gw, int D);
 int launch_patch_embed(const void* img, int u8, int B, int H, int W, int p, const bf16_t* Wp, int x3, const float* bias, const float* pos,
-                       float* out, int D, hipStream_t s);
-int launch_cls_row(const float* cls, const float* pos, float* x, int B, int N, int D, hipStream_t s);
+                       float* out, int D, hipStream_t s, const PeProd* prod = nullptr);
+int launch_cls_row(const float* cls, const float* pos, float* x, int B, int N, int D, hipStream_t s, const PeProd* prod = nullptr);
+int launch_embed_shift(const float* cls, const float* bias, const float* pos, int N, int D, float* kshift, hipStream_t s);
 int launch_pos_resize(const float* pos_in, int G, int gh, int gw, int D, float* pos_out, hipStream_t s);
 int launch_interleave_halves(const float* src, float* dst, int F, int cols, hipStream_t s);
 int launch_swiglu(const float* in_f32, const bf16_t* in_bf16, int rows, int Fh, float* out_f32, bf16_t* out_bf16, hipStream_t s);
diff --git a/dinov2_od_amd/csrc/dod_forward.hip b/dinov2_od_amd/csrc/dod_forward.hip
--- a/dinov2_od_amd/csrc/dod_forward.hip
+++ b/dinov2_od_amd/csrc/dod_forward.hip
@@ -70,9 +70,19 @@
     HIPCHK(h, hipMalloc((void**)&buf, need * 4));
     h->owned.push_back(buf);
     KCHK(h, launch_pos_resize(h->pos, g.pos_grid, gh, gw, g.hidden, buf, s));
+    int rc = embed_shift_table(h, buf, gh * gw + 1, s); if (rc) return rc;
     it = h->pos_cache.emplace(key, buf).first;
   }
   h->pos_hw = it->second; h->pos_H = H; h->pos_W = W;
+  return DOD_OK;
+}
+
+int dod::embed_shift_table(dod_handle* h, const float* pos, int N, hipStream_t s) {
+  float* k = nullptr;
+  HIPCHK(h, hipMalloc((void**)&k, (size_t)N * 4));
+  h->owned.push_back(k);
+  KCHK(h, launch_embed_shift(h->cls, h->bpatch, pos, N, h->cfg.hidden, k, s));
+  h->shift_cache[pos] = k;
   return DOD_OK;
 }
 
@@ -266,10 +276,24 @@
   if (bf && D / g.heads != 64) return fail(h, DOD_ERR_INVALID, "bf16 attention kernel needs head_dim 64 (got %d)", D / g.heads);
   int rc = prepare_impl(h, H, W, s); if (rc) return rc;
   if (pixels_u8 && !h->Wpe) return fail(h, DOD_ERR_INVALID, "uint8 input needs the fused patch embed (bf16 / bf16x3 / fp8 precision, patch size 14 or 16)");
-  if (h->Wpe && (pixels_u8 || W % 2 == 0)) {
+  const bool x3 = is_x3(h);
+  const int nblocks = stop_blocks >= 0 ? (stop_blocks < g.layers ? stop_blocks : g.layers) : g.layers;
+  const bool fold = ln_foldable(h) && !h->L.empty() && h->L[0].fold;
+  if (fold && !(ws.lnp && ws.lns && ws.lns2)) return fail(h, DOD_ERR_STATE, "internal: the weights were packed with the LayerNorm folded but the workspace has no statistics buffers");
+  BlockRun run(h, ws, s, B, N, fold);
+  const bool fused_pe = h->Wpe && (pixels_u8 || W % 2 == 0);
+  const int pe_opt = dod_option(DOD_OPT_PE_PRODUCER);
+  PeProd prod{(bf16_t*)ws.y, ws.lnp, run.stat[0], nullptr, pe_opt == 2 ? 1 : (pe_opt == 3 ? 2 : 0)};
+  const bool pe_prod = fold && fused_pe && run.op_kind == LNOP_BF16 && (pe_opt > 0 || (pe_opt < 0 && pe_producer_pays(B, gh, gw, D)));
+  if (pe_prod) {
+    auto it = h->shift_cache.find(h->pos_hw);
+    if (it == h->shift_cache.end()) return fail(h, DOD_ERR_STATE, "internal: the position table has no shift table");
+    prod.kshift = it->second;
+  }
+  if (fused_pe) {
     ProfScope ps(h, s, PC_GEMM_BF16, 2.0 * B * Np * (double)D * 3.0 * p * p);
-    KCHK(h, launch_patch_embed(pixels_u8 ? (const void*)pixels_u8 : (const void*)pixels, pixels_u8 ? 1 : 0, B, H, W, p, h->Wpe, is_x3(h) ? 1 : 0,
-                               h->bpatch, h->pos_hw, ws.x, D, s));
+    KCHK(h, launch_patch_embed(pixels_u8 ? (const void*)pixels_u8 : (const void*)pixels, pixels_u8 ? 1 : 0, B, H, W, p, h->Wpe, x3 ? 1 : 0,
+                               h->bpatch, h->pos_hw, ws.x, D, s, pe_prod ? &prod : nullptr));
   } else if (is_x3(h) && h->Wpatch2 && (size_t)3 * D * 6 >= (size_t)h->Kp2 * 4) {
     const int K2 = h->Kp2;
     KCHK(h, launch_im2col(pixels, B, H, W, p, K2, (float*)ws.hbuf, nullptr, s));
@@ -284,15 +308,11 @@
     e.pos = h->pos_hw; e.rows_per_img = Np; e.out_rows_per_img = N;
     rc = linear(h, bf, ws.hbuf, h->Kp, h->Wpatch, h->Kp, B * Np, D, h->Kp, e, s); if (rc) return rc;
   }
-  KCHK(h, launch_cls_row(h->cls, h->pos_hw, ws.x, B, N, D, s));
+  KCHK(h, launch_cls_row(h->cls, h->pos_hw, ws.x, B, N, D, s, pe_prod ? &prod : nullptr));
   tap(h, 0, ws.x, false, (size_t)M * D, s);
   float* yf = bf ? nullptr : (float*)ws.y; bf16_t* yb = bf ? (bf16_t*)ws.y : nullptr;
-  const bool x3 = is_x3(h);
-  const int nblocks = stop_blocks >= 0 ? (stop_blocks < g.layers ? stop_blocks : g.layers) : g.layers;
-  const bool fold = ln_foldable(h) && !h->L.empty() && h->L[0].fold;
-  if (fold && !(ws.lnp && ws.lns && ws.lns2)) return fail(h, DOD_ERR_STATE, "internal: the weights were packed with the LayerNorm folded but the workspace has no statistics buffers");
-  BlockRun run(h, ws, s, B, N, fold);
-  if (fold && nblocks > 0) { ProfScope ps(h, s, PC_LAYERNORM, 0); KCHK(h, launch_rowstats(ws.x, M, D, g.ln_eps, ws.y, run.op_kind, run.stat[0], s)); }
+  if (pe_prod) run.fresh = true;
+  else if (fold && nblocks > 0) { ProfScope ps(h, s, PC_LAYERNORM, 0); KCHK(h, launch_rowstats(ws.x, M, D, g.ln_eps, ws.y, run.op_kind, run.stat[0], s)); }
   for (int i = 0; i < nblocks; ++i) {
     rc = run.block(h->L[i], i + 1 < g.layers); if (rc) return rc;
     tap(h, 1 + i, ws.x, false, (size_t)M * D, s);
diff --git a/dinov2_od_amd/csrc/dod_internal.h b/dinov2_od_amd/csrc/dod_internal.h
--- a/dinov2_od_amd/csrc/dod_internal.h
+++ b/dinov2_od_amd/csrc/dod_internal.h
@@ -57,6 +57,7 @@
   float *l0_tgt = nullptr, *l0_proj = nullptr;
   std::map<std::pair<int, int>, float*> pos_cache;
   int pos_H = -1, pos_W = -1; float* pos_hw = nullptr;
+  std::map<const float*, float*> shift_cache;
   std::map<int, float*> taps;
   bool prof_on = false;
   struct ProfRec { hipEvent_t a, b; int cls; double flops; };
@@ -125,6 +126,7 @@
 int finalize_impl(dod_handle* h, hipStream_t s);
 int launch_widen_bf16(const bf16_t* in, float* out, size_t n, hipStream_t s);
 int prepare_impl(dod_handle* h, int H, int W, hipStream_t s);
+int embed_shift_table(dod_handle* h, const float* pos, int N, hipStream_t s);
 int backbone_impl(dod_handle* h, const float* pixels, int B, int H, int W, const BbWS& ws, float* feat_f32, bool want_mem, hipStream_t s,
                   int stop_blocks = -1, float* x_out = nullptr, const unsigned char* pixels_u8 = nullptr);
 int decoder_impl(dod_handle* h, const void* mem_op, int B, int N, const DecWS& ws, float* det, hipStream_t s, bool l0_only = false);
diff --git a/dinov2_od_amd/csrc/dod_pack.hip b/dinov2_od_amd/csrc/dod_pack.hip
--- a/dinov2_od_amd/csrc/dod_pack.hip
+++ b/dinov2_od_amd/csrc/dod_pack.hip
@@ -318,7 +318,7 @@
 int dod::finalize_impl(dod_handle* h, hipStream_t s) {
   for (void* p : h->owned) (void)hipFree(p);
   h->owned.clear(); h->L.clear(); h->DL.clear(); h->finalized = false;
-  h->pos_H = h->pos_W = -1; h->pos_hw = nullptr; h->pos_cache.clear();
+  h->pos_H = h->pos_W = -1; h->pos_hw = nullptr; h->pos_cache.clear(); h->shift_cache.clear();
   Packer P(h, s);
   int rc = widen_bf16_weights(P); if (rc) return rc;
   h->has_bb = h->has_dec = false;
@@ -328,6 +328,7 @@
   }
   if (!h->has_bb && !h->has_dec) return fail(h, DOD_ERR_MISSING, "no 'backbone.*' or 'decoder.*' weights were registered");
   if (h->has_bb) { rc = pack_backbone(P); if (rc) return rc; }
+  if (h->has_bb && !P.rc && h->pos && h->cls && h->bpatch) { rc = embed_shift_table(h, h->pos, h->cfg.pos_grid * h->cfg.pos_grid + 1, s); if (rc) return rc; }
   if (h->has_dec) { rc = pack_decoder(P); if (rc) return rc; }
   hipError_t se = hipStreamSynchronize(s);
   if (P.rc) return P.rc;
diff --git a/dinov2_od_amd/csrc/patch_embed.hip b/dinov2_od_amd/csrc/patch_embed.hip
--- a/dinov2_od_amd/csrc/patch_embed.hip
+++ b/dinov2_od_amd/csrc/patch_embed.hip
@@ -1,22 +1,37 @@
 #include "dod_common.h"
+#include <atomic>
 
 #define PE_M 128
-#define PE_N 128
+#define PE_PROD_MIN_GRID 512
+#ifndef PE_WIDE_MIN_GRID
+#define PE_WIDE_MIN_GRID 1024
+#endif
 #define PE_PLANE (128 * 64)
 
 __device__ __forceinline__ int pe_swz(int row, int chunk) { return chunk ^ (((row >> 3) & 1) << 1); }
 
-template <bool X3, bool U8, int P>
-__global__ __launch_bounds__(256) void patch_embed_kernel(const void* __restrict__ img_, const bf16_t* __restrict__ Wp, int ldw,
-                                                          const float* __restrict__ bias, const float* __restrict__ pos,
-                                                          float* __restrict__ out, int B, int H, int W, int gh, int gw, int D) {
+__device__ __forceinline__ float pe_rows4_sum(float v) {
+  unsigned b = __float_as_uint(v);
+  const auto s16 = __builtin_amdgcn_permlane16_swap(b, b, false, false);
+  v = __uint_as_float(s16[0]) + __uint_as_float(s16[1]);
+  b = __float_as_uint(v);
+  const auto s32 = __builtin_amdgcn_permlane32_swap(b, b, false, false);
+  return __uint_as_float(s32[0]) + __uint_as_float(s32[1]);
+}
+
+template <bool X3, bool U8, int P, int NW, bool PROD>
+__global__ __launch_bounds__(256 * NW) void patch_embed_kernel(const void* __restrict__ img_, const bf16_t* __restrict__ Wp, int ldw,
+                                                               const float* __restrict__ bias, const float* __restrict__ pos,
+                                                               float* __restrict__ out, int B, int H, int W, int gh, int gw, int D, PeProd pr) {
   constexpr int p = P;
   extern __shared__ __attribute__((aligned(16))) char smem[];
-  constexpr int NPL = X3 ? 4 : 2;
-  constexpr int STAGE = NPL * PE_PLANE;
+  constexpr int NT = 256 * NW, PE_N = 128 * NW, WN = 2 * NW;
+  constexpr int NA = X3 ? 2 : 1;
+  constexpr int WPL = NW * PE_PLANE;
+  constexpr int STAGE = NA * (PE_PLANE + WPL);
   const int tid = threadIdx.x, lane = tid & 63, wid = tid >> 6;
   const int wu = __builtin_amdgcn_readfirstlane(wid);
-  const int wm = wu >> 1, wn = wu & 1;
+  const int wm = wu / WN, wn = wu % WN;
   const int Np = gh * gw, Mtot = B * Np;
   const int tiles_m = (Mtot + PE_M - 1) / PE_M;
   const int tiles_n = (D + PE_N - 1) / PE_N;
@@ -26,14 +41,16 @@
   const int m0 = tm * PE_M, n0 = tn * PE_N;
   const int nsteps = 3 * (p / 2), kp = nsteps * 32;
 
-  constexpr int NP2 = P / 2;
-  unsigned goff[NP2];
-  int lofs[NP2];
+  constexpr int NP2 = P / 2, PAIRS = 256 * NP2;
+  constexpr int NPASS = (PAIRS + NT - 1) / NT;
+  unsigned goff[NPASS];
+  int lofs[NPASS];
   size_t cstride, rstride;
   if (U8) { cstride = 1; rstride = (size_t)W * 3; } else { cstride = (size_t)H * W; rstride = (size_t)W; }
 #pragma unroll
-  for (int i = 0; i < NP2; ++i) {
-    const int e = tid + 256 * i;
+  for (int i = 0; i < NPASS; ++i) {
+    int e = tid + NT * i;
+    if (PAIRS % NT != 0) e = e < PAIRS ? e : e - PAIRS;
     const int rr = e / (PE_M * NP2), rem_e = e - rr * (PE_M * NP2), pl = rem_e / NP2, j = 2 * (rem_e - pl * NP2);
     int m = m0 + pl; m = m < Mtot ? m : Mtot - 1;
     const int b = m / Np, rem = m - b * Np, py = rem / gw, px = rem - py * gw;
@@ -42,7 +59,7 @@
     const int kq = rr * 16 + j;
     lofs[i] = pl * 64 + pe_swz(pl, kq >> 3) * 16 + (kq & 7) * 2;
   }
-  float pv0[P], pv1[P], pv2[P];
+  float pv0[2 * NPASS], pv1[2 * NPASS], pv2[2 * NPASS];
   uint4 wA0, wB0, wC0, wD0, wA1, wB1, wC1, wD1, wA2, wB2, wC2, wD2;
   const bf16_t* gWr;
   int wofs0, wofs1;
@@ -57,7 +74,7 @@
   {                                                                                                         \
     const int c_ = (s_) / (p / 2), si_ = (s_) - c_ * (p / 2);                                               \
     const size_t o_ = c_ * cstride + (size_t)(2 * si_) * rstride;                                           \
-    _Pragma("unroll") for (int i = 0; i < NP2; ++i) {                                                       \
+    _Pragma("unroll") for (int i = 0; i < NPASS; ++i) {                                                     \
       if (U8) {                                                                                             \
         const unsigned char* q_ = (const unsigned char*)img_ + goff[i] + o_;                                \
         PV[2 * i] = (float)q_[0] / 255.0f; PV[2 * i + 1] = (float)q_[3] / 255.0f;              \
@@ -73,16 +90,16 @@
 #define PE_SWRITE(PV, WA, WB, WC, WD, stage_)                                                               \
   {                                                                                                         \
     char* sa_ = smem + (stage_) * STAGE;                                                                    \
-    _Pragma("unroll") for (int i = 0; i < NP2; ++i) {                                                       \
+    _Pragma("unroll") for (int i = 0; i < NPASS; ++i) {                                                     \
       const unsigned hi_ = pack2bf(PV[2 * i], PV[2 * i + 1]);                                               \
       *reinterpret_cast<unsigned*>(sa_ + lofs[i]) = hi_;                                                    \
       if (X3) *reinterpret_cast<unsigned*>(sa_ + PE_PLANE + lofs[i]) =                                      \
           pack2bf(PV[2 * i] - __uint_as_float(hi_ << 16), PV[2 * i + 1] - __uint_as_float(hi_ & 0xffff0000u)); \
     }                                                                                                       \
-    char* sw_ = sa_ + (X3 ? 2 : 1) * PE_PLANE;                                                              \
+    char* sw_ = sa_ + NA * PE_PLANE;                                                                        \
     *reinterpret_cast<uint4*>(sw_ + wofs0) = WA;                                                            \
     *reinterpret_cast<uint4*>(sw_ + wofs1) = WB;                                                            \
-    if (X3) { *reinterpret_cast<uint4*>(sw_ + PE_PLANE + wofs0) = WC; *reinterpret_cast<uint4*>(sw_ + PE_PLANE + wofs1) = WD; } \
+    if (X3) { *reinterpret_cast<uint4*>(sw_ + WPL + wofs0) = WC; *reinterpret_cast<uint4*>(sw_ + WPL + wofs1) = WD; } \
   }
 
   f32x4 acc[4][4];
@@ -95,11 +112,11 @@
 #pragma unroll
   for (int i = 0; i < 4; ++i) { const int row = wm * 64 + i * 16 + l15; offA[i] = row * 64 + pe_swz(row, l4) * 16; }
 #pragma unroll
-  for (int j = 0; j < 4; ++j) { const int row = wn * 64 + j * 16 + l15; offW[j] = (X3 ? 2 : 1) * PE_PLANE + row * 64 + pe_swz(row, l4) * 16; }
-
-  for (int i = tid; i < 2 * STAGE / 16; i += 256) {
+  for (int j = 0; j < 4; ++j) { const int row = wn * 64 + j * 16 + l15; offW[j] = NA * PE_PLANE + row * 64 + pe_swz(row, l4) * 16; }
+
+  for (int i = tid; i < 2 * STAGE / 16; i += NT) {
     const int st_ = i / (STAGE / 16), o_ = (i - st_ * (STAGE / 16)) * 16;
-    if (o_ < (X3 ? 2 : 1) * PE_PLANE) *reinterpret_cast<uint4*>(smem + st_ * STAGE + o_) = make_uint4(0u, 0u, 0u, 0u);
+    if (o_ < NA * PE_PLANE) *reinterpret_cast<uint4*>(smem + st_ * STAGE + o_) = make_uint4(0u, 0u, 0u, 0u);
   }
   __syncthreads();
   auto compute = [&](int stage) {
@@ -108,7 +125,7 @@
 #pragma unroll
     for (int j = 0; j < 4; ++j) {
       wh[j] = *reinterpret_cast<const bf16x8*>(st + offW[j]);
-      if (X3) wl[j] = *reinterpret_cast<const bf16x8*>(st + offW[j] + PE_PLANE);
+      if (X3) wl[j] = *reinterpret_cast<const bf16x8*>(st + offW[j] + WPL);
     }
 #pragma unroll
     for (int i = 0; i < 4; ++i) {
@@ -145,20 +162,67 @@
     __syncthreads();
   }
   const int N = Np + 1;
+  float gs[4], gq[4], gk[4];
 #pragma unroll
   for (int i = 0; i < 4; ++i) {
     const int m = m0 + wm * 64 + i * 16 + l15;
-    if (m >= Mtot) continue;
-    const int b = m / Np, rem = m - b * Np;
-    float* orow = out + ((size_t)b * N + 1 + rem) * D;
+    const bool mv = m < Mtot;
+    if (!PROD && !mv) continue;
+    const int mc = mv ? m : Mtot - 1;
+    const int b = mc / Np, rem = mc - b * Np;
+    const size_t orow_i = (size_t)b * N + 1 + rem;
+    float* orow = out + orow_i * D;
     const float* prow = pos + (size_t)(1 + rem) * D;
+    float kk = 0.f, ssum = 0.f, qsum = 0.f;
+    if (PROD) kk = pr.kshift[1 + rem];
+    uint2 pk[4];
 #pragma unroll
     for (int j = 0; j < 4; ++j) {
       const int n = n0 + wn * 64 + j * 16 + 4 * l4;
+      if (PROD) pk[j] = make_uint2(0u, 0u);
       if (n >= D) continue;
       const float4 bv = *reinterpret_cast<const float4*>(bias + n), pp = *reinterpret_cast<const float4*>(prow + n);
       const f32x4 a = acc[i][j];
-      *reinterpret_cast<float4*>(orow + n) = make_float4(a[0] + bv.x + pp.x, a[1] + bv.y + pp.y, a[2] + bv.z + pp.z, a[3] + bv.w + pp.w);
+      const float4 v = make_float4(a[0] + bv.x + pp.x, a[1] + bv.y + pp.y, a[2] + bv.z + pp.z, a[3] + bv.w + pp.w);
+      if (mv) *reinterpret_cast<float4*>(orow + n) = v;
+      if (PROD) {
+        pk[j] = make_uint2(pack2bf(v.x, v.y), pack2bf(v.z, v.w));
+        const float d0 = v.x - kk, d1 = v.y - kk, d2 = v.z - kk, d3 = v.w - kk;
+        ssum += (d0 + d1) + (d2 + d3);
+        qsum += (d0 * d0 + d1 * d1) + (d2 * d2 + d3 * d3);
+      }
+    }
+    if (PROD) {
+#pragma unroll
+      for (int j = 0; j < 4; j += 2) {
+        const auto r0 = __builtin_amdgcn_permlane16_swap(pk[j].x, pk[j + 1].x, false, false);
+        const auto r1 = __builtin_amdgcn_permlane16_swap(pk[j].y, pk[j + 1].y, false, false);
+        const int n = n0 + wn * 64 + (j + (l4 & 1)) * 16 + 4 * (l4 & 2);
+        if (mv && n < D) *reinterpret_cast<uint4*>(pr.op + orow_i * D + n) = make_uint4(r0[0], r1[0], r0[1], r1[1]);
+      }
+    }
+    if (PROD) { gs[i] = pe_rows4_sum(ssum); gq[i] = pe_rows4_sum(qsum); gk[i] = kk; }
+  }
+  if (PROD) {
+    float2* red = reinterpret_cast<float2*>(smem);
+    if ((wn & 1) && l4 == 0) {
+#pragma unroll
+      for (int i = 0; i < 4; ++i) red[(wn >> 1) * PE_M + wm * 64 + i * 16 + l15] = make_float2(gs[i], gq[i]);
+    }
+    __syncthreads();
+    const int ng = n0 + (wn >> 1) * 128;
+    if (!(wn & 1) && l4 == 0 && ng < D) {
+      const int npart = (D + 127) >> 7;
+#pragma unroll
+      for (int i = 0; i < 4; ++i) {
+        const int rl = wm * 64 + i * 16 + l15, m = m0 + rl;
+        if (m >= Mtot) continue;
+        const int b = m / Np, rem = m - b * Np;
+        const size_t orow_i = (size_t)b * N + 1 + rem;
+        const float2 o = red[(wn >> 1) * PE_M + rl];
+        pr.part[orow_i * npart + (ng >> 7)] = make_float2(gs[i] + o.x, gq[i] + o.y);
+        if (ng == 0) pr.shift_out[orow_i] = make_float2(gk[i], 0.f);
+      }
     }
   }
 }
@@ -188,24 +252,39 @@
   return hipGetLastError() == hipSuccess ? 0 : 3;
 }
 
+static std::atomic<long> g_pe_wide_launches{0};
+long pe_wide_launch_count() { return g_pe_wide_launches.load(); }
+bool pe_producer_pays(int B, int gh, int gw, int D) {
+  const int tiles_m8 = ((B * gh * gw + PE_M - 1) / PE_M + 7) / 8 * 8;
+  return tiles_m8 * ((D + 127) / 128) > PE_PROD_MIN_GRID;
+}
+static bool pe_wide_tile(int tiles_m8, int D) { return D > 128 && tiles_m8 * ((D + 255) / 256) >= PE_WIDE_MIN_GRID; }
+
 int launch_patch_embed(const void* img, int u8, int B, int H, int W, int p, const bf16_t* Wp, int x3, const float* bias, const float* pos,
-                       float* out, int D, hipStream_t s) {
+                       float* out, int D, hipStream_t s, const PeProd* prod) {
   if ((p != 14 && p != 16) || D % 4 != 0 || B <= 0 || (!u8 && (W & 1))) return 2;
   const int gh = H / p, gw = W / p;
   if (gh <= 0 || gw <= 0) return 2;
   if ((size_t)B * 3 * H * W >= 0xffffffffull) return 2;
+  if (prod && (x3 || D % 8 != 0 || !prod->op || !prod->part || !prod->shift_out || !prod->kshift)) return 2;
   const int kp = 3 * (p / 2) * 32, ldw = x3 ? 2 * kp : kp;
-  const int tiles = ((((B * gh * gw) + PE_M - 1) / PE_M + 7) / 8 * 8) * ((D + PE_N - 1) / PE_N);
-  const int lds = 2 * (x3 ? 4 : 2) * PE_PLANE;
-#define PE_LAUNCH(X3_, U8_, P_) hipLaunchKernelGGL((patch_embed_kernel<X3_, U8_, P_>), dim3(tiles), dim3(256), lds, s, img, Wp, ldw, bias, pos, out, B, H, W, gh, gw, D)
-  if (p == 14) {
-    if (x3) { if (u8) PE_LAUNCH(true, true, 14); else PE_LAUNCH(true, false, 14); }
-    else { if (u8) PE_LAUNCH(false, true, 14); else PE_LAUNCH(false, false, 14); }
-  } else {
-    if (x3) { if (u8) PE_LAUNCH(true, true, 16); else PE_LAUNCH(true, false, 16); }
-    else { if (u8) PE_LAUNCH(false, true, 16); else PE_LAUNCH(false, false, 16); }
-  }
+  const int tiles_m8 = (((B * gh * gw) + PE_M - 1) / PE_M + 7) / 8 * 8;
+  const bool wide = prod && (prod->tile == 2 || (prod->tile == 0 && pe_wide_tile(tiles_m8, D)));
+  const int nw = wide ? 2 : 1;
+  const int tiles = tiles_m8 * ((D + 128 * nw - 1) / (128 * nw));
+  const int lds = 2 * (x3 ? 2 : 1) * (1 + nw) * PE_PLANE;
+  const PeProd pr = prod ? *prod : PeProd{nullptr, nullptr, nullptr, nullptr, 0};
+#define PE_GO(X3_, U8_, P_, NW_, PR_) hipLaunchKernelGGL((patch_embed_kernel<X3_, U8_, P_, NW_, PR_>), dim3(tiles), dim3(256 * NW_), lds, s, img, Wp, ldw, bias, pos, out, B, H, W, gh, gw, D, pr)
+#define PE_LAUNCH(U8_, P_)                                                         \
+  if (x3) PE_GO(true, U8_, P_, 1, false);                                          \
+  else if (!prod) PE_GO(false, U8_, P_, 1, false);                                 \
+  else if (wide) PE_GO(false, U8_, P_, 2, true);                                   \
+  else PE_GO(false, U8_, P_, 1, true);
+  if (p == 14) { if (u8) { PE_LAUNCH(true, 14) } else { PE_LAUNCH(false, 14) } }
+  else { if (u8) { PE_LAUNCH(true, 16) } else { PE_LAUNCH(false, 16) } }
 #undef PE_LAUNCH
+#undef PE_GO
   gemm_form_launched(FORM_PATCH_FUSED);
+  if (wide) ++g_pe_wide_launches;
   return hipGetLastError() == hipSuccess ? 0 : 3;
 }
diff --git a/dinov2_od_amd/csrc/rowops.hip b/dinov2_od_amd/csrc/rowops.hip
--- a/dinov2_od_amd/csrc/rowops.hip
+++ b/dinov2_od_amd/csrc/rowops.hip
@@ -1,4 +1,5 @@
 #include "dod_common.h"
+#include <atomic>
 
 #define LN_MAXC 8
 enum { LN_F32 = 1, LN_BF16 = 2, LN_PAIR = 4, LN_H2 = 8, LN_FP8 = 16, LN_S3 = 32, LN_FP8MX = 64 };
@@ -254,9 +255,13 @@
 #undef RS_GO
 }
 
+static std::atomic<long> g_rowstats_launches{0};
+long rowstats_launch_count() { return g_rowstats_launches.load(); }
+
 int launch_rowstats(const float* x, int rows, int D, float eps, void* op, int op_kind, float2* stats, hipStream_t s) {
   if (rows <= 0) return 1;
   if (D % 4 != 0 || D > 256 * LN_MAXC || !op || !stats) return 2;
+  ++g_rowstats_launches;
   if (op_kind == LNOP_H2) { if (D % 32) return 2; rowstats_dispatch<LNOP_H2>(x, rows, D, eps, op, stats, s); }
   else if (op_kind == LNOP_PAIR) rowstats_dispatch<LNOP_PAIR>(x, rows, D, eps, op, stats, s);
   else if (op_kind == LNOP_BF16) rowstats_dispatch<LNOP_BF16>(x, rows, D, eps, op, stats, s);
@@ -358,8 +363,53 @@
   const int b = i / D, d = i - b * D;
   x[(size_t)b * N * D + d] = cls[d] + pos[d];
 }
-int launch_cls_row(const float* cls, const float* pos, float* x, int B, int N, int D, hipStream_t s) {
-  hipLaunchKernelGGL(cls_row_kernel, dim3((B * D + 255) / 256), dim3(256), 0, s, cls, pos, x, B, N, D);
+__global__ __launch_bounds__(64) void cls_row_prod_kernel(const float* __restrict__ cls, const float* __restrict__ pos, float* __restrict__ x,
+                                                          int B, int N, int D, PeProd pr) {
+  const int npart = (D + 127) >> 7;
+  const int b = blockIdx.x / npart, g = blockIdx.x - b * npart;
+  const int lane = threadIdx.x, n = g * 128 + 4 * lane;
+  const size_t row = (size_t)b * N;
+  const float k = pr.kshift[0];
+  float s = 0.f, q = 0.f;
+  if (lane < 32 && n < D) {
+    const float4 c = *reinterpret_cast<const float4*>(cls + n), p = *reinterpret_cast<const float4*>(pos + n);
+    const float4 v = make_float4(c.x + p.x, c.y + p.y, c.z + p.z, c.w + p.w);
+    *reinterpret_cast<float4*>(x + row * D + n) = v;
+    *reinterpret_cast<uint2*>(pr.op + row * D + n) = make_uint2(pack2bf(v.x, v.y), pack2bf(v.z, v.w));
+    const float a0 = v.x - k, a1 = v.y - k, a2 = v.z - k, a3 = v.w - k;
+    s = (a0 + a1) + (a2 + a3);
+    q = (a0 * a0 + a1 * a1) + (a2 * a2 + a3 * a3);
+  }
+  s = wave_sum(s); q = wave_sum(q);
+  if (lane == 0) {
+    pr.part[row * npart + g] = make_float2(s, q);
+    if (g == 0) pr.shift_out[row] = make_float2(k, 0.f);
+  }
+}
+int launch_cls_row(const float* cls, const float* pos, float* x, int B, int N, int D, hipStream_t s, const PeProd* prod) {
+  if (prod) {
+    if (D % 4 != 0 || !prod->op || !prod->part || !prod->shift_out || !prod->kshift) return 2;
+    hipLaunchKernelGGL(cls_row_prod_kernel, dim3(B * ((D + 127) / 128)), dim3(64), 0, s, cls, pos, x, B, N, D, *prod);
+  } else {
+    hipLaunchKernelGGL(cls_row_kernel, dim3((B * D + 255) / 256), dim3(256), 0, s, cls, pos, x, B, N, D);
+  }
+  return hipGetLastError() == hipSuccess ? 0 : 3;
+}
+
+__global__ __launch_bounds__(256) void embed_shift_kernel(const float* __restrict__ cls, const float* __restrict__ bias, const float* __restrict__ pos,
+                                                          int N, int D, float* __restrict__ kshift) {
+  const int lane = threadIdx.x & 63;
+  const int t = blockIdx.x * 4 + (threadIdx.x >> 6);
+  if (t >= N) return;
+  const float* add = t == 0 ? cls : bias;
+  float acc = 0.f;
+  for (int n = lane; n < D; n += 64) acc += add[n] + pos[(size_t)t * D + n];
+  acc = wave_sum(acc);
+  if (lane == 0) kshift[t] = acc / (float)D;
+}
+int launch_embed_shift(const float* cls, const float* bias, const float* pos, int N, int D, float* kshift, hipStream_t s) {
+  if (N <= 0 || D <= 0) return 1;
+  hipLaunchKernelGGL(embed_shift_kernel, dim3((N + 3) / 4), dim3(256), 0, s, cls, bias, pos, N, D, kshift);
   return hipGetLastError() == hipSuccess ? 0 : 3;
 }
 
```

Result: no change. 2581 images/s (median of 6 runs) (+0.2%).
